# StarsX/RayTracedGGX

Measured on AMD Instinct MI355X. Metric: Mrays/s + ms/frame, bunny 1920x1080 1spp+denoise, 1/2/4/8 GPUs, higher is better.
Workload: dtype f32; 1 GPU; configs[1]: bunny.obj + rnl_cross env, 1920x1080, 1spp GGX reflection + full denoise chain (refl H,V; diff H,V, shared-memory variant; temporal; tone map), all-metal default materials, dt=1/60; parallelism=row strips x1, history_apron_rows=18, history_overreach_rows=0, setup_priming_frames=256, trace_workgroup_waves=12

## Files before the change

include/rtggx.h:

```cpp
#ifndef RTGGX_H
#define RTGGX_H

#include <stddef.h>
#include <stdint.h>

#ifdef __cplusplus
extern "C" {
#endif

typedef struct rtggx_context rtggx_context;

enum { RTGGX_GROUND = 0, RTGGX_MODEL_OBJ = 1, RTGGX_NUM_MESH = 2 };

typedef struct RtggxCBGlobal {
  float    WorldViewProjs[2][16];
  float    WorldViewProjsPrev[2][16];
  float    Worlds[2][12];
  float    WorldITs0[12];
  float    WorldIT1[11];
  uint32_t FrameIndex;
} RtggxCBGlobal;
typedef struct RtggxRayGenConstants {
  float ProjToWorld[16];
  float EyePt[4];
  float ProjBias[2];
  float pad[2];
} RtggxRayGenConstants;
typedef struct RtggxCBPerObject {
  float WorldViewProj[16];
  float ProjBias[2];
  float pad[2];
} RtggxCBPerObject;
typedef struct RtggxCBMaterial {
  float BaseColors[2][4];
  float RoughMetals[2][4];
} RtggxCBMaterial;
typedef struct RtggxFrameConstants {
  RtggxCBGlobal        global;
  RtggxRayGenConstants rayGen;
  RtggxCBPerObject     perObject[2];
  RtggxCBMaterial      material;
} RtggxFrameConstants;

enum { RTGGX_FORMAT_RGBA32F = 2, RTGGX_FORMAT_RGBA16F = 10, RTGGX_FORMAT_BC6H_UF16 = 95, RTGGX_FORMAT_BC6H_SF16 = 96 };

enum {
  RTGGX_BUF_VISIBILITY = 0,
  RTGGX_BUF_DEPTH = 1,
  RTGGX_BUF_NORMAL = 2,
  RTGGX_BUF_ROUGH_METAL = 3,
  RTGGX_BUF_VELOCITY = 4,
  RTGGX_BUF_RT_REFL = 5,
  RTGGX_BUF_RT_DIFF = 6,
  RTGGX_BUF_TSS0 = 7,
  RTGGX_BUF_TSS1 = 8,
  RTGGX_BUF_FLT_RFL = 9,
  RTGGX_BUF_FLT_DFF = 10,
  RTGGX_BUF_BACKBUFFER = 11,
  RTGGX_BUF_SH_COEFFS = 12,
  RTGGX_BUF_BVH_NODES0 = 13,
  RTGGX_BUF_BVH_TRIS0 = 14,
  RTGGX_BUF_BVH_NODES1 = 15,
  RTGGX_BUF_BVH_TRIS1 = 16,
  RTGGX_BUF_TLAS = 17,
  RTGGX_BUF_ENV = 18,
  RTGGX_BUF_BVH4_NODES0 = 19,
  RTGGX_BUF_BVH4_NODES1 = 20,
  RTGGX_BUF_BIN_WORK = 21,
  RTGGX_BUF_BVH4_TOP0 = 22,
  RTGGX_BUF_BVH4_TOP1 = 23,
  RTGGX_BUF_EXCHANGE_TOKENS = 24,
  RTGGX_BUF_ACC_REFL = 25,
  RTGGX_BUF_ACC_DIFF = 26,
  RTGGX_BUF_CONVERGED = 27,
  RTGGX_BUF_COUNT = 28
};

typedef struct RtggxTimings {
  float update_as, visibility, ray_trace, spatial_refl_h, spatial_refl_v, spatial_diff_h, spatial_diff_v,
        temporal, tone_map, frame,
        ray_trace_kernel;
} RtggxTimings;

const char* rtggx_last_error(void);

int  rtggx_create(rtggx_context** out, uint32_t width, uint32_t height, int device);
void rtggx_destroy(rtggx_context* ctx);

int  rtggx_set_strip(rtggx_context* ctx, uint32_t row_begin, uint32_t row_end);

int  rtggx_set_history_apron(rtggx_context* ctx, uint32_t rows);
int  rtggx_history_overreach(rtggx_context* ctx, uint32_t* rows, int reset);

int  rtggx_set_stream(rtggx_context* ctx, void* hip_stream);
int  rtggx_get_stream(rtggx_context* ctx, void** hip_stream);
#define RTGGX_MAX_PEERS 16
#define RTGGX_IPC_HANDLE_BYTES 64
int  rtggx_set_history_peers(rtggx_context* ctx, uint32_t world, const uint32_t* bounds, void* const* tss0, void* const* tss1);
int  rtggx_history_ipc_export(rtggx_context* ctx, void* handles, size_t bytes);
int  rtggx_history_ipc_open(rtggx_context* ctx, const void* handles, size_t bytes, void** tss0, void** tss1);

int  rtggx_set_async_compute(rtggx_context* ctx, int enable);

int  rtggx_set_mesh(rtggx_context* ctx, uint32_t slot, const float* verts, uint32_t num_verts,
                    const uint32_t* indices, uint32_t num_indices);
int  rtggx_set_env(rtggx_context* ctx, int format, uint32_t size, uint32_t mips, const void* data, size_t bytes);
enum { RTGGX_ENV_EQUIRECT = 0, RTGGX_ENV_VCROSS = 1, RTGGX_ENV_HCROSS = 2 };
enum { RTGGX_PIXELS_RGBE8 = 0, RTGGX_PIXELS_RGB32F = 1 };
int  rtggx_set_env_image(rtggx_context* ctx, int layout, int pixels, uint32_t width, uint32_t height, const void* data, size_t bytes,
                         uint32_t cube_size);
int  rtggx_generate_env_mips(rtggx_context* ctx);
int  rtggx_set_material(rtggx_context* ctx, uint32_t mesh, const float base_color[4], float roughness, float metallic);
int  rtggx_set_metallic(rtggx_context* ctx, uint32_t mesh, float metallic);
int  rtggx_set_sampler(rtggx_context* ctx, int vndf);
int  rtggx_set_ray_rate(rtggx_context* ctx, uint32_t pixels_per_ray);
#define RTGGX_MAX_RECURSION_DEPTH 4u
int  rtggx_set_max_recursion_depth(rtggx_context* ctx, uint32_t depth);
#define RTGGX_MAX_SAMPLES_PER_PIXEL 8u
int  rtggx_set_samples_per_pixel(rtggx_context* ctx, uint32_t samples);
#define RTGGX_MIN_SAMPLE_SET 256u
#define RTGGX_MAX_SAMPLE_SET 65536u
int  rtggx_set_sample_set(rtggx_context* ctx, uint32_t size);
int  rtggx_set_accumulation(rtggx_context* ctx, int enable);
int  rtggx_reset_accumulation(rtggx_context* ctx);
int  rtggx_accumulated_frames(rtggx_context* ctx, uint32_t* frames);
int  rtggx_present_accumulation(rtggx_context* ctx);

typedef struct RtggxScore {
  uint64_t index;
  uint32_t frame_index;
  uint32_t pad;
  uint64_t pixels, covered;
  uint64_t skipped_out, skipped_raw;
  double se_out_rgb, se_out_luma;
  double se_raw_rgb, se_raw_luma;
  double ref_rgb2, ref_luma2;
  double se_out_rgb_cov, se_raw_rgb_cov, ref_rgb2_cov;
} RtggxScore;
enum { RTGGX_SCORE_RING = 256 };
int  rtggx_set_reference(rtggx_context* ctx, const void* rgba16f, size_t bytes);
int  rtggx_reference_from_accumulation(rtggx_context* ctx);
int  rtggx_set_scoring(rtggx_context* ctx, int enable);
int  rtggx_read_scores(rtggx_context* ctx, RtggxScore* out, uint32_t capacity, uint32_t* count);

int  rtggx_set_sample_map(rtggx_context* ctx, const uint8_t* counts, uint32_t blocks_x, uint32_t blocks_y);
int  rtggx_read_sample_map(rtggx_context* ctx, uint8_t* counts, uint32_t capacity, uint32_t* blocks_x, uint32_t* blocks_y);

int  rtggx_build_as(rtggx_context* ctx);

int  rtggx_refit_as(rtggx_context* ctx, uint32_t slot, const float* verts, uint32_t num_verts);
int  rtggx_refit_as_device(rtggx_context* ctx, uint32_t slot, const float* device_verts, uint32_t num_verts, void* hip_stream);
int  rtggx_set_refit_policy(rtggx_context* ctx, float rebuild_ratio, uint32_t steps_per_frame);
int  rtggx_refit_stats(rtggx_context* ctx, uint32_t slot, float* cost_ratio, uint32_t* refits, uint32_t* rebuilds);

int  rtggx_update_frame(rtggx_context* ctx, const RtggxFrameConstants* constants);
int  rtggx_update_as(rtggx_context* ctx);
int  rtggx_transform_sh(rtggx_context* ctx);
int  rtggx_render_visibility(rtggx_context* ctx);
int  rtggx_ray_trace(rtggx_context* ctx);
int  rtggx_denoise(rtggx_context* ctx, int use_shared_mem);
int  rtggx_tone_map(rtggx_context* ctx);

int  rtggx_debug_fuse_tone_map(rtggx_context* ctx, int mode);
int  rtggx_debug_placement(rtggx_context* ctx, int force_small, uint32_t* key, uint32_t* where);
int  rtggx_debug_tile_words(rtggx_context* ctx, int enable);
int  rtggx_debug_static_sky(rtggx_context* ctx, int enable);
int  rtggx_debug_sky_runs(rtggx_context* ctx, uint32_t* runs, uint32_t capacity, uint32_t* tiles_x, uint32_t* tiles_y, uint32_t* threshold);
int  rtggx_debug_settled_sky(rtggx_context* ctx, int enable);
int  rtggx_debug_settled_words(rtggx_context* ctx, uint32_t* words0, uint32_t* words1, uint32_t capacity, uint32_t* blocks_x, uint32_t* blocks_y, uint32_t* epoch);
int  rtggx_debug_collapse_weights(rtggx_context* ctx, const float* set, float* get);
int  rtggx_debug_fence_wait(rtggx_context* ctx, double* us_total, uint32_t* waits, int reset);

int  rtggx_sync(rtggx_context* ctx);
int  rtggx_ray_count(rtggx_context* ctx, uint64_t* rays);
int  rtggx_ray_total(rtggx_context* ctx, uint64_t* rays, int reset);
int  rtggx_debug_counters(rtggx_context* ctx, uint32_t* out, uint32_t n, int reset);
int  rtggx_debug_trace_split(rtggx_context* ctx, uint32_t work_per_wave, uint32_t max_shift, int capacity, uint32_t* last_demand);
int  rtggx_debug_trace_residency(rtggx_context* ctx, uint32_t force_waves, uint32_t* waves, float* share);
int  rtggx_debug_environment(rtggx_context* ctx, const float* dirs3, const float* levels, uint32_t n, int level0_path, float* rgb3);
int  rtggx_get_timings(rtggx_context* ctx, RtggxTimings* out);
#define RTGGX_KERNEL_RING 4096
int  rtggx_enable_timing(rtggx_context* ctx, int mode);
int  rtggx_kernel_times(rtggx_context* ctx, float* ms, uint32_t capacity, uint32_t* count);

int  rtggx_debug_shader_clock(rtggx_context* ctx, double* mhz);

int  rtggx_copy_bandwidth(rtggx_context* ctx, size_t bytes, int iterations, double* gbytes_per_s);

int  rtggx_buffer_size(rtggx_context* ctx, int buffer_id, size_t* bytes);
int  rtggx_readback(rtggx_context* ctx, int buffer_id, void* dst, size_t bytes);
int  rtggx_buffer_ptr(rtggx_context* ctx, int buffer_id, void** device_ptr);
int  rtggx_upload(rtggx_context* ctx, int buffer_id, const void* src, size_t bytes);
int  rtggx_frame_parity(rtggx_context* ctx, uint32_t* parity);
int  rtggx_bvh_root(rtggx_context* ctx, uint32_t slot, int32_t* root);

int  rtggx_trace_rays(rtggx_context* ctx, const float* rays, uint32_t n, float* out);

#ifdef __cplusplus
}
#endif
#endif
```

raytracedggx_amd/capi.py:

```python
import ctypes as C
import os

import numpy as np

_HERE = os.path.dirname(os.path.abspath(__file__))
LIB_PATH = os.path.join(_HERE, "librtggx.so")

BUF_VISIBILITY, BUF_DEPTH, BUF_NORMAL, BUF_ROUGH_METAL, BUF_VELOCITY, BUF_RT_REFL, BUF_RT_DIFF, BUF_TSS0, BUF_TSS1, \
    BUF_FLT_RFL, BUF_FLT_DFF, BUF_BACKBUFFER, BUF_SH_COEFFS, BUF_BVH_NODES0, BUF_BVH_TRIS0, BUF_BVH_NODES1, BUF_BVH_TRIS1, \
    BUF_TLAS, BUF_ENV, BUF_BVH4_NODES0, BUF_BVH4_NODES1, BUF_BIN_WORK, BUF_BVH4_TOP0, BUF_BVH4_TOP1, BUF_EXCHANGE_TOKENS, \
    BUF_ACC_REFL, BUF_ACC_DIFF, BUF_CONVERGED = range(28)
MAX_PEERS, IPC_HANDLE_BYTES = 16, 64
FORMAT_RGBA32F, FORMAT_RGBA16F, FORMAT_BC6H_UF16, FORMAT_BC6H_SF16 = 2, 10, 95, 96
ENV_EQUIRECT, ENV_VCROSS, ENV_HCROSS = 0, 1, 2
PIXELS_RGBE8, PIXELS_RGB32F = 0, 1

_BUF_DTYPE = {BUF_VISIBILITY: np.uint32, BUF_DEPTH: np.uint32, BUF_NORMAL: np.uint32, BUF_ROUGH_METAL: np.uint16,
              BUF_VELOCITY: np.uint32, BUF_RT_REFL: np.uint32, BUF_RT_DIFF: np.uint32, BUF_TSS0: np.uint64, BUF_TSS1: np.uint64,
              BUF_FLT_RFL: np.uint64, BUF_FLT_DFF: np.uint64, BUF_BACKBUFFER: np.uint32, BUF_SH_COEFFS: np.float32,
              BUF_BVH_NODES0: np.uint32, BUF_BVH_TRIS0: np.uint32, BUF_BVH_NODES1: np.uint32, BUF_BVH_TRIS1: np.uint32,
              BUF_TLAS: np.float32, BUF_ENV: np.uint16, BUF_BVH4_NODES0: np.uint32, BUF_BVH4_NODES1: np.uint32, BUF_BIN_WORK: np.uint32,
              BUF_BVH4_TOP0: np.uint32, BUF_BVH4_TOP1: np.uint32, BUF_EXCHANGE_TOKENS: np.uint32,
              BUF_ACC_REFL: np.float32, BUF_ACC_DIFF: np.float32, BUF_CONVERGED: np.uint64}

EXPORTS = ["rtggx_last_error", "rtggx_create", "rtggx_destroy", "rtggx_set_strip", "rtggx_set_stream", "rtggx_set_mesh",
           "rtggx_set_env", "rtggx_set_material", "rtggx_set_metallic", "rtggx_build_as", "rtggx_update_frame", "rtggx_update_as",
           "rtggx_transform_sh", "rtggx_render_visibility", "rtggx_ray_trace", "rtggx_denoise", "rtggx_tone_map", "rtggx_sync",
           "rtggx_ray_count", "rtggx_get_timings", "rtggx_enable_timing", "rtggx_buffer_size", "rtggx_readback", "rtggx_buffer_ptr",
           "rtggx_upload", "rtggx_frame_parity", "rtggx_bvh_root", "rtggx_trace_rays", "rtggx_ray_total", "rtggx_kernel_times", "rtggx_debug_counters", "rtggx_debug_trace_split", "rtggx_debug_trace_residency", "rtggx_get_stream", "rtggx_set_history_peers", "rtggx_history_ipc_export", "rtggx_history_ipc_open",
           "rtggx_set_async_compute", "rtggx_set_history_apron", "rtggx_history_overreach", "rtggx_copy_bandwidth", "rtggx_refit_as", "rtggx_refit_as_device", "rtggx_refit_stats", "rtggx_set_refit_policy", "rtggx_set_sampler", "rtggx_set_ray_rate", "rtggx_set_max_recursion_depth", "rtggx_set_samples_per_pixel", "rtggx_debug_fuse_tone_map", "rtggx_debug_placement", "rtggx_debug_tile_words", "rtggx_debug_static_sky", "rtggx_debug_settled_sky", "rtggx_debug_settled_words", "rtggx_debug_sky_runs", "rtggx_debug_collapse_weights", "rtggx_debug_fence_wait", "rtggx_debug_shader_clock", "rtggx_debug_environment",
           "rtggx_set_accumulation", "rtggx_reset_accumulation", "rtggx_accumulated_frames", "rtggx_present_accumulation", "rtggx_set_sample_set",
           "rtggx_set_reference", "rtggx_reference_from_accumulation", "rtggx_set_scoring", "rtggx_read_scores",
           "rtggx_set_env_image", "rtggx_generate_env_mips",
           "rtggx_set_sample_map", "rtggx_read_sample_map"]
SCORE_RING = 256


class Timings(C.Structure):
    _fields_ = [(n, C.c_float) for n in ("update_as", "visibility", "ray_trace", "spatial_refl_h", "spatial_refl_v",
                                         "spatial_diff_h", "spatial_diff_v", "temporal", "tone_map", "frame", "ray_trace_kernel")]


class Score(C.Structure):
    _fields_ = [("index", C.c_uint64), ("frame_index", C.c_uint32), ("pad", C.c_uint32), ("pixels", C.c_uint64), ("covered", C.c_uint64),
                ("skipped_out", C.c_uint64), ("skipped_raw", C.c_uint64)] + \
               [(n, C.c_double) for n in ("se_out_rgb", "se_out_luma", "se_raw_rgb", "se_raw_luma", "ref_rgb2", "ref_luma2",
                                          "se_out_rgb_cov", "se_raw_rgb_cov", "ref_rgb2_cov")]

    def as_dict(self):
        return {n: getattr(self, n) for n, _ in self._fields_ if n != "pad"}


_lib = None


def load():
    global _lib
    if _lib is not None:
        return _lib
    if not os.path.exists(LIB_PATH):
        raise ImportError("librtggx.so is not built: run `python -c 'import __graft_entry__ as g; g.build()'` "
                          "or `make -C raytracedggx_amd` (hipcc, gfx950). There is no CPU path.")
    L = C.CDLL(LIB_PATH)
    L.rtggx_last_error.restype = C.c_char_p
    vp = C.c_void_p
    L.rtggx_create.argtypes = [C.POINTER(vp), C.c_uint32, C.c_uint32, C.c_int]
    L.rtggx_destroy.argtypes = [vp]
    L.rtggx_destroy.restype = None
    L.rtggx_set_strip.argtypes = [vp, C.c_uint32, C.c_uint32]
    L.rtggx_set_stream.argtypes = [vp, vp]
    L.rtggx_set_async_compute.argtypes = [vp, C.c_int]
    L.rtggx_set_ray_rate.argtypes = [vp, C.c_uint32]
    L.rtggx_set_max_recursion_depth.argtypes = [vp, C.c_uint32]
    L.rtggx_set_samples_per_pixel.argtypes = [vp, C.c_uint32]
    L.rtggx_set_sample_set.argtypes = [vp, C.c_uint32]
    L.rtggx_set_accumulation.argtypes = [vp, C.c_int]
    L.rtggx_reset_accumulation.argtypes = [vp]
    L.rtggx_accumulated_frames.argtypes = [vp, C.POINTER(C.c_uint32)]
    L.rtggx_present_accumulation.argtypes = [vp]
    L.rtggx_set_reference.argtypes = [vp, vp, C.c_size_t]
    L.rtggx_reference_from_accumulation.argtypes = [vp]
    L.rtggx_set_scoring.argtypes = [vp, C.c_int]
    L.rtggx_read_scores.argtypes = [vp, C.POINTER(Score), C.c_uint32, C.POINTER(C.c_uint32)]
    L.rtggx_set_sample_map.argtypes = [vp, vp, C.c_uint32, C.c_uint32]
    L.rtggx_read_sample_map.argtypes = [vp, vp, C.c_uint32, C.POINTER(C.c_uint32), C.POINTER(C.c_uint32)]
    L.rtggx_set_history_apron.argtypes = [vp, C.c_uint32]
# ... 67 lines not shown

    def set_stream(self, stream_handle):
        self._check(self.L.rtggx_set_stream(self.h, C.c_void_p(stream_handle)))

    def shader_clock_mhz(self):
        m = C.c_double()
        self._check(self.L.rtggx_debug_shader_clock(self.h, C.byref(m)))
        return m.value

    def copy_bandwidth(self, nbytes=1 << 30, iterations=8):
        g = C.c_double()
        self._check(self.L.rtggx_copy_bandwidth(self.h, int(nbytes), int(iterations), C.byref(g)))
        return g.value

    def set_history_apron(self, rows):
        self._check(self.L.rtggx_set_history_apron(self.h, int(rows)))

    def history_overreach(self, reset=True):
        n = C.c_uint32()
        self._check(self.L.rtggx_history_overreach(self.h, C.byref(n), int(reset)))
        return n.value

    def set_async_compute(self, enable):
        self._check(self.L.rtggx_set_async_compute(self.h, int(bool(enable))))

    def set_mesh(self, slot, verts, indices):
        v = np.ascontiguousarray(verts, np.float32).reshape(-1, 6)
        i = np.ascontiguousarray(indices, np.uint32).reshape(-1)
        self._check(self.L.rtggx_set_mesh(self.h, slot, _p(v), v.shape[0], _p(i), i.size))

    def refit_as(self, slot, verts):
        v = np.ascontiguousarray(verts, np.float32).reshape(-1, 6)
        self._check(self.L.rtggx_refit_as(self.h, slot, _p(v), v.shape[0]))

    def refit_as_device(self, slot, device_ptr, num_verts, stream=0):
        self.L.rtggx_refit_as_device.argtypes = [C.c_void_p, C.c_uint32, C.c_void_p, C.c_uint32, C.c_void_p]
        self._check(self.L.rtggx_refit_as_device(self.h, slot, C.c_void_p(int(device_ptr)), int(num_verts), C.c_void_p(int(stream) or None)))

    def fence_wait(self, reset=True):
        us, n = C.c_double(0.0), C.c_uint32(0)
        self.L.rtggx_debug_fence_wait.argtypes = [C.c_void_p, C.POINTER(C.c_double), C.POINTER(C.c_uint32), C.c_int]
        self._check(self.L.rtggx_debug_fence_wait(self.h, C.byref(us), C.byref(n), 1 if reset else 0))
        return us.value, n.value

    def fuse_tone_map(self, mode):
        self._check(self.L.rtggx_debug_fuse_tone_map(self.h, -1 if mode is None else 1 if mode else 0))

    def tile_words(self, enable):
        self._check(self.L.rtggx_debug_tile_words(self.h, 1 if enable else 0))

    def static_sky(self, enable):
        self._check(self.L.rtggx_debug_static_sky(self.h, 1 if enable else 0))

    def sky_runs(self):
        tiles = ((self.W + 15) // 16) * ((self.H + 15) // 16 + 1)
        runs = np.zeros(tiles, np.uint32)
        tx, ty, th = C.c_uint32(), C.c_uint32(), C.c_uint32()
        self.L.rtggx_debug_sky_runs.argtypes = [C.c_void_p, C.c_void_p, C.c_uint32, C.c_void_p, C.c_void_p, C.c_void_p]
        self._check(self.L.rtggx_debug_sky_runs(self.h, _p(runs), tiles, C.byref(tx), C.byref(ty), C.byref(th)))
        return runs[:tx.value * ty.value].reshape(ty.value, tx.value), int(th.value)

    def settled_sky(self, enable):
        self.L.rtggx_debug_settled_sky.argtypes = [C.c_void_p, C.c_int]
        self._check(self.L.rtggx_debug_settled_sky(self.h, 1 if enable else 0))

    def settled_words(self):
        n = ((self.W + 63) // 64) * ((self.H + 3) // 4)
        w = np.zeros((2, n), np.uint32)
        bx, by, ep = C.c_uint32(), C.c_uint32(), C.c_uint32()
        self.L.rtggx_debug_settled_words.argtypes = [C.c_void_p, C.c_void_p, C.c_void_p, C.c_uint32, C.c_void_p, C.c_void_p, C.c_void_p]
        self._check(self.L.rtggx_debug_settled_words(self.h, _p(w[0]), _p(w[1]), n, C.byref(bx), C.byref(by), C.byref(ep)))
        return np.ascontiguousarray(w.reshape(2, bx.value, by.value).transpose(0, 2, 1)), int(ep.value)

    def placement(self, force_small=-1):
        k, w = C.c_uint32(), C.c_uint32()
        self.L.rtggx_debug_placement.argtypes = [C.c_void_p, C.c_int, C.c_void_p, C.c_void_p]
        self._check(self.L.rtggx_debug_placement(self.h, int(force_small), C.byref(k), C.byref(w)))
        names = ("main", "B", "C", "R", "?")
        key = {n: bool((k.value >> i) & 1) for i, n in enumerate(("small", "strip", "deforming", "diffuse", "caller_stream"))}
        where = {"raster": names[(w.value >> 16) & 15], "gen": names[w.value & 15], "trace": names[(w.value >> 4) & 15], "shade": names[(w.value >> 8) & 15], "frames_in_flight": (w.value >> 12) & 15}
        return key, where

    def collapse_weights(self, area=None, tris=None):
        self.L.rtggx_debug_collapse_weights.argtypes = [C.c_void_p, C.c_void_p, C.c_void_p]
        get = (C.c_float * 2)()
        if area is not None:
            st = (C.c_float * 2)(float(area), float(tris))
            self._check(self.L.rtggx_debug_collapse_weights(self.h, st, get))
        else:
            self._check(self.L.rtggx_debug_collapse_weights(self.h, None, get))
        return float(get[0]), float(get[1])

    def set_history_peers(self, bounds, tss0, tss1):
        self.L.rtggx_set_history_peers.argtypes = [C.c_void_p, C.c_uint32, C.c_void_p, C.c_void_p, C.c_void_p]
        if bounds is None:
            self._check(self.L.rtggx_set_history_peers(self.h, 0, None, None, None))
            return
        world = len(bounds) - 1
        b = (C.c_uint32 * (world + 1))(*[int(x) for x in bounds])
        p0 = (C.c_void_p * world)(*[C.c_void_p(int(x) or None) for x in tss0])
        p1 = (C.c_void_p * world)(*[C.c_void_p(int(x) or None) for x in tss1])
        self._check(self.L.rtggx_set_history_peers(self.h, world, b, p0, p1))

    def history_ipc_export(self):
        self.L.rtggx_history_ipc_export.argtypes = [C.c_void_p, C.c_void_p, C.c_size_t]
        buf = C.create_string_buffer(2 * IPC_HANDLE_BYTES)
# ... 250 lines not shown
```

raytracedggx_amd/csrc/context.hip:

```cpp
#include <cstdarg>
#include <cstdio>
#include <cstring>
#include <cmath>
#include <vector>
#include "capi_internal.h"
#include "rt_queue.h"

#ifndef RT_REFIT_REBUILD_RATIO
#define RT_REFIT_REBUILD_RATIO 1.2f
#endif
#ifndef RT_REBUILD_STEPS
#define RT_REBUILD_STEPS 16u
#endif
namespace rt {
static thread_local char g_err[512] = "";
void setError(const char* fmt, ...) {
  va_list ap; va_start(ap, fmt); vsnprintf(g_err, sizeof g_err, fmt, ap); va_end(ap);
}

__global__ void uploadParamsKernel(FrameParams src, FrameParams* dst) {
  const uint32_t* s = reinterpret_cast<const uint32_t*>(&src);
  uint32_t* d = reinterpret_cast<uint32_t*>(dst);
  for (uint32_t i = threadIdx.x; i < sizeof(FrameParams) / 4; i += blockDim.x) d[i] = s[i];
}
int uploadParams(rtggx_context* c, uint32_t slot, hipStream_t s) {
  hipLaunchKernelGGL(uploadParamsKernel, dim3(1), dim3(64), 0, s, c->slots[slot], c->dParams + slot);
  RT_HIP(hipGetLastError());
  return 0;
}
int resetSettled(rtggx_context* c) {
  for (auto& w : c->settled) {
    RT_HIP(hipMemset(w, 0xFF, c->settledWords() * 4));
    RT_HIP(hipMemset2D(w + c->settledPitch + 1u, (size_t)c->settledPitch * 4, 0, (size_t)c->settledY * 4, c->settledX));
  }
  RT_HIP(hipStreamSynchronize(nullptr));
  return 0;
}
int allocSet(rtggx_context* c, uint32_t i) {
  InputSet& s = c->sets[i];
  const size_t n = (size_t)c->W * c->H, slots = (size_t)c->numBinsMax * c->binSlots;
  for (DevBuf<uint32_t>* p : {&s.normal, &s.depth32, &s.velocity, &s.rtRefl, &s.rtDiff}) if (!*p) RT_HIP(allocFilled(*p, n));
  if (!s.roughMetal) RT_HIP(allocFilled(s.roughMetal, n));
  if (!s.rayQueue) RT_HIP(alloc(s.rayQueue, slots * sizeof(rt::RayRec)));
  if (!s.hitQueue) RT_HIP(alloc(s.hitQueue, slots * 8));
  if (!s.binCount) RT_HIP(allocFilled(s.binCount, (size_t)c->numBinsMax));
  if (!s.splitList) RT_HIP(alloc(s.splitList, (size_t)RT_SPLIT_CAP));
  if (!s.skyRun) RT_HIP(allocFilled(s.skyRun, c->skyTiles));
  c->breakSkyRuns();
  s.splitCount = c->largeCountBase + 2 + i;
  if (!s.evRead) RT_HIP(create(s.evRead, RT_EVENT_FLAGS));
  return 0;
}

static int initContext(rtggx_context* c, uint32_t width, uint32_t height, int device) {
  c->device = device; c->W = width; c->H = height; c->rowBegin = 0; c->rowEnd = height;
  const size_t n = (size_t)width * height;
  int prioLeast = 0, prioGreatest = 0;
  RT_HIP(hipDeviceGetStreamPriorityRange(&prioLeast, &prioGreatest));
  const int prioMid = (prioLeast + prioGreatest) / 2;
  RT_HIP(create(c->ownMain, hipStreamNonBlocking, prioGreatest));
  RT_HIP(create(c->ownAS, hipStreamNonBlocking, prioLeast));
  c->streamMain = c->ownMain; c->streamAS = c->ownAS;
  RT_HIP(create(c->ownVis, hipStreamNonBlocking, prioLeast)); c->streamVis = c->ownVis;
  RT_HIP(create(c->streamRefit, hipStreamNonBlocking, prioMid));
  for (Event* e : {&c->evVis, &c->evRefit, &c->evAS, &c->evRT}) RT_HIP(create(*e, RT_EVENT_FLAGS));
  for (auto& f : c->frames) { RT_HIP(create(f.gen, RT_EVENT_FLAGS)); RT_HIP(create(f.trace, RT_EVENT_FLAGS)); }
  for (auto& e : c->tev) RT_HIP(create(e));
  c->rebuildRatio = RT_REFIT_REBUILD_RATIO; c->rebuildSteps = RT_REBUILD_STEPS;
  {
    hipDeviceProp_t prop;
    RT_HIP(hipGetDeviceProperties(&prop, device));
    c->numCUs = prop.multiProcessorCount > 0 ? (uint32_t)prop.multiProcessorCount : 256u;
  }
  c->numBinsMax = ((width + 15) / 16) * ((height + 15) / 16) * 4u;
  if (c->numBinsMax < 64u) c->numBinsMax = 64u;
  c->binSlots = RT_BIN_MIN;
  c->largeCapacity = 1u << 16;
  c->skyTiles = (size_t)((width + 15) / 16) * ((height + 15) / 16 + 1);
  for (auto& b : c->largeTrisBuf) RT_HIP(alloc(b, (size_t)c->largeCapacity * 56));
  RT_HIP(allocFilled(c->largeCountBase, 2 + RT_SETS));
  for (uint32_t i = 0; i < RT_SETS; ++i) { const int r = allocSet(c, i); if (r) return r; }
  for (auto& v : c->vis) { RT_HIP(allocFilled(v.depth, n)); RT_HIP(allocFilled(v.dirty, c->skyTiles, 0xFF)); }
  RT_HIP(allocFilled(c->visDirtyOnes, c->skyTiles, 0xFF));
  c->settledX = (width + 63) / 64; c->settledY = (height + 3) / 4;
  c->settledPitch = (c->settledY + 3u) / 4u * 4u + 2u;
  for (auto& w : c->settled) RT_HIP(alloc(w, c->settledWords()));
  { const int r = resetSettled(c); if (r) return r; }
  RT_HIP(allocFilled(c->backbuffer, n));
  RT_HIP(allocFilled(c->tss[0], n)); RT_HIP(allocFilled(c->tss[1], n)); RT_HIP(allocFilled(c->fltRfl, n)); RT_HIP(allocFilled(c->fltDff, n));
  RT_HIP(allocFilled(c->rayCounter, 512));
  RT_HIP(allocFilled(c->rayCounterBuf, 1792));
  c->lastRayCounter32 = c->rayCounterBuf;
  RT_HIP(allocFilled(c->traceStamps, 8));
  RT_HIP(alloc(c->hostRayCounters, 264)); memset(c->hostRayCounters, 0, 264 * 4); RT_HIP(create(c->evRayCounters, hipEventDisableTiming));
  for (auto& b : c->binWorkBuf) RT_HIP(allocFilled(b, (size_t)c->numBinsMax));
  c->selectSet(0);
  c->splitWork = RT_SPLIT_WORK; c->splitMaxShift = RT_SPLIT_MAX_SHIFT;
  RT_HIP(allocFilled(c->dEnvMipOffset, 16));
  RT_HIP(allocFilled(c->dummyRecord, 128));
  RT_HIP(allocFilled(c->histReach, 1));
  RT_HIP(allocFilled(c->exchangeTokens, 2 * RT_MAX_PEERS));
  RT_HIP(allocFilled(c->dPeerTable, sizeof(void*) * 2 * RT_MAX_PEERS + 4 * (RT_MAX_PEERS + 1)));
  RT_HIP(allocFilled(c->sh, 27));
  RT_HIP(alloc(c->cosSinTab, 512));
  RT_HIP(alloc(c->dParams, RT_SLOTS));
  {
    float tab[512];
    for (int s = 0; s < 256; ++s) { const double phi = 2.0 * 3.14159265358979323846 * (double)s / 256.0; tab[s] = (float)cos(phi); tab[256 + s] = (float)sin(phi); }
    RT_HIP(hipMemcpy(c->cosSinTab, tab, sizeof tab, hipMemcpyHostToDevice));
  }
  const float bc0[4] = {0.95f, 0.93f, 0.88f, 1.0f}, bc1[4] = {1.0f, 0.71f, 0.29f, 1.0f};
  const float rm0[4] = {0.5f, 1.0f, 0.0f, 0.0f}, rm1[4] = {0.16f, 1.0f, 0.0f, 0.0f};
  memcpy(c->material.BaseColors[0], bc0, 16); memcpy(c->material.BaseColors[1], bc1, 16);
  memcpy(c->material.RoughMetals[0], rm0, 16); memcpy(c->material.RoughMetals[1], rm1, 16);
  memset(c->invWorld, 0, sizeof c->invWorld);
  for (int i = 0; i < 2; ++i) for (int k = 0; k < 4; ++k) c->invWorld[i][k * 5] = 1.0f;
  memset(c->slots, 0, sizeof c->slots);
  { const int r = setMeshImpl(c, RTGGX_GROUND, &kGroundVerts[0][0], 24, kGroundIdx, 36); if (r) return r; }
  RT_HIP(hipStreamSynchronize(nullptr));
  return 0;
}
int allocSamples(rtggx_context* c) {
  if (c->sppAcc && c->sppParams) return 0;
  const size_t n = (size_t)c->W * c->H;
  if (!c->evSpp) RT_HIP(create(c->evSpp, hipEventDisableTiming));
  if (!c->sppParams) RT_HIP(alloc(c->sppParams, RT_SLOTS * RTGGX_MAX_SAMPLES_PER_PIXEL));
  if (!c->sppAcc) {
    RT_HIP(allocFilled(c->sppAcc, n * 2u * 3u));
    RT_HIP(hipStreamSynchronize(nullptr));
  }
  return 0;
}
int allocSampleTable(rtggx_context* c, uint32_t m) {
  DevBuf<float>& tab = c->cosSinWide[rtggx_context::sampleSetSlot(m)];
  if (tab) return 0;
  std::vector<float> host(2u * (size_t)m);
  for (uint32_t s = 0; s < m; ++s) { const double phi = 2.0 * 3.14159265358979323846 * (double)s / (double)m; host[2u * s] = (float)cos(phi); host[2u * s + 1u] = (float)sin(phi); }
  DevBuf<float> d;
  hipError_t e = alloc(d, host.size());
  if (e == hipSuccess) e = hipMemcpy(d, host.data(), host.size() * sizeof(float), hipMemcpyHostToDevice);
  if (e != hipSuccess) { setError("rtggx_set_sample_set: %s (%zu bytes for the table of %u samples)", hipGetErrorString(e), host.size() * sizeof(float), m); return -2; }
  tab = std::move(d);
  return 0;
}
int allocAccumulation(rtggx_context* c) {
  if (c->accRefl) return 0;
  const size_t n = (size_t)c->W * c->H;
// ... 115 lines not shown
int rtggx_history_ipc_export(rtggx_context* c, void* handles, size_t bytes) {
  RT_CHECK_CTX(c);
  static_assert(sizeof(hipIpcMemHandle_t) == RTGGX_IPC_HANDLE_BYTES, "hipIpcMemHandle_t size");
  if (!handles || bytes < 2 * sizeof(hipIpcMemHandle_t)) { setError("rtggx_history_ipc_export: room for two %zu-byte handles", sizeof(hipIpcMemHandle_t)); return -1; }
  hipIpcMemHandle_t h[2];
  for (int p = 0; p < 2; ++p) RT_HIP(hipIpcGetMemHandle(&h[p], c->tss[p]));
  memcpy(handles, h, sizeof h);
  return 0;
}
int rtggx_history_ipc_open(rtggx_context* c, const void* handles, size_t bytes, void** tss0, void** tss1) {
  RT_CHECK_CTX(c);
  if (!handles || bytes < 2 * sizeof(hipIpcMemHandle_t) || !tss0 || !tss1) { setError("rtggx_history_ipc_open: bad arguments"); return -1; }
  hipIpcMemHandle_t h[2]; memcpy(h, handles, sizeof h);
  void* p[2] = {nullptr, nullptr};
  for (int k = 0; k < 2; ++k) {
    IpcMapping mapped;
    RT_HIP(hipIpcOpenMemHandle(mapped.put(), h[k], hipIpcMemLazyEnablePeerAccess));
    p[k] = mapped;
    c->ipcMapped.push_back(std::move(mapped));
  }
  *tss0 = p[0]; *tss1 = p[1];
  return 0;
}

int rtggx_get_stream(rtggx_context* c, void** stream) {
  RT_CHECK_CTX(c);
  if (!stream) { setError("rtggx_get_stream: null"); return -1; }
  *stream = (void*)c->streamMain;
  return 0;
}

int rtggx_set_async_compute(rtggx_context* c, int enable) {
  RT_CHECK_CTX(c);
  if ((enable != 0) == c->asyncCompute) return 0;
  RT_HIP(syncStreams(c));
  c->asyncCompute = enable != 0; c->sppStream = nullptr;
  c->streamAS = c->asyncCompute ? c->ownAS : c->streamMain;
  c->streamVis = c->asyncCompute ? c->ownVis : nullptr;
  c->evVisStream = nullptr; for (auto& f : c->frames) f.genFrame = 0u;
  return 0;
}

int rtggx_set_ray_rate(rtggx_context* c, uint32_t pixelsPerRay) {
  RT_CHECK_CTX(c);
  if (pixelsPerRay != 1u && pixelsPerRay != 4u) { setError("rtggx_set_ray_rate: %u pixels per ray: 1 or 4", pixelsPerRay); return -1; }
  if (pixelsPerRay != 1u && c->samplesRequested > 1u) { setError("rtggx_set_ray_rate: rate %u on a context tracing %u samples per pixel (rtggx_set_samples_per_pixel): one asks for fewer rays, the other for more", pixelsPerRay, c->samplesRequested); return -1; }
  if (pixelsPerRay != 1u && c->accumulateRequested) { setError("rtggx_set_ray_rate: rate %u on an accumulating context (rtggx_set_accumulation): three quarters of such a frame are interpolations", pixelsPerRay); return -1; }
  if (pixelsPerRay != 1u && (c->rowBegin > 0u || c->rowEnd < c->H)) { setError("rtggx_set_ray_rate: rate %u on a strip (rows [%u,%u) of %u): whole frames only", pixelsPerRay, c->rowBegin, c->rowEnd, c->H); return -1; }
  if (pixelsPerRay == c->rayRate) return 0;
  RT_HIP(syncStreams(c));
  c->rayRate = pixelsPerRay;
  for (auto& b : c->binWorkBuf) RT_HIP(hipMemset(b, 0, (size_t)c->numBinsMax * 4));
  RT_HIP(hipDeviceSynchronize());
  c->splitDemand = 0u; c->rayCountersInFlight = false; c->lastFrameRays = 0xFFFFFFFFu; c->traceLaunches = 0u;
  return 0;
}

int rtggx_set_max_recursion_depth(rtggx_context* c, uint32_t depth) {
  RT_CHECK_CTX(c);
  if (depth < 1u || depth > RTGGX_MAX_RECURSION_DEPTH) { setError("rtggx_set_max_recursion_depth: depth %u: 1 to %u", depth, RTGGX_MAX_RECURSION_DEPTH); return -1; }
  c->depthRequested = depth;
  return 0;
}

int rtggx_set_samples_per_pixel(rtggx_context* c, uint32_t samples) {
  RT_CHECK_CTX(c);
  if (samples != 1u && samples != 2u && samples != 4u && samples != 8u) { setError("rtggx_set_samples_per_pixel: %u samples per pixel: 1, 2, 4 or %u", samples, RTGGX_MAX_SAMPLES_PER_PIXEL); return -1; }
  if (samples > 1u && c->rayRate != 1u) { setError("rtggx_set_samples_per_pixel: %u samples per pixel on a context tracing one pixel in %u (rtggx_set_ray_rate): one asks for more rays, the other for fewer", samples, c->rayRate); return -1; }
  if (samples > 1u) { const int r = allocSamples(c); if (r) return r; }
  c->samplesRequested = samples;
  return 0;
}

int rtggx_set_sample_set(rtggx_context* c, uint32_t size) {
  RT_CHECK_CTX(c);
  if (size < RTGGX_MIN_SAMPLE_SET || size > RTGGX_MAX_SAMPLE_SET || (size & (size - 1u)) != 0u) { setError("rtggx_set_sample_set: %u samples: a power of two from %u to %u", size, RTGGX_MIN_SAMPLE_SET, RTGGX_MAX_SAMPLE_SET); return -1; }
  if (size == c->sampleSetRequested) return 0;
  RT_HIP(syncStreams(c));
  if (size > RTGGX_MIN_SAMPLE_SET) { const int r = allocSampleTable(c, size); if (r) return r; }
  c->sampleSetRequested = size;
  return 0;
}

int rtggx_set_accumulation(rtggx_context* c, int enable) {
  RT_CHECK_CTX(c);
  if (enable && c->rayRate != 1u) { setError("rtggx_set_accumulation: on a context tracing one pixel in %u (rtggx_set_ray_rate): three quarters of such a frame are interpolations", c->rayRate); return -1; }
  if (enable) { const int r = allocAccumulation(c); if (r) return r; }
  c->accumulateRequested = enable != 0;
  return 0;
}
int rtggx_reset_accumulation(rtggx_context* c) {
  RT_CHECK_CTX(c);
  if (c->accRefl) {
    const size_t n = (size_t)c->W * c->H;
    RT_HIP(hipMemsetAsync(c->accRefl, 0, n * 16, c->streamMain));
    RT_HIP(hipMemsetAsync(c->accDiff, 0, n * 16, c->streamMain));
  }
  c->accumFrames = 0u;
  return 0;
}
int rtggx_accumulated_frames(rtggx_context* c, uint32_t* frames) {
  RT_CHECK_CTX(c);
  if (!frames) { setError("rtggx_accumulated_frames: null result"); return -1; }
  *frames = c->accumFrames;
  return 0;
}
int rtggx_present_accumulation(rtggx_context* c) {
// ... 180 lines not shown
```

raytracedggx_amd/csrc/debug.hip:

```cpp
#include <cstring>
#include "capi_internal.h"
#include "rt_queue.h"
namespace rt {
__global__ void __launch_bounds__(256) copyKernel(const float4* __restrict__ src, float4* __restrict__ dst, size_t n) {
  for (size_t i = (size_t)blockIdx.x * 256u + threadIdx.x; i < n; i += (size_t)gridDim.x * 256u) dst[i] = src[i];
}
typedef float __attribute__((ext_vector_type(4))) CopyVec4;
__global__ void __launch_bounds__(256) copyKernelNT(const CopyVec4* __restrict__ src, CopyVec4* __restrict__ dst, size_t n) {
  for (size_t i = (size_t)blockIdx.x * 256u + threadIdx.x; i < n; i += (size_t)gridDim.x * 256u) __builtin_nontemporal_store(__builtin_nontemporal_load(&src[i]), &dst[i]);
}
}
using namespace rt;

extern "C" {
int rtggx_ray_count(rtggx_context* c, uint64_t* rays) {
  RT_CHECK_CTX(c);
  uint32_t h[256];
  RT_HIP(syncStreams(c));
  RT_HIP(hipMemcpy(h, c->lastRayCounter32, sizeof h, hipMemcpyDeviceToHost));
  uint64_t s = 0; for (auto v : h) s += v;
  *rays = s;
  return 0;
}

int rtggx_debug_counters(rtggx_context* c, uint32_t* out, uint32_t n, int reset) {
  RT_CHECK_CTX(c);
  if (n > 768) { setError("rtggx_debug_counters: at most 768 words"); return -1; }
  RT_HIP(syncStreams(c));
  RT_HIP(hipMemcpy(out, c->rayCounterBuf + 1024, (size_t)n * 4, hipMemcpyDeviceToHost));
  if (reset) { RT_HIP(hipMemset(c->rayCounterBuf + 1024, 0, 768 * 4)); RT_HIP(hipStreamSynchronize(nullptr)); }
  return 0;
}

int rtggx_debug_fence_wait(rtggx_context* c, double* usTotal, uint32_t* waits, int reset) {
  RT_CHECK_CTX(c);
  if (usTotal) *usTotal = c->fenceWaitUs;
  if (waits) *waits = c->fenceWaits;
  if (reset) { c->fenceWaitUs = 0.0; c->fenceWaits = 0u; }
  return 0;
}
int rtggx_debug_fuse_tone_map(rtggx_context* c, int mode) {
  RT_CHECK_CTX(c);
  c->fuseToneMap = mode < 0 ? -1 : mode != 0;
  return 0;
}
int rtggx_debug_tile_words(rtggx_context* c, int enable) {
  RT_CHECK_CTX(c);
  c->useTileWords = enable != 0;
  c->breakSkyRuns();
  return 0;
}
int rtggx_debug_static_sky(rtggx_context* c, int enable) {
  RT_CHECK_CTX(c);
  c->staticSky = enable != 0;
  c->breakSkyRuns();
  return 0;
}
int rtggx_debug_sky_runs(rtggx_context* c, uint32_t* runs, uint32_t capacity, uint32_t* tilesX, uint32_t* tilesY, uint32_t* threshold) {
  RT_CHECK_CTX(c);
  const uint32_t n = c->skyGen.tilesX * c->skyGen.tilesY;
  if (!runs || capacity < n || n > c->skyTiles) { setError("rtggx_debug_sky_runs: room for %u words", n); return -1; }
  RT_HIP(syncStreams(c));
  if (n) RT_HIP(hipMemcpy(runs, c->cur().skyRun, (size_t)n * 4, hipMemcpyDeviceToHost));
  for (uint32_t i = 0; i < n; ++i) runs[i] = (runs[i] >> 8) == c->skyEpoch ? runs[i] & 0xFFu : 0u;
  if (tilesX) *tilesX = c->skyGen.tilesX;
  if (tilesY) *tilesY = c->skyGen.tilesY;
  if (threshold) *threshold = RT_SKY_PREV_RUN + 1u;
  return 0;
}
int rtggx_debug_settled_sky(rtggx_context* c, int enable) {
  RT_CHECK_CTX(c);
  c->settledSky = enable != 0;
  c->breakSkyRuns();
  return 0;
}
int rtggx_debug_settled_words(rtggx_context* c, uint32_t* words0, uint32_t* words1, uint32_t capacity, uint32_t* blocksX, uint32_t* blocksY, uint32_t* epoch) {
  RT_CHECK_CTX(c);
  const uint32_t n = c->settledX * c->settledY;
  if (!words0 || !words1 || capacity < n) { setError("rtggx_debug_settled_words: room for %u words each", n); return -1; }
  RT_HIP(syncStreams(c));
  uint32_t* const out[2] = {words0, words1};
  for (int p = 0; p < 2 && n; ++p)
    RT_HIP(hipMemcpy2D(out[p], (size_t)c->settledY * 4, c->settled[p] + c->settledPitch + 1u, (size_t)c->settledPitch * 4, (size_t)c->settledY * 4, c->settledX, hipMemcpyDeviceToHost));
  if (blocksX) *blocksX = c->settledX;
  if (blocksY) *blocksY = c->settledY;
  if (epoch) *epoch = c->skyEpoch;
  return 0;
}
int rtggx_debug_placement(rtggx_context* c, int forceSmall, uint32_t* key, uint32_t* where) {
  RT_CHECK_CTX(c);
  if (forceSmall < -1 || forceSmall > 1) { setError("rtggx_debug_placement: force_small is -1, 0 or 1"); return -1; }
  c->forcePlacement = forceSmall;
  if (forceSmall >= 0) c->lastTraceSmall = forceSmall == 1;
  if (key) *key = c->lastPlacement[0];
  if (where) *where = c->lastPlacement[1];
  return 0;
}
int rtggx_debug_collapse_weights(rtggx_context* c, const float* set, float* get) {
  RT_CHECK_CTX(c);
  if (set) { if (!(set[0] >= 0.0f) || !(set[1] >= 0.0f) || !(set[0] + set[1] > 0.0f)) { setError("rtggx_debug_collapse_weights: two non-negative weights, not both zero"); return -1; }
             c->collapseWeights[0] = set[0]; c->collapseWeights[1] = set[1]; }
  if (get) { get[0] = c->collapseWeights[0]; get[1] = c->collapseWeights[1]; }
  return 0;
}
int rtggx_debug_trace_residency(rtggx_context* c, uint32_t forceWaves, uint32_t* waves, float* share) {
  RT_CHECK_CTX(c);
  if (forceWaves != 0u && forceWaves != 10u && forceWaves != 12u && forceWaves != 14u && forceWaves != 16u) { setError("rtggx_debug_trace_residency: %u waves: 0, 10, 12, 14 or 16", forceWaves); return -1; }
  c->traceWavesForced = forceWaves;
  if (forceWaves) c->traceWaves = forceWaves;
  if (waves) *waves = c->traceWaves;
  if (share) *share = c->traceShare;
  return 0;
}

int rtggx_debug_environment(rtggx_context* c, const float* dirs3, const float* levels, uint32_t n, int level0Path, float* rgb3) {
  RT_CHECK_CTX(c);
  if (!c->env.texels) { setError("rtggx_debug_environment: no environment map"); return -1; }
  if (n == 0 || !dirs3 || !rgb3 || (!levels && !level0Path)) { setError("rtggx_debug_environment: no directions, levels or result (n %u)", n); return -1; }
  DevBuf<float> dD, dL, dO;
  hipError_t e = alloc(dD, (size_t)n * 3);
  if (e == hipSuccess) e = alloc(dO, (size_t)n * 3);
  if (e == hipSuccess && levels) e = alloc(dL, (size_t)n);
  if (e == hipSuccess) e = hipMemcpy(dD, dirs3, (size_t)n * 12, hipMemcpyHostToDevice);
  if (e == hipSuccess && levels) e = hipMemcpy(dL, levels, (size_t)n * 4, hipMemcpyHostToDevice);
  int r = 0;
  if (e == hipSuccess) r = launchDebugEnvironment(c, dD, dL, n, level0Path, dO, c->streamMain);
  if (e == hipSuccess && !r) e = hipStreamSynchronize(c->streamMain);
  if (e == hipSuccess && !r) e = hipMemcpy(rgb3, dO, (size_t)n * 12, hipMemcpyDeviceToHost);
  if (e != hipSuccess) { setError("rtggx_debug_environment: %s", hipGetErrorString(e)); return -2; }
  return r;
}

int rtggx_debug_trace_split(rtggx_context* c, uint32_t workPerWave, uint32_t maxShift, int capacity, uint32_t* lastDemand) {
  RT_CHECK_CTX(c);
  if (maxShift > 3u) { setError("rtggx_debug_trace_split: max_shift %u > 3", maxShift); return -1; }
  if (capacity > (int)RT_SPLIT_CAP) { setError("rtggx_debug_trace_split: capacity %d > %u", capacity, RT_SPLIT_CAP); return -1; }
  RT_HIP(syncStreams(c));
  if (lastDemand) RT_HIP(hipMemcpy(lastDemand, c->cur().splitCount, 4, hipMemcpyDeviceToHost));
  c->splitWork = workPerWave; c->splitMaxShift = maxShift;
  c->splitCapForced = capacity < 0 ? 0xFFFFFFFFu : ((uint32_t)capacity / 32u) * 32u;
  return 0;
}

int rtggx_ray_total(rtggx_context* c, uint64_t* rays, int reset) {
  RT_CHECK_CTX(c);
  unsigned long long h[256];
  RT_HIP(syncStreams(c));
  RT_HIP(hipMemcpy(h, c->rayCounter + 256, sizeof h, hipMemcpyDeviceToHost));
// ... 12 lines not shown
    for (uint32_t i = 0; i < RTGGX_KERNEL_RING; ++i) { RT_HIP(create(c->kevBegin[i])); RT_HIP(create(c->kevEnd[i])); }
  }
  return 0;
}
int rtggx_kernel_times(rtggx_context* c, float* ms, uint32_t capacity, uint32_t* count) {
  RT_CHECK_CTX(c);
  RT_HIP(syncStreams(c));
  const uint32_t n = c->kevCount < capacity ? c->kevCount : capacity;
  for (uint32_t i = 0; i < n; ++i) RT_HIP(hipEventElapsedTime(&ms[i], c->kevBegin[i], c->kevEnd[i]));
  *count = n;
  c->kevCount = 0;
  return 0;
}
int rtggx_get_timings(rtggx_context* c, RtggxTimings* out) {
  RT_CHECK_CTX(c);
  if (!c->timing || !c->timingsPending) { setError("rtggx_get_timings: timing not enabled or no complete frame"); return -1; }
  RT_HIP(syncStreams(c));
  auto ms = [&](int a, int b) { float t = 0.0f; hipEventElapsedTime(&t, c->tev[a], c->tev[b]); return t; };
  RtggxTimings t;
  t.update_as = ms(0, 1); t.visibility = ms(2, 13); t.ray_trace = ms(3, 14); t.spatial_refl_h = ms(9, 4); t.spatial_refl_v = ms(4, 5);
  t.spatial_diff_h = ms(5, 6); t.spatial_diff_v = ms(6, 7); t.temporal = ms(7, 8); t.tone_map = ms(8, 10); t.frame = ms(2, 10);
  t.ray_trace_kernel = ms(11, 12);
  *out = t;
  return 0;
}

static int bufferInfo(rtggx_context* c, int id, void** ptr, size_t* bytes) {
  const size_t n = (size_t)c->W * c->H;
  switch (id) {
    case RTGGX_BUF_VISIBILITY: case RTGGX_BUF_DEPTH: *ptr = nullptr; *bytes = n * 4; return 0;
    case RTGGX_BUF_NORMAL: *ptr = c->cur().normal; *bytes = n * 4; return 0;
    case RTGGX_BUF_ROUGH_METAL: *ptr = c->cur().roughMetal; *bytes = n * 2; return 0;
    case RTGGX_BUF_VELOCITY: *ptr = c->cur().velocity; *bytes = n * 4; return 0;
    case RTGGX_BUF_RT_REFL: *ptr = c->cur().rtRefl; *bytes = n * 4; return 0;
    case RTGGX_BUF_RT_DIFF: *ptr = c->cur().rtDiff; *bytes = n * 4; return 0;
    case RTGGX_BUF_TSS0: *ptr = c->tss[0]; *bytes = n * 8; return 0;
    case RTGGX_BUF_TSS1: *ptr = c->tss[1]; *bytes = n * 8; return 0;
    case RTGGX_BUF_FLT_RFL: *ptr = c->fltRflIsFltDff ? c->fltDff.get() : c->fltRfl.get(); *bytes = n * 8; return 0;
    case RTGGX_BUF_FLT_DFF: *ptr = c->fltDff; *bytes = n * 8; return 0;
    case RTGGX_BUF_BACKBUFFER: *ptr = c->backbuffer; *bytes = n * 4; return 0;
    case RTGGX_BUF_SH_COEFFS: *ptr = c->sh; *bytes = 108; return 0;
    case RTGGX_BUF_BVH_NODES0: case RTGGX_BUF_BVH_NODES1: { const MeshDev& m = c->mesh[id == RTGGX_BUF_BVH_NODES1]; *ptr = m.nodes; *bytes = m.numTris > 1 && m.nodes ? (size_t)(m.numTris - 1) * 64 : 0; return 0; }
    case RTGGX_BUF_BVH_TRIS0: case RTGGX_BUF_BVH_TRIS1: { const MeshDev& m = c->mesh[id == RTGGX_BUF_BVH_TRIS1]; *ptr = m.tris; *bytes = m.tris ? (size_t)m.numTris * 64 : 0; return 0; }
    case RTGGX_BUF_TLAS: *ptr = nullptr; *bytes = 128; return 0;
    case RTGGX_BUF_BVH4_NODES0: case RTGGX_BUF_BVH4_NODES1: { const MeshDev& m = c->mesh[id == RTGGX_BUF_BVH4_NODES1]; *ptr = m.nodes4; *bytes = m.numTris > 1 && m.nodes4 ? (size_t)(m.numTris - 1) * sizeof(Bvh4Node) : 0; return 0; }
    case RTGGX_BUF_BVH4_TOP0: case RTGGX_BUF_BVH4_TOP1: { const MeshDev& m = c->mesh[id == RTGGX_BUF_BVH4_TOP1]; *ptr = m.top; *bytes = m.top ? (size_t)m.topCount * sizeof(Bvh4Node) : 0; return 0; }
    case RTGGX_BUF_BIN_WORK: *ptr = c->binWork; *bytes = (size_t)(((c->W + 15) / 16) * ((c->H + 15) / 16)) * 4u * 4u; return 0;
    case RTGGX_BUF_ENV: *ptr = c->env.texels; *bytes = (size_t)c->env.totalTexels * 8; return 0;
    case RTGGX_BUF_EXCHANGE_TOKENS: *ptr = c->exchangeTokens; *bytes = 4 * 2 * RT_MAX_PEERS; return 0;
    case RTGGX_BUF_ACC_REFL: case RTGGX_BUF_ACC_DIFF: case RTGGX_BUF_CONVERGED:
      if (!c->accRefl) { setError("buffer %d exists once accumulation has been enabled (rtggx_set_accumulation)", id); return -1; }
      *ptr = id == RTGGX_BUF_ACC_REFL ? (void*)c->accRefl : id == RTGGX_BUF_ACC_DIFF ? (void*)c->accDiff : (void*)c->converged;
      *bytes = n * (id == RTGGX_BUF_CONVERGED ? 8u : 16u); return 0;
    default: setError("unknown buffer id %d", id); return -1;
  }
}

int rtggx_buffer_size(rtggx_context* c, int id, size_t* bytes) { RT_CHECK_CTX(c); void* p; return bufferInfo(c, id, &p, bytes); }

int rtggx_buffer_ptr(rtggx_context* c, int id, void** dptr) {
  RT_CHECK_CTX(c);
  size_t bytes;
  const int r = bufferInfo(c, id, dptr, &bytes);
  if (r) return r;
  if (id == RTGGX_BUF_VISIBILITY || id == RTGGX_BUF_DEPTH) *dptr = c->curVis().depth;
  if (!*dptr) { setError("buffer %d has no device storage", id); return -1; }
  return 0;
}

int rtggx_readback(rtggx_context* c, int id, void* dst, size_t bytes) {
  RT_CHECK_CTX(c);
  void* p; size_t need;
  int r = bufferInfo(c, id, &p, &need);
  if (r) return r;
  if (bytes < need) { setError("rtggx_readback: buffer %d needs %zu bytes, %zu given", id, need, bytes); return -1; }
  RT_HIP(syncStreams(c));
  if (id == RTGGX_BUF_TLAS) { memcpy(dst, c->invWorld, 128); return 0; }
  if (id == RTGGX_BUF_VISIBILITY || id == RTGGX_BUF_DEPTH) {
    DevBuf<uint32_t> dVis, dDepth;
    RT_HIP(alloc(dVis, need / 4)); RT_HIP(alloc(dDepth, need / 4));
    r = unpackVisDepth(c, dVis, dDepth, c->streamMain);
    if (!r && hipStreamSynchronize(c->streamMain) != hipSuccess) { setError("readback: stream sync failed"); r = -2; }
    if (!r) { hipError_t e = hipMemcpy(dst, id == RTGGX_BUF_VISIBILITY ? dVis.get() : dDepth.get(), need, hipMemcpyDeviceToHost); if (e != hipSuccess) { setError("hipMemcpy: %s", hipGetErrorString(e)); r = -2; } }
    return r;
  }
  if (need == 0) return 0;
  RT_HIP(hipMemcpy(dst, p, need, hipMemcpyDeviceToHost));
  return 0;
}

int rtggx_upload(rtggx_context* c, int id, const void* src, size_t bytes) {
  RT_CHECK_CTX(c);
  void* p; size_t need;
  int r = bufferInfo(c, id, &p, &need);
  if (r) return r;
  if (bytes != need) { setError("rtggx_upload: buffer %d is %zu bytes, %zu given", id, need, bytes); return -1; }
  RT_HIP(syncStreams(c));
  c->toneMapDone = false;
  c->curVis().flags.rasterFrame = 0u;
  c->breakSkyRuns();
  if (id == RTGGX_BUF_VISIBILITY || id == RTGGX_BUF_DEPTH) {
    DevBuf<uint32_t> dVis, dDepth;
    RT_HIP(alloc(dVis, need / 4)); RT_HIP(alloc(dDepth, need / 4));
    r = unpackVisDepth(c, dVis, dDepth, c->streamMain);
    if (!r && hipStreamSynchronize(c->streamMain) != hipSuccess) { setError("upload: stream sync failed"); r = -2; }
    if (!r) { hipError_t e = hipMemcpy(id == RTGGX_BUF_VISIBILITY ? dVis.get() : dDepth.get(), src, need, hipMemcpyHostToDevice); if (e != hipSuccess) { setError("hipMemcpy: %s", hipGetErrorString(e)); r = -2; } }
// ... 90 lines not shown
```

raytracedggx_amd/csrc/denoise.hip:

```cpp
#include <cstring>
#include <type_traits>
#include "rtggx_context.h"

namespace rt {

#define RT_RADIUS 16
#ifndef RT_VBW
#define RT_VBW 16
#define RT_VBH 16
#endif

RT_DEV float rcpFast(float x) { return __builtin_amdgcn_rcpf(x); }

struct GTexel { float nx, ny, nz, nw, rough, metal, depth; };

RT_DEV GTexel loadG(const uint32_t* __restrict__ normal, const uint16_t* __restrict__ roughMetal, const uint32_t* __restrict__ depth32,
                    int x, int y, int W, int H) {
  GTexel g;
  if (x < 0 || y < 0 || x >= W || y >= H) { g.nx = g.ny = g.nz = -1023.0f; g.nw = 0.0f; g.rough = 0.0f; g.metal = 0.0f; g.depth = 0.0f; return g; }
  const size_t i = (size_t)y * W + x;
  const uint32_t n = normal[i];
  g.nx = (float)(2 * (int)(n & 1023u) - 1023);
  g.ny = (float)(2 * (int)((n >> 10) & 1023u) - 1023);
  g.nz = (float)(2 * (int)((n >> 20) & 1023u) - 1023);
  g.nw = (float)(n >> 30) * (1.0f / 3.0f);
  const uint32_t rm = roughMetal[i];
  g.rough = (float)(rm & 0xFFu) * (1.0f / 255.0f); g.metal = (rm >> 8) == 255u ? 1.0f : (float)(rm >> 8) * (1.0f / 255.0f);
  g.depth = (float)depth32[i] * (1.0f / 16777215.0f);
  return g;
}
RT_DEV f3 TM3(f3 c) { const float r = rcpFast(1.0f + ((c.x * 0.25f + c.y * 0.5f) + c.z * 0.25f)); return mk3(c.x * r, c.y * r, c.z * r); }
RT_DEV f3 ITM3(f3 c) { const float r = rcpFast(1.0f - ((c.x * 0.25f + c.y * 0.5f) + c.z * 0.25f)); return mk3(c.x * r, c.y * r, c.z * r); }
struct Targets {
  const uint32_t* normal; const uint16_t* roughMetal; const uint32_t* depth32; const uint32_t* velocity;
  const uint32_t* rtRefl; const uint32_t* rtDiff;
  uint2* scratch; const uint2* history; uint2* fltRfl; uint2* fltDff; uint32_t* backbuffer;
  int W, H, rowBegin, rowEnd;
  int histLo, histHi; uint32_t* histReach;
  const uint2* const* peerHist; const uint32_t* peerBounds; int peerWorld;
  int outBegin, outEnd;
  const uint32_t* tileWords; int tilesX, tileRow0;
  const uint32_t* skyRun; uint32_t skyEpoch;
  uint32_t* settledOut; const uint32_t* settledIn; uint32_t settledPitch;
};
#define RT_SGPR(v) ((uint32_t)__builtin_amdgcn_readfirstlane((int)(v)))
RT_DEV uint32_t tileWordsOr(const uint32_t* words, uint32_t i0, uint32_t i1, uint32_t i2, uint32_t i3) {
  uint32_t a, b, c, d;
  asm volatile("s_load_dword %0, %4, %5\n\ts_load_dword %1, %4, %6\n\ts_load_dword %2, %4, %7\n\ts_load_dword %3, %4, %8\n\ts_waitcnt lgkmcnt(0)"
               : "=&s"(a), "=&s"(b), "=&s"(c), "=&s"(d) : "s"(words), "s"(RT_SGPR(i0 * 4u)), "s"(RT_SGPR(i1 * 4u)), "s"(RT_SGPR(i2 * 4u)), "s"(RT_SGPR(i3 * 4u)) : "memory");
  return a | b | c | d;
}

RT_DEV uint32_t tileWordsOr6(const uint32_t* words, uint32_t i0, uint32_t i1, uint32_t i2, uint32_t i3, uint32_t i4, uint32_t i5) {
  uint32_t a, b, c, d, e, f;
  asm volatile("s_load_dword %0, %6, %7\n\ts_load_dword %1, %6, %8\n\ts_load_dword %2, %6, %9\n\ts_load_dword %3, %6, %10\n\ts_load_dword %4, %6, %11\n\ts_load_dword %5, %6, %12\n\ts_waitcnt lgkmcnt(0)"
               : "=&s"(a), "=&s"(b), "=&s"(c), "=&s"(d), "=&s"(e), "=&s"(f)
               : "s"(words), "s"(RT_SGPR(i0 * 4u)), "s"(RT_SGPR(i1 * 4u)), "s"(RT_SGPR(i2 * 4u)), "s"(RT_SGPR(i3 * 4u)), "s"(RT_SGPR(i4 * 4u)), "s"(RT_SGPR(i5 * 4u)) : "memory");
  return a | b | c | d | e | f;
}
RT_DEV uint32_t skyRunMin6(const uint32_t* words, uint32_t epoch, uint32_t i0, uint32_t i1, uint32_t i2, uint32_t i3, uint32_t i4, uint32_t i5) {
  uint32_t w[6];
  asm volatile("s_load_dword %0, %6, %7\n\ts_load_dword %1, %6, %8\n\ts_load_dword %2, %6, %9\n\ts_load_dword %3, %6, %10\n\ts_load_dword %4, %6, %11\n\ts_load_dword %5, %6, %12\n\ts_waitcnt lgkmcnt(0)"
               : "=&s"(w[0]), "=&s"(w[1]), "=&s"(w[2]), "=&s"(w[3]), "=&s"(w[4]), "=&s"(w[5])
               : "s"(words), "s"(RT_SGPR(i0 * 4u)), "s"(RT_SGPR(i1 * 4u)), "s"(RT_SGPR(i2 * 4u)), "s"(RT_SGPR(i3 * 4u)), "s"(RT_SGPR(i4 * 4u)), "s"(RT_SGPR(i5 * 4u)) : "memory");
  uint32_t run = 0xFFu;
#pragma unroll
  for (int k = 0; k < 6; ++k) run = min(run, (w[k] >> 8) == epoch ? w[k] & 0xFFu : 0u);
  return run;
}

typedef uint32_t U2 __attribute__((ext_vector_type(2)));
typedef uint32_t U4 __attribute__((ext_vector_type(4)));
RT_DEV void loadTemporalWords(const uint32_t* rowA, const uint32_t* rowB, const uint32_t* col0, const uint32_t* col1, const uint32_t* col2,
                              U4& a4, U2& a2, U4& b4, U2& b2, U4& c0, U4& c1, U4& c2) {
  asm volatile("s_load_dwordx4 %0, %7, 0x0\n\ts_load_dwordx2 %1, %7, 0x10\n\ts_load_dwordx4 %2, %8, 0x0\n\ts_load_dwordx2 %3, %8, 0x10\n\t"
               "s_load_dwordx4 %4, %9, 0x0\n\ts_load_dwordx4 %5, %10, 0x0\n\ts_load_dwordx4 %6, %11, 0x0\n\ts_waitcnt lgkmcnt(0)"
               : "=&s"(a4), "=&s"(a2), "=&s"(b4), "=&s"(b2), "=&s"(c0), "=&s"(c1), "=&s"(c2)
               : "s"(rowA), "s"(rowB), "s"(col0), "s"(col1), "s"(col2) : "memory");
}
RT_DEV void loadToneMapWords(const uint32_t* col0, const uint32_t* col1, const uint32_t* col2, U4& a4, U2& a2, U4& b4, U2& b2, U4& c4, U2& c2) {
  asm volatile("s_load_dwordx4 %0, %6, 0x0\n\ts_load_dwordx2 %1, %6, 0x10\n\ts_load_dwordx4 %2, %7, 0x0\n\ts_load_dwordx2 %3, %7, 0x10\n\t"
               "s_load_dwordx4 %4, %8, 0x0\n\ts_load_dwordx2 %5, %8, 0x10\n\ts_waitcnt lgkmcnt(0)"
               : "=&s"(a4), "=&s"(a2), "=&s"(b4), "=&s"(b2), "=&s"(c4), "=&s"(c2) : "s"(col0), "s"(col1), "s"(col2) : "memory");
}

#define RT_LOG2E 1.44269504088896341f

struct Centre { float nx, ny, nz, depth, rough, gaussK , depthK ; };
#define RT_NORMAL_SCALE_SQ 1046529.0f
RT_DEV float log2OfDot(float I) {
  const float d = fmaxf((I - RT_NORMAL_SCALE_SQ) * (1.0f / RT_NORMAL_SCALE_SQ), -1.0f);
  const float xr = 1.0f + d;
  const float dropped = (1.0f - xr) + d;
  return __builtin_fmaf(dropped, RT_LOG2E, __builtin_amdgcn_logf(xr));
}
template <bool DIFFUSE, int UNIFORM = 0>
RT_DEV float tapWeight(const Centre& c, int i, float nx, float ny, float nz, float depth, float rough) {
// ... 18 lines not shown
  const float sigma = (float)(br + 1) * (1.0f / 3.0f);
  c.gaussK = (-0.5f * RT_LOG2E) * rcpFast(sigma * sigma);
  c.depthK = depth * (4.0f * RT_LOG2E);
  return c;
}
template <int MODE>
RT_DEV void storeFiltered(const Targets& T, size_t pix, float mx, float my, float mz, float wsum) {
  const float rw = rcpFast(wsum);
  f3 mu = mk3(mx * rw, my * rw, mz * rw);
  if (MODE == 0 || MODE == 2) T.scratch[pix] = packRGBA16F(mu.x, mu.y, mu.z, 0.0f);
  if (MODE == 1) { mu = ITM3(mu); const uint2 v = packRGBA16F(mu.x, mu.y, mu.z, 1.0f); if (T.fltRfl) T.fltRfl[pix] = v; T.fltDff[pix] = v; }
  if (MODE == 3) {
    const f4 dest = unpackRGBA16F(T.fltRfl[pix]);
    mu = ITM3(mu);
    T.fltDff[pix] = packRGBA16F(dest.x + mu.x, dest.y + mu.y, dest.z + mu.z, dest.w);
  }
}
template <int MODE>
RT_DEV void storeSkipped(const Targets& T, size_t pix) {
  if (MODE == 1) { const f3 s = unpackR11G11B10F(T.rtRefl[pix]); const uint2 v = packRGBA16F(s.x, s.y, s.z, 0.0f); if (T.fltRfl) T.fltRfl[pix] = v; T.fltDff[pix] = v; }
}
template <int MODE>
RT_DEV f3 tapColour(const Targets& T, size_t ti) {
  if (MODE & 1) { const f4 v = unpackRGBA16F(T.scratch[ti]); return mk3(v.x, v.y, v.z); }
  return TM3(unpackR11G11B10F(MODE >= 2 ? T.rtDiff[ti] : T.rtRefl[ti]));
}

template <int MODE>
__global__ void __launch_bounds__(256) spatialDirectKernel(Targets T) {
  constexpr bool vertical = (MODE & 1) != 0;
  constexpr bool diffuse = MODE >= 2;
  const int x = blockIdx.x * 64 + (threadIdx.x & 63);
  const int y = T.rowBegin + blockIdx.y * 4 + (threadIdx.x >> 6);
  if (x >= T.W || y >= T.rowEnd) return;
  const size_t pix = (size_t)y * T.W + x;
  const GTexel gc = loadG(T.normal, T.roughMetal, T.depth32, x, y, T.W, T.H);
  if (diffuse ? (gc.nw <= 0.0f || gc.metal >= 1.0f) : (gc.nw <= 0.0f)) { storeSkipped<MODE>(T, pix); return; }
  const Centre c = makeCentre<diffuse>(gc.nx, gc.ny, gc.nz, gc.depth, gc.rough, T.W, T.H);
  float mx = 0.0f, my = 0.0f, mz = 0.0f, wsum = 0.0f;
  for (int i = -RT_RADIUS; i <= RT_RADIUS; ++i) {
    const int tx = vertical ? x : x + i, ty = vertical ? y + i : y;
    const bool inside = tx >= 0 && ty >= 0 && tx < T.W && ty < T.H;
    const GTexel g = loadG(T.normal, T.roughMetal, T.depth32, tx, ty, T.W, T.H);
    if (diffuse && (g.nw <= 0.0f || g.metal >= 1.0f)) continue;
    const f3 src = inside ? tapColour<MODE>(T, (size_t)ty * T.W + tx) : mk3(0.0f, 0.0f, 0.0f);
    const float w = tapWeight<diffuse>(c, i, g.nx, g.ny, g.nz, g.depth, g.nw > 0.0f ? g.rough : __uint_as_float(__float_as_uint(g.rough) | 0x80000000u));
    mx = __builtin_fmaf(src.x, w, mx); my = __builtin_fmaf(src.y, w, my); mz = __builtin_fmaf(src.z, w, mz);
    wsum += w;
  }
  storeFiltered<MODE>(T, pix, mx, my, mz, wsum);
}

typedef float V4 __attribute__((ext_vector_type(4)));
template <int MODE>
__global__ void __launch_bounds__(256) spatialTiledKernel(Targets T) {
  constexpr bool vertical = (MODE & 1) != 0;
  constexpr bool diffuse = MODE >= 2;
  constexpr int BW = vertical ? RT_VBW : 64, BH = vertical ? RT_VBH : 4;
  constexpr int TW = vertical ? RT_VBW : 96, TH = vertical ? RT_VBH + 2 * RT_RADIUS : 4;
  constexpr int PER = vertical ? BW * BH / 256 : 1, ROWSTEP = 256 / BW;
  constexpr int N = TW * TH;
  __shared__ V4 smA[N], smB[N];
  __shared__ uint32_t roughLo, roughHi, unflagged;
  if (threadIdx.x == 0) { roughLo = 0xFFFFFFFFu; roughHi = 0u; unflagged = 0u; }
  const int bx0 = blockIdx.x * BW, by0 = T.rowBegin + blockIdx.y * BH;
  const int lx = threadIdx.x % BW, ly = threadIdx.x / BW;
  const int x = bx0 + lx;

  static_assert(RT_VBW <= 32 && RT_VBH <= 32, "the V block spans at most two tiles across and three down");
  bool nothingDrawn;
  { const uint32_t txLast = (uint32_t)T.tilesX - 1u, tx0 = (uint32_t)bx0 >> 4, tx1 = min(tx0 + 1u, txLast);
    const uint32_t ty0 = (uint32_t)(by0 - T.tileRow0) >> 4, ty1 = (uint32_t)(min(by0 + BH, T.rowEnd) - 1 - T.tileRow0) >> 4;
    const uint32_t r0 = ty0 * (uint32_t)T.tilesX, r1 = ty1 * (uint32_t)T.tilesX, rm = ((ty0 + ty1) >> 1) * (uint32_t)T.tilesX;
    if (MODE == 1 && T.skyRun != nullptr && skyRunMin6(T.skyRun, T.skyEpoch, r0 + tx0, r0 + tx1, rm + tx0, rm + tx1, r1 + tx0, r1 + tx1) >= RT_SKY_V_RUN) return;
    nothingDrawn = vertical ? tileWordsOr6(T.tileWords, r0 + tx0, r0 + tx1, rm + tx0, rm + tx1, r1 + tx0, r1 + tx1) == 0u
                            : tileWordsOr(T.tileWords, r0 + tx0, r0 + tx1, r0 + min(tx0 + 2u, txLast), r0 + min(tx0 + 3u, txLast)) == 0u; }
  if (nothingDrawn) {
    if (MODE == 1) {
#pragma unroll
      for (int k = 0; k < PER; ++k) { const int y = by0 + ly + k * ROWSTEP; if (x < T.W && y < T.rowEnd) storeSkipped<MODE>(T, (size_t)y * T.W + x); }
    }
    return;
  }
  bool todo[PER]; bool any = false;
#pragma unroll
  for (int k = 0; k < PER; ++k) {
    const int y = by0 + ly + k * ROWSTEP;
    todo[k] = false;
    if (x < T.W && y < T.rowEnd) {
      const size_t pix = (size_t)y * T.W + x;
      const bool skip = (T.normal[pix] >> 30) == 0u || (diffuse && (T.roughMetal[pix] >> 8) == 255u);
      if (skip) storeSkipped<MODE>(T, pix); else { todo[k] = true; any = true; }
    }
  }
  if (!__syncthreads_or(any ? 1 : 0)) return;

  const int ox = vertical ? bx0 : bx0 - RT_RADIUS, oy = vertical ? by0 - RT_RADIUS : by0;
  uint32_t myLo = 0xFFFFFFFFu, myHi = 0u, myUnflagged = 0u;
  for (int t = threadIdx.x; t < N; t += 256) {
    const int tx = ox + t % TW, ty = oy + t / TW;
    float v[8] = {0.0f, 0.0f, 0.0f, 0.0f, 0.0f, 0.0f, 0.0f, 0.0f};
    const bool inside = tx >= 0 && ty >= 0 && tx < T.W && ty < T.H;
    const GTexel g = loadG(T.normal, T.roughMetal, T.depth32, tx, ty, T.W, T.H);
    v[3] = g.depth; v[4] = g.rough;
    if (diffuse) {
      if (g.nw > 0.0f && g.metal < 1.0f) {
        const f3 src = tapColour<MODE>(T, (size_t)ty * T.W + tx);
        v[0] = g.nx; v[1] = g.ny; v[2] = g.nz; v[5] = src.x; v[6] = src.y; v[7] = src.z;
      }
    } else {
      v[0] = g.nx; v[1] = g.ny; v[2] = g.nz;
      if (g.nw <= 0.0f) { v[4] = __uint_as_float(__float_as_uint(g.rough) | 0x80000000u); myUnflagged = 1u; }
      else { myLo = min(myLo, __float_as_uint(g.rough)); myHi = max(myHi, __float_as_uint(g.rough)); }
      if (inside) { const f3 src = tapColour<MODE>(T, (size_t)ty * T.W + tx); v[5] = src.x; v[6] = src.y; v[7] = src.z; }
    }
    smA[t] = V4{v[0], v[1], v[2], v[3]}; smB[t] = V4{v[4], v[5], v[6], v[7]};
  }
  if (!diffuse) {
    for (int o = 32; o > 0; o >>= 1) { myLo = min(myLo, (uint32_t)__shfl_down((int)myLo, o)); myHi = max(myHi, (uint32_t)__shfl_down((int)myHi, o)); }
    const unsigned long long anyUnflagged = __ballot(myUnflagged != 0u);
    if ((threadIdx.x & 63) == 0) { atomicMin(&roughLo, myLo); atomicMax(&roughHi, myHi); if (anyUnflagged) atomicOr(&unflagged, 1u); }
  }
  __syncthreads();
  const int uniform = diffuse ? 0 : (roughLo != roughHi ? 0 : unflagged ? 1 : 2);

  auto filter = [&](auto uniformTag) {
    constexpr int UNIFORM = decltype(uniformTag)::value;
#pragma unroll
    for (int k = 0; k < PER; ++k) {
      if (!todo[k]) continue;
      const int y = by0 + ly + k * ROWSTEP;
      const int ci = vertical ? (ly + k * ROWSTEP + RT_RADIUS) * TW + lx : ly * TW + lx + RT_RADIUS;
      const V4 ca = smA[ci];
      const Centre c = makeCentre<diffuse>(ca.x, ca.y, ca.z, ca.w, smB[ci].x, T.W, T.H);
      float mx = 0.0f, my = 0.0f, mz = 0.0f, wsum = 0.0f;
      typedef __attribute__((address_space(3))) const V4 LdsV4;
      LdsV4* pa = (LdsV4*)&smA[ci - RT_RADIUS * (vertical ? TW : 1)]; LdsV4* pb = (LdsV4*)&smB[ci - RT_RADIUS * (vertical ? TW : 1)];
      asm volatile("" : "+v"(pa)); asm volatile("" : "+v"(pb));
#pragma unroll
      for (int i = -RT_RADIUS; i <= RT_RADIUS; ++i) {
        const int ti = (i + RT_RADIUS) * (vertical ? TW : 1);
        const V4 a = pa[ti], b = pb[ti];
        const float w = tapWeight<diffuse, UNIFORM>(c, i, a.x, a.y, a.z, a.w, b.x);
        mx = __builtin_fmaf(b.y, w, mx); my = __builtin_fmaf(b.z, w, my); mz = __builtin_fmaf(b.w, w, mz);
        wsum += w;
      }
      storeFiltered<MODE>(T, (size_t)y * T.W + x, mx, my, mz, wsum);
    }
  };
  if (uniform == 2) filter(std::integral_constant<int, 2>{});
  else if (uniform == 1) filter(std::integral_constant<int, 1>{});
  else filter(std::integral_constant<int, 0>{});
}

RT_DEV f3 rgbToYCoCg(f3 c) {
  return mk3((c.x * 1.0f + c.y * 2.0f) + c.z * 1.0f, (c.x * 2.0f + c.y * 0.0f) + c.z * -2.0f, (c.x * -1.0f + c.y * 2.0f) + c.z * -1.0f);
}
RT_DEV f3 yCoCgToRGB(f3 c) {
  const float y = c.x * 0.25f, co = c.y * 0.25f, cg = c.z * 0.25f;
  return mk3(y + co - cg, y + cg, y - co - cg);
}
RT_DEV f3 tssTM(f3 hdr) {
  const f3 c = rgbToYCoCg(hdr); const float d = 4.0f + c.x;
  f3 q; div3Shared(c.x, c.y, c.z, d, q.x, q.y, q.z); return q;
}
RT_DEV f3 tssITM(f3 col) { const float k = 4.0f * rcpFast(1.0f - col.x); return yCoCgToRGB(mk3(col.x * k, col.y * k, col.z * k)); }
RT_DEV f3 tssTMSmooth(f3 hdr) { const f3 c = rgbToYCoCg(hdr); const float r = rcpFast(4.0f + c.x); return mk3(c.x * r, c.y * r, c.z * r); }
RT_DEV f2 loadVel(const uint32_t* __restrict__ vel, int x, int y, int W, int H) {
  f2 v; v.x = 0.0f; v.y = 0.0f;
  if (x < 0 || y < 0 || x >= W || y >= H) return v;
  const uint32_t p = vel[(size_t)y * W + x];
  v.x = f16ToF32(p & 0xFFFFu); v.y = f16ToF32(p >> 16);
  return v;
}
RT_DEV f4 loadRGBA16(const uint2* __restrict__ b, int x, int y, int W, int H) {
  if (x < 0 || y < 0 || x >= W || y >= H) { f4 z; z.x = z.y = z.z = z.w = 0.0f; return z; }
  return unpackRGBA16F(b[(size_t)y * W + x]);
}

RT_DEV const uint2* peerHistoryRow(const Targets& T, int iy) {
  int r = 0;
  while (r + 1 < T.peerWorld && (int)T.peerBounds[r + 1] <= iy) ++r;
  return T.peerHist[r] + (size_t)iy * T.W;
}
template <int ROWS, int PITCH>
RT_DEV uint2 temporalPixel(const Targets& T, const float4 (&tile)[ROWS][PITCH], const uint32_t (&velRaw)[ROWS][PITCH], const float (&velSq)[ROWS][PITCH], int x, int y, int lx, int ly) {
  const int W = T.W, H = T.H;
  const float Wf = (float)W, Hf = (float)H;
  const float uvx = ((float)x + 0.5f) * rcpFast(Wf), uvy = ((float)y + 0.5f) * rcpFast(Hf);
  const float4 cur = tile[ly][lx];
  const f3 currentTM = mk3(cur.x, cur.y, cur.z);
  f4 current; current.x = current.y = current.z = 0.0f; current.w = cur.w;
  const int ox[8] = {-1, 1, 0, 0, -1, 1, 1, -1}, oy[8] = {0, 0, -1, 1, -1, -1, 1, 1};
  f2 vmax;
  {
    float speedSq = velSq[ly][lx];
    uint32_t raw = velRaw[ly][lx];
    for (int i = 4; i < 8; ++i) {
      const float sq = velSq[ly + oy[i]][lx + ox[i]];
      const uint32_t r = velRaw[ly + oy[i]][lx + ox[i]];
      if (sq > speedSq) { raw = r; speedSq = sq; }
    }
    vmax.x = f16ToF32(raw & 0xFFFFu); vmax.y = f16ToF32(raw >> 16);
  }
  float alphaFiltered = cur.w;
  for (int i = 0; i < 8; ++i) alphaFiltered = __builtin_fmaf(tile[ly + oy[i]][lx + ox[i]].w, i < 4 ? 0.5f : 0.25f, alphaFiltered);
// ... 296 lines not shown
  T.peerHist = peers ? reinterpret_cast<const uint2* const*>(c->dPeerTable.get()) + (c->frameParity ^ 1u) * RT_MAX_PEERS : nullptr;
  T.peerBounds = peers ? reinterpret_cast<const uint32_t*>(reinterpret_cast<const uint2* const*>(c->dPeerTable.get()) + 2 * RT_MAX_PEERS) : nullptr;
  T.peerWorld = peers ? (int)c->peerWorld : 0;
  { uint32_t gb, ge; passRows(fp, ROWS_GBUFFER, gb, ge);
    T.tileWords = c->tileWords(gb, ge); T.tilesX = (int)((fp.W + 15) / 16); T.tileRow0 = (int)gb; }
  T.skyRun = nullptr; T.skyEpoch = 0u;
  T.settledOut = nullptr; T.settledIn = nullptr; T.settledPitch = c->settledPitch;
  return T;
}

static bool skyVPassMaySkip(rtggx_context* c, const Targets& TV, uint32_t gbufferRow0, uint32_t* epoch) {
  rtggx_context::SkyV now;
  const bool genValid = c->skyGen.any && c->skyGen.frame == c->frameCounter && c->skyGen.epoch == c->skyEpoch && c->skyGen.rows[0] == gbufferRow0;
  now.any = true; now.fltRflNull = TV.fltRfl == nullptr; now.frame = c->frameCounter; now.genEpoch = genValid ? c->skyGen.epoch : 0xFFFFFFFFu;
  now.rows[0] = (uint32_t)TV.rowBegin; now.rows[1] = (uint32_t)TV.rowEnd;
  const rtggx_context::SkyV& was = c->skyV;
  const bool may = c->staticSky && genValid && was.any && (was.frame == now.frame || was.frame + 1u == now.frame) && was.genEpoch == now.genEpoch
                   && was.rows[0] == now.rows[0] && was.rows[1] == now.rows[1] && was.fltRflNull == now.fltRflNull;
  c->skyV = now;
  *epoch = c->skyEpoch;
  return may;
}

static bool skyTemporalMaySkip(rtggx_context* c, const Targets& TT, const FrameParams& fp, bool fused, bool* words) {
  rtggx_context::SkyT now;
  const rtggx_context::SkyT& was = c->skyT;
  const bool whole = fp.rowBegin == 0u && fp.rowEnd == fp.H && fp.W == c->W && fp.H == c->H;
  const bool genValid = c->skyGen.any && c->skyGen.frame == c->frameCounter && c->skyGen.epoch == c->skyEpoch && c->skyGen.rows[0] == (uint32_t)TT.tileRow0;
  now.any = true; now.frame = c->frameCounter; now.epoch = c->skyEpoch; now.parity = c->frameParity;
  now.words = c->staticSky && c->settledSky && !fused && whole && fp.W >= 96u
              && was.any && was.epoch == now.epoch;
  now.rows[0] = (uint32_t)TT.rowBegin; now.rows[1] = (uint32_t)TT.rowEnd;
  const bool may = now.words && genValid && was.words && was.frame + 1u == now.frame && was.parity == (now.parity ^ 1u)
                   && was.rows[0] == now.rows[0] && was.rows[1] == now.rows[1];
  c->skyT = now;
  ++c->tssWrites[now.parity];
  *words = now.words;
  return may;
}

int launchDenoise(rtggx_context* c, const FrameParams& fp, int useLds, hipStream_t s, hipEvent_t done, bool fuseToneMap) {
  c->frameParity ^= 1u;
  if (fp.rowEnd <= fp.rowBegin) return 0;
  const Targets TH = makeTargets(c, fp, ROWS_GBUFFER), TV = makeTargets(c, fp, ROWS_VFILTER), TT = makeTargets(c, fp, ROWS_TEMPORAL);
  const dim3 block(256);
  auto grid = [&](const Targets& T, uint32_t bw, uint32_t bh) { return dim3((fp.W + bw - 1) / bw, (T.rowEnd - T.rowBegin + bh - 1) / bh); };
  auto mark = [&](int i) { if (c->timing) hipEventRecord(c->tev[i], s); };
  const bool anyDiffuse = fp.mat.RoughMetals[0][1] < 1.0f || fp.mat.RoughMetals[1][1] < 1.0f;
  c->fltRflIsFltDff = !anyDiffuse;
  Targets TVr = TV; if (!anyDiffuse) TVr.fltRfl = nullptr;
  { uint32_t epoch;
    if (skyVPassMaySkip(c, TVr, (uint32_t)TV.tileRow0, &epoch) && useLds) { TVr.skyRun = c->cur().skyRun; TVr.skyEpoch = epoch; } }
  if (useLds) {
    hipLaunchKernelGGL(spatialTiledKernel<0>, grid(TH, 64, 4), block, 0, s, TH); mark(4);
    hipLaunchKernelGGL(spatialTiledKernel<1>, grid(TV, RT_VBW, RT_VBH), block, 0, s, TVr); mark(5);
    if (anyDiffuse) hipLaunchKernelGGL(spatialTiledKernel<2>, grid(TH, 64, 4), block, 0, s, TH);
    mark(6);
    if (anyDiffuse) hipLaunchKernelGGL(spatialTiledKernel<3>, grid(TV, RT_VBW, RT_VBH), block, 0, s, TV);
    mark(7);
  } else if (!anyDiffuse) {
    hipLaunchKernelGGL(spatialDirectKernel<0>, grid(TH, 64, 4), block, 0, s, TH); mark(4);
    hipLaunchKernelGGL(spatialDirectKernel<1>, grid(TV, 64, 4), block, 0, s, TVr); mark(5); mark(6); mark(7);
  } else {
    hipLaunchKernelGGL(spatialDirectKernel<0>, grid(TH, 64, 4), block, 0, s, TH); mark(4);
    hipLaunchKernelGGL(spatialDirectKernel<1>, grid(TV, 64, 4), block, 0, s, TV); mark(5);
    hipLaunchKernelGGL(spatialDirectKernel<2>, grid(TH, 64, 4), block, 0, s, TH); mark(6);
    hipLaunchKernelGGL(spatialDirectKernel<3>, grid(TV, 64, 4), block, 0, s, TV); mark(7);
  }
  Targets TTs = TT;
  { bool words;
    const bool may = skyTemporalMaySkip(c, TT, fp, fuseToneMap, &words);
    if (words) { TTs.settledOut = c->settled[c->frameParity]; TTs.skyEpoch = c->skyEpoch; }
    if (may) { TTs.settledIn = c->settled[c->frameParity ^ 1u]; TTs.skyRun = c->cur().skyRun; } }
  if (fuseToneMap) {
    const dim3 g((fp.W + RT_TT_W - 1) / RT_TT_W, (uint32_t)(TT.outEnd - TT.outBegin + RT_TT_H - 1) / RT_TT_H), b(RT_TT_TW * RT_TT_TH);
    launch(temporalToneKernel, g, b, s, nullptr, done, TT);
    c->skyTM.any = false;
  } else launch(TTs.settledOut ? temporalKernel<true> : temporalKernel<false>, grid(TT, 64, RT_TP_ROWS), block, s, nullptr, done, TTs);
  mark(8);
  RT_HIP(hipGetLastError());
  return 0;
}

int launchToneMap(rtggx_context* c, const FrameParams& fp, hipStream_t s, hipEvent_t done, const uint2* source) {
  if (fp.rowEnd <= fp.rowBegin) return 0;
  Targets T = makeTargets(c, fp, ROWS_FINAL);
  if (source) T.scratch = const_cast<uint2*>(source);
  { rtggx_context::SkyTM now;
    now.any = true; now.fromTss = source == nullptr; now.frame = c->frameCounter; now.epoch = c->skyEpoch; now.parity = c->frameParity; now.writes = c->tssWrites[c->frameParity];
    now.rows[0] = (uint32_t)T.rowBegin; now.rows[1] = (uint32_t)T.rowEnd;
    const rtggx_context::SkyTM& was = c->skyTM; const rtggx_context::SkyT& t = c->skyT;
    const bool whole = fp.rowBegin == 0u && fp.rowEnd == fp.H && fp.W == c->W && fp.H == c->H;
    const bool may = c->staticSky && c->settledSky && whole && now.fromTss && t.any && t.words && t.frame == now.frame && t.parity == now.parity && t.epoch == now.epoch
                     && was.any && was.fromTss && was.frame + 1u == now.frame && was.epoch == now.epoch && was.rows[0] == now.rows[0] && was.rows[1] == now.rows[1]
                     && was.parity == (now.parity ^ 1u) && was.writes == c->tssWrites[now.parity ^ 1u];
    c->skyTM = now;
    if (may) { T.settledIn = c->settled[c->frameParity]; T.skyEpoch = c->skyEpoch; } }
  const dim3 grid((fp.W + 63) / 64, (uint32_t)(T.rowEnd - T.rowBegin + RT_TM_ROWS - 1) / RT_TM_ROWS), block(256);
  launch(T.settledIn ? toneMapKernel<true> : toneMapKernel<false>, grid, block, s, nullptr, done, T);
  RT_HIP(hipGetLastError());
  return 0;
}

}
```

raytracedggx_amd/csrc/raytrace.hip:

```cpp
#include <cstring>
#include <type_traits>
#include "rt_queue.h"
#include "rt_traverse.h"

namespace rt {

#define RT_PI 3.1415926535897f
#define RT_SGPR(v) ((uint32_t)__builtin_amdgcn_readfirstlane((int)(v)))

struct EnvRef { const uint2* __restrict__ texels; uint32_t size, mips; const uint32_t* __restrict__ mipOffset; };

RT_DEV void cubeFaceUV(f3 d, int& face, float& u, float& v) {
  const float ax = fabsf(d.x), ay = fabsf(d.y), az = fabsf(d.z);
  if (ax >= ay && ax >= az) { face = d.x >= 0.0f ? 0 : 1; u = (d.x >= 0.0f ? -d.z : d.z) / ax; v = -d.y / ax; }
  else if (ay >= az) { face = d.y >= 0.0f ? 2 : 3; u = d.x / ay; v = (d.y >= 0.0f ? d.z : -d.z) / ay; }
  else { face = d.z >= 0.0f ? 4 : 5; u = (d.z >= 0.0f ? d.x : -d.x) / az; v = -d.y / az; }
}
RT_DEV f3 cubeFaceDir(int face, float u, float v) {
  switch (face) {
    case 0: return mk3(1.0f, -v, -u);
    case 1: return mk3(-1.0f, -v, u);
    case 2: return mk3(u, 1.0f, v);
    case 3: return mk3(u, -1.0f, -v);
    case 4: return mk3(u, -v, 1.0f);
    default: return mk3(-u, -v, -1.0f);
  }
}
template <bool MIP0 = false>
RT_DEV f3 cubeTexel(const EnvRef& e, uint32_t mip, int face, int x, int y) {
  const int s = (int)((e.size >> mip) ? (e.size >> mip) : 1u);
  if (x < 0 || y < 0 || x >= s || y >= s) {
    const float u = ((float)x + 0.5f) / (float)s * 2.0f - 1.0f, v = ((float)y + 0.5f) / (float)s * 2.0f - 1.0f;
    float uu, vv; cubeFaceUV(cubeFaceDir(face, u, v), face, uu, vv);
    x = (int)floorf((uu * 0.5f + 0.5f) * (float)s); y = (int)floorf((vv * 0.5f + 0.5f) * (float)s);
    x = min(max(x, 0), s - 1); y = min(max(y, 0), s - 1);
  }
  const uint2 t = e.texels[(MIP0 ? 0u : e.mipOffset[mip]) + (uint32_t)face * (uint32_t)(s * s) + (uint32_t)(y * s + x)];
  return mk3(f16ToF32(t.x & 0xFFFFu), f16ToF32(t.x >> 16), f16ToF32(t.y & 0xFFFFu));
}
template <bool MIP0 = false>
RT_DEV f3 cubeBilinear(const EnvRef& e, uint32_t mip, int face, float u, float v) {
  const int s = (int)((e.size >> mip) ? (e.size >> mip) : 1u);
  const float x = (u * 0.5f + 0.5f) * (float)s - 0.5f, y = (v * 0.5f + 0.5f) * (float)s - 0.5f;
  const float x0 = floorf(x), y0 = floorf(y);
  const float fx = x - x0, fy = y - y0;
  const int ix = (int)x0, iy = (int)y0;
  const float w00 = (1.0f - fx) * (1.0f - fy), w10 = fx * (1.0f - fy), w01 = (1.0f - fx) * fy, w11 = fx * fy;
  const f3 c00 = cubeTexel<MIP0>(e, mip, face, ix, iy), c10 = cubeTexel<MIP0>(e, mip, face, ix + 1, iy);
  const f3 c01 = cubeTexel<MIP0>(e, mip, face, ix, iy + 1), c11 = cubeTexel<MIP0>(e, mip, face, ix + 1, iy + 1);
  return ((c00 * w00 + c10 * w10) + c01 * w01) + c11 * w11;
}
RT_DEV f3 environmentLevel0(const EnvRef& e, f3 dir) {
  int face; float u, v; cubeFaceUV(dir, face, u, v);
  return cubeBilinear<true>(e, 0u, face, u, v);
}
__device__ __noinline__ f3 environment(EnvRef e, f3 dir, float level) {
// ... 199 lines not shown
  for (uint32_t k = 0; k < 4u; ++k) {
    const uint32_t r = waveRays[0][k], d = waveRays[1][k];
    if (k < wave) { baseR += r; baseD += d; }
    nR += r; nD += d;
  }
  RayRec* dst = A.rays + (size_t)bin * A.binSlots;
  HitKey* keys = A.hits + (size_t)bin * A.binSlots;
  if (wantRefl) { const uint32_t k = baseR + (uint32_t)__popcll(maskR & below); dst[k] = rr; keys[k] = hitKey(RT_RAY_TMAX, 0xFFFFFFFFu); }
  const uint32_t kD = nR + baseD + (uint32_t)__popcll(maskD & below);
  if (wantDiff && kD < A.binSlots) { dst[kD] = rd; keys[kD] = hitKey(RT_RAY_TMAX, 0xFFFFFFFFu); }
  if (threadIdx.x != 0) return;
  const uint32_t nRaysInBin = min(nR + nD, A.binSlots);
  uint32_t mark = 0u;
  if (A.binWork != nullptr) {
    const uint32_t w = A.binWork[bin];
    A.binWork[bin] = 0u;
    uint32_t shift = 0u;
    while (shift < A.splitMaxShift && (w >> shift) > A.splitWork) ++shift;
    const uint32_t n = (shift || w > A.frontWork) ? 1u << shift : 0u;
    if (n) {
      const uint32_t base = atomicAdd(A.splitCount, n);
      const bool fits = base + n <= A.splitCap;
      for (uint32_t k = 0; k < n && base + k < A.splitCap; ++k) A.splitList[base + k] = fits ? ((shift << 28) | (k << 24) | bin) : 0xFFFFFFFFu;
      mark = fits ? (shift << 1) | 1u : 0u;
    }
  }
  A.binCount[bin] = nRaysInBin | (mark << 8);
}
template <int RATE, bool WIDE = false>
__global__ void __launch_bounds__(256, RT_GEN_MIN_BLOCKS) rayGenKernel(const FrameParams* __restrict__ fpp, GenArgs A) {
  const FrameParams& fp = *fpp;
  if (blockIdx.x == 0) A.frameRays[threadIdx.x] = 0u;
  if (blockIdx.x == 0 && threadIdx.x == 0 && A.visNext != nullptr) { *A.zeroNext0 = 0u; *A.zeroNext1 = 0u; }
  uint32_t tile = blockIdx.x;
  if constexpr (RATE == 4) {
    const uint32_t superX = (A.tilesX + 1u) >> 1, sup = blockIdx.x >> 2;
    const uint32_t tx = (sup % superX) * 2u + (blockIdx.x & 1u), ty = (sup / superX) * 2u + ((blockIdx.x >> 1) & 1u);
    tile = ty * A.tilesX + tx;
    if (tx >= A.tilesX || tile >= A.numTiles) {
      if (threadIdx.x == 0) { A.binCount[blockIdx.x] = 0u; if (A.binWork != nullptr) A.binWork[blockIdx.x] = 0u; }
      return;
    }
  }
  const uint32_t wave = threadIdx.x >> 6, lane = threadIdx.x & 63u;
  const uint32_t px = (tile % A.tilesX) * 16 + (wave & 1u) * 8 + (lane & 7u);
  const uint32_t py = A.rowBegin + (tile / A.tilesX) * 16 + (wave >> 1) * 8 + (lane >> 3);
  const bool inside = px < fp.W && py < A.rowEnd;
  const bool traced = RATE == 1 || quadTraced(px, py, fp.g.FrameIndex);
  uint32_t wordHere, wordNext, skyWord;
  asm volatile("s_load_dword %0, %3, %6\n\ts_load_dword %1, %4, %6\n\ts_load_dword %2, %5, %6\n\ts_waitcnt lgkmcnt(0)"
               : "=&s"(wordHere), "=&s"(wordNext), "=&s"(skyWord) : "s"(A.visDirty), "s"(A.visDirtyNext), "s"(A.skyPrev), "s"(tile * 4u) : "memory");
  const bool drawn = wordHere != 0u;
  const bool clearNext = A.visNext != nullptr && wordNext != 0u;
  const uint32_t skyPrevRun = (skyWord >> 8) == A.skyEpoch ? skyWord & 0xFFu : 0u;
  const uint32_t skyWordOut = (A.skyEpoch << 8) | (drawn || RATE != 1 ? 0u : min(skyPrevRun + 1u, RT_SKY_RUN_CAP));
  if (RATE == 1 && !drawn && !clearNext && skyPrevRun >= A.skyPrevRun) {
    if (threadIdx.x == 0) A.skyOut[tile] = skyWordOut;
    return;
  }
  const EnvRef env{A.env, A.envSize, A.envMips, A.envMipOffset};
  bool wantRefl = false, wantDiff = false;
  RayRec rr, rd;
  if (inside) {
    const uint32_t W = fp.W, H = fp.H;
    const size_t pix = (size_t)py * W + px;
    const unsigned long long visWord = drawn ? A.visDepth[pix] : RT_VIS_CLEAR;
    if (clearNext) A.visNext[pix] = RT_VIS_CLEAR;
    float xiY = 0.0f, cosPhi = 0.0f, sinPhi = 0.0f;
    if constexpr (WIDE) { if (drawn) sampleParamWide(fp, A.cosSin, py * W + px, xiY, cosPhi, sinPhi); }
    else if (drawn) {
      uint32_t s = py * W + px;
      s = rng(s); s += fp.g.FrameIndex; s = rng(s); s %= 256u;
      xiY = (float)(rng(s) & 0xffffu) / 65536.0f;
      cosPhi = A.cosSin[s]; sinPhi = A.cosSin[256 + s];
    }
    uint32_t visibility = (uint32_t)visWord;
    A.depthOut[pix] = (uint32_t)(visWord >> 32);
    f2 screenPos; screenPos.x = ((float)px + 0.5f) / (float)W * 2.0f - 1.0f; screenPos.y = ((float)py + 0.5f) / (float)H * 2.0f - 1.0f;
    screenPos.y = -screenPos.y;
    const f3 eye = mk3(fp.rg.EyePt[0], fp.rg.EyePt[1], fp.rg.EyePt[2]);
    bool hit; f3 N, V, P, color; f2 rghMtl, velocity; uint32_t inst = 0, prim = 0;
    if (visibility > 0) {
      --visibility;
      hit = true; inst = visibility >> 24; prim = visibility & 0xFFFFFFu;
      asm volatile("" : "+v"(prim));
      const Tri3 v = getVertices(inst ? A.fat1 : A.fat0, prim);
      const M4 wvp = cbLoad4x4(fp.g.WorldViewProjs[inst]);
      f4 p[3];
      for (int k = 0; k < 3; ++k) p[k] = mulPoint(v.pos[k], wvp);
      screenPos.x -= fp.rg.ProjBias[0]; screenPos.y -= fp.rg.ProjBias[1];
      const f2 bary = calcBarycentrics(p, screenPos);
      const Attrib a = interpAttrib(v, bary.x, bary.y);
      color = mk3(fp.mat.BaseColors[inst][0], fp.mat.BaseColors[inst][1], fp.mat.BaseColors[inst][2]);
      rghMtl = getRoughMetal(fp.mat, inst, a.UV);
      const f4 hPrev = mulPoint(a.Pos, cbLoad4x4(fp.g.WorldViewProjsPrev[inst]));
      velocity.x = (screenPos.x - hPrev.x / hPrev.w) * 0.5f; velocity.y = (screenPos.y - hPrev.y / hPrev.w) * -0.5f;
      const f4 P4 = mulPoint(a.Pos, cbLoad4x3(fp.g.Worlds[inst]));
      P = mk3(P4.x, P4.y, P4.z);
      N = normalize3(mulDir(a.Nrm, cbLoad3x3(inst ? fp.g.WorldIT1 : fp.g.WorldITs0)));
      V = normalize3(eye - P);
    } else {
      f4 sp4; sp4.x = screenPos.x; sp4.y = screenPos.y; sp4.z = 0.0f; sp4.w = 1.0f;
      const f4 world = mulVec4(sp4, cbLoad4x4(fp.rg.ProjToWorld));
      hit = false; velocity.x = 0.0f; velocity.y = 0.0f;
      P = mk3(world.x / world.w, world.y / world.w, world.z / world.w);
      N = mk3(0.0f, 0.0f, 0.0f);
      V = normalize3(eye - P);
      rghMtl.x = 0.0f; rghMtl.y = 0.0f;
// ... 46 lines not shown
        if (traced) {
          const float cosTheta = 1.0f - 2.0f * xiY;
          const float sinTheta = sqrtf(1.0f - cosTheta * cosTheta);
          const f3 dir = normalize3(N + mk3(cosPhi * sinTheta, sinPhi * sinTheta, cosTheta));
          wantDiff = true;
          rd.ox = P.x; rd.oy = P.y; rd.oz = P.z;
          rd.dx = dir.x; rd.dy = dir.y; rd.dz = dir.z;
          rd.pixel = (uint32_t)pix; rd.skip = skip; rd.flags = 1u;
          rd.wx = color.x * (1.0f - 0.04f); rd.wy = color.y * (1.0f - 0.04f); rd.wz = color.z * (1.0f - 0.04f);
        }
      } else if (A.diffPrev != nullptr) A.diffOut[pix] = A.diffPrev[pix];
    }
  }
  if (threadIdx.x == 0) { A.skyOut[tile] = skyWordOut; if (clearNext) A.visDirtyNextOut[tile] = 0u; }
  if constexpr (RATE == 4) { rayGenQuadBin(A, wantRefl, wantDiff, rr, rd); return; }

  const uint32_t bin = blockIdx.x * 4u + wave;
  const unsigned long long maskR = __ballot(wantRefl), maskD = __ballot(wantDiff), below = (1ull << lane) - 1ull;
  const uint32_t nR = (uint32_t)__popcll(maskR);
  RayRec* dst = A.rays + (size_t)bin * A.binSlots;
  HitKey* keys = A.hits + (size_t)bin * A.binSlots;
  if (wantRefl) { const uint32_t k = (uint32_t)__popcll(maskR & below); dst[k] = rr; keys[k] = hitKey(RT_RAY_TMAX, 0xFFFFFFFFu); }
  const uint32_t kD = nR + (uint32_t)__popcll(maskD & below);
  if (wantDiff && kD < A.binSlots) { dst[kD] = rd; keys[kD] = hitKey(RT_RAY_TMAX, 0xFFFFFFFFu); }
  const uint32_t nRaysInBin = min(nR + (uint32_t)__popcll(maskD), A.binSlots);
  if (A.binWork == nullptr) {
    if (lane == 0) A.binCount[bin] = nRaysInBin;
    return;
  }
  __shared__ uint32_t want[4], listBase;
  uint32_t shift = 0u, n = 0u;
  if (lane == 0) {
    const uint32_t w = A.binWork[bin];
    A.binWork[bin] = 0u;
    while (shift < A.splitMaxShift && (w >> shift) > A.splitWork) ++shift;
    n = (shift || w > A.frontWork) ? 1u << shift : 0u;
    want[wave] = n;
  }
  __syncthreads();
  if (threadIdx.x == 0) { const uint32_t total = want[0] + want[1] + want[2] + want[3]; listBase = total ? atomicAdd(A.splitCount, total) : 0u; }
  __syncthreads();
  if (lane == 0) {
    uint32_t base = listBase, mark = 0u;
    for (uint32_t k = 0; k < wave; ++k) base += want[k];
    if (n) {
      const bool fits = base + n <= A.splitCap;
      for (uint32_t k = 0; k < n && base + k < A.splitCap; ++k) A.splitList[base + k] = fits ? ((shift << 28) | (k << 24) | bin) : 0xFFFFFFFFu;
      mark = fits ? (shift << 1) | 1u : 0u;
    }
    A.binCount[bin] = nRaysInBin | (mark << 8);
  }
}

struct ShadeArgs {
  const RayRec* rays; const HitKey* hits; const uint32_t* binCount; uint32_t binSlots;
  const float4* fat0; const float4* fat1;
  const uint2* env; const uint32_t* envMipOffset; uint32_t envSize, envMips;
  const float* sh;
  uint32_t* reflOut; uint32_t* diffOut;
  const uint32_t* diffPrev; const unsigned long long* visDepth; uint32_t tilesX, rowBegin, rowEnd, carryMask;
  const uint32_t* tileWords;
  RayRec* spawnRays; HitKey* spawnHits; uint32_t* spawnCount; const float* cosSin;
  float* accRefl; float* accDiff;
};

enum ShadePass { SHADE_FINAL = 0, SHADE_SPAWN = 1, SHADE_FINAL_DEEP = 2, SHADE_ACCUM = 3, SHADE_SPAWN_ACCUM = 4 };
constexpr bool shadeSpawns(int pass) { return pass == SHADE_SPAWN || pass == SHADE_SPAWN_ACCUM; }
constexpr bool shadeAccumulates(int pass) { return pass == SHADE_ACCUM || pass == SHADE_SPAWN_ACCUM; }

RT_DEV f3 reflectionDepth1(const EnvRef& env, f2 rghMtl, f3 N, f3 V, f3 color) {
  const float level = calcMipFromRoughness(rghMtl.x, (float)env.mips);
  const float a = rghMtl.x * rghMtl.x;
  const f3 R = reflect3(-V, N);
  const f3 dir = lerp3(N, R, (1.0f - a) * (sqrtf(1.0f - a) + a));
  const float NoL = dot3(N, dir);
  if (NoL <= 0.0f) return mk3(0.0f, 0.0f, 0.0f);
  const f3 e = environment(env, dir, level);
  const f3 f0 = mk3(lerpf(0.04f, color.x, rghMtl.y), lerpf(0.04f, color.y, rghMtl.y), lerpf(0.04f, color.z, rghMtl.y));
  const float NoV = saturatef(dot3(N, V));
  return e * envBRDFApprox(f0, rghMtl.x, NoV);
}

RT_DEV uint32_t quadTileWord(const uint32_t* words, uint32_t tile32, uint32_t tilesX, uint32_t tilesY) {
  const uint32_t superX = (tilesX + 1u) >> 1, tx = (tile32 % superX) * 2u, ty = (tile32 / superX) * 2u;
  const uint32_t i0 = ty * tilesX + tx;
  const bool right = tx + 1u < tilesX, down = ty + 1u < tilesY;
  const uint32_t i1 = right ? i0 + 1u : i0, i2 = down ? i0 + tilesX : i0, i3 = right && down ? i0 + tilesX + 1u : i0;
  uint32_t a, b, c, d;
  asm volatile("s_load_dword %0, %4, %5\n\ts_load_dword %1, %4, %6\n\ts_load_dword %2, %4, %7\n\ts_load_dword %3, %4, %8\n\ts_waitcnt lgkmcnt(0)"
               : "=&s"(a), "=&s"(b), "=&s"(c), "=&s"(d)
               : "s"(words), "s"(RT_SGPR(i0 * 4u)), "s"(RT_SGPR(i1 * 4u)), "s"(RT_SGPR(i2 * 4u)), "s"(RT_SGPR(i3 * 4u)) : "memory");
  return a | b | c | d;
}
template <int RATE, int PASS, bool WIDE = false>
__global__ void __launch_bounds__(256, RT_GEN_MIN_BLOCKS) shadeKernel(const FrameParams* __restrict__ fpp, ShadeArgs A) {
  const FrameParams& fp = *fpp;
  const EnvRef env{A.env, A.envSize, A.envMips, A.envMipOffset};
  const uint32_t tile = blockIdx.x;
  { uint32_t word;
    if constexpr (RATE == 1) asm volatile("s_load_dword %0, %1, %2\n\ts_waitcnt lgkmcnt(0)" : "=s"(word) : "s"(A.tileWords), "s"(tile * 4u) : "memory");
    else word = quadTileWord(A.tileWords, tile, A.tilesX, (A.rowEnd - A.rowBegin + 15u) / 16u);
    if (word == 0u) return; }
  const uint32_t bin = tile * 4u + (threadIdx.x >> 6);
  if (RATE == 1 && A.carryMask != 0u) {
    const uint32_t lane = threadIdx.x & 63u, wave = threadIdx.x >> 6;
    const uint32_t px = (tile % A.tilesX) * 16u + (wave & 1u) * 8u + (lane & 7u);
    const uint32_t py = A.rowBegin + (tile / A.tilesX) * 16u + (wave >> 1) * 8u + (lane >> 3);
    if (px < fp.W && py < A.rowEnd) {
      const size_t pix = (size_t)py * fp.W + px;
      const uint32_t vis = (uint32_t)A.visDepth[pix];
      if (vis != 0u && ((A.carryMask >> ((vis - 1u) >> 24)) & 1u)) A.diffOut[pix] = A.diffPrev[pix];
    }
  }
  const uint32_t count = min(A.binCount[bin] & 0xFFu, A.binSlots);
  uint32_t spawned = 0u;
  for (uint32_t i = threadIdx.x & 63u; i < count; i += 64u) {
    const size_t slot = (size_t)bin * A.binSlots + i;
    const float4* rp = reinterpret_cast<const float4*>(A.rays + slot);
    const float4 q0 = rp[0], q1 = rp[1], q2 = rp[2];
    const float4 ra = make_float4(q0.x, q0.y, q0.z, RT_RAY_TMIN), rb = make_float4(q0.w, q1.x, q1.y, RT_RAY_TMAX), rw = make_float4(q2.x, q2.y, q2.z, 0.0f);
    const uint4 rc = make_uint4(__float_as_uint(q1.z), __float_as_uint(q1.w), __float_as_uint(q2.w), 0u);
    const uint32_t hitId = hitKeyId(A.hits[slot]);
    const f3 dir = mk3(rb.x, rb.y, rb.z);
    const bool diffuseGroup = (rc.z & 1u) != 0u;
    const uint32_t srcInst = rc.y >> 24;
    f3 col;
    bool child = false; RayRec cr;
    if (hitId == 0xFFFFFFFFu) col = environmentLevel0(env, dir);
    else {
      const float m = fp.mat.RoughMetals[srcInst][1];
      const f3 preset = mk3(fp.mat.BaseColors[srcInst][0] * m, fp.mat.BaseColors[srcInst][1] * m, fp.mat.BaseColors[srcInst][2] * m);
      if (!diffuseGroup && preset.x <= 0.0f && preset.y <= 0.0f && preset.z <= 0.0f) col = preset;
      else {
        const uint32_t hInst = hitId >> 24;
        uint32_t hPrim = hitId & 0xFFFFFFu;
        asm volatile("" : "+v"(hPrim));
        const Tri3 v = getVertices(hInst ? A.fat1 : A.fat0, hPrim);
        float ht, hb1 = 0.0f, hb2 = 0.0f;
        woopTestVerts(toObject(ra.x, ra.y, ra.z, rb.x, rb.y, rb.z, hInst ? fp.invWorld[1] : fp.invWorld[0]), v.pos[0], v.pos[1], v.pos[2], ht, hb1, hb2);
        const Attrib a = interpAttrib(v, hb1, hb2);
        const f3 N = normalize3(mulDir(a.Nrm, cbLoad3x3(hInst ? fp.g.WorldIT1 : fp.g.WorldITs0)));
        const f2 rm = getRoughMetal(fp.mat, hInst, a.UV);
        f3 color = mk3(fp.mat.BaseColors[hInst][0], fp.mat.BaseColors[hInst][1], fp.mat.BaseColors[hInst][2]);
        const f3 V = -dir;
        if constexpr (!shadeSpawns(PASS)) {
          if (rm.y > 0.5f) col = reflectionDepth1(env, rm, N, V, color);
          else {
            if (diffuseGroup) color = color * (1.0f - rm.y);
            const f3 irr = evaluateSHIrradiance(A.sh, N);
            col = mk3(irr.x / RT_PI, irr.y / RT_PI, irr.z / RT_PI) * color;
          }
        } else {
          const f3 P = mk3(ra.x + ht * rb.x, ra.y + ht * rb.y, ra.z + ht * rb.z);
          float xiY, cosPhi, sinPhi;
          if constexpr (WIDE) sampleParamWide(fp, A.cosSin, rc.x, xiY, cosPhi, sinPhi);
          else {
            uint32_t s = rng(rc.x); s += fp.g.FrameIndex; s = rng(s); s %= 256u;
            xiY = (float)(rng(s) & 0xffffu) / 65536.0f; cosPhi = A.cosSin[s]; sinPhi = A.cosSin[256 + s];
          }
          const uint32_t toDiffImage = (rc.z ^ (rc.z >> 1)) & 1u;
          f3 w, L;
          if (rm.y > 0.5f) {
            const bool vndf = (fp.flags & RT_FLAG_VNDF) != 0u;
            const f3 Hh = reflectionHalfVector(vndf, N, V, rm.x * rm.x, cosPhi, sinPhi, xiY);
            L = reflect3(-V, Hh);
            const float NoL = dot3(N, L);
            if (NoL <= 0.0f) col = mk3(0.0f, 0.0f, 0.0f);
            else { w = reflectionWeight(vndf, N, V, Hh, NoL, rm, color); child = true; cr.flags = toDiffImage << 1; }
          } else {
            if (diffuseGroup) color = color * (1.0f - rm.y);
            L = diffuseDirection(N, cosPhi, sinPhi, xiY);
            w = color; child = true; cr.flags = 1u | ((toDiffImage ^ 1u) << 1);
          }
          if (child) {
            cr.ox = P.x; cr.oy = P.y; cr.oz = P.z; cr.dx = L.x; cr.dy = L.y; cr.dz = L.z;
            cr.pixel = rc.x; cr.skip = hitId;
            cr.wx = rw.x * w.x; cr.wy = rw.y * w.y; cr.wz = rw.z * w.z;
          }
        }
      }
    }
    if constexpr (shadeSpawns(PASS)) {
      const unsigned long long mask = __ballot(child);
      if (child) {
        const size_t k = (size_t)bin * A.binSlots + spawned + (uint32_t)__popcll(mask & ((1ull << (threadIdx.x & 63u)) - 1ull));
        A.spawnRays[k] = cr; A.spawnHits[k] = hitKey(RT_RAY_TMAX, 0xFFFFFFFFu);
      }
      spawned += (uint32_t)__popcll(mask);
      if (child) continue;
    }
    if constexpr (shadeAccumulates(PASS)) {
      float* acc = (((rc.z ^ (rc.z >> 1)) & 1u) != 0u ? A.accDiff : A.accRefl) + 3u * (size_t)rc.x;
      acc[0] = acc[0] + col.x * rw.x; acc[1] = acc[1] + col.y * rw.y; acc[2] = acc[2] + col.z * rw.z;
      continue;
    }
    const uint32_t packed = packR11G11B10F(mk3(col.x * rw.x, col.y * rw.y, col.z * rw.z));
    const bool toDiff = PASS == SHADE_FINAL ? diffuseGroup : ((rc.z ^ (rc.z >> 1)) & 1u) != 0u;
    if (toDiff) A.diffOut[rc.x] = packed; else A.reflOut[rc.x] = packed;
  }
  if constexpr (shadeSpawns(PASS)) { if ((threadIdx.x & 63u) == 0u) A.spawnCount[bin] = spawned; }
}

struct ReconArgs {
  const unsigned long long* visDepth; const uint32_t* normal; const uint16_t* roughMetal; const uint32_t* depth32;
  uint32_t* reflOut; uint32_t* diffOut;
  const uint32_t* diffPrev; uint32_t carryMask, diffMask;
  const uint32_t* tileWords; uint32_t tilesX, rowBegin, rowEnd;
};
struct ReconTexel { float nx, ny, nz, depth, rough; };
RT_DEV ReconTexel reconTexel(const ReconArgs& A, size_t i) {
  const uint32_t n = A.normal[i];
  ReconTexel t;
  t.nx = (float)(2 * (int)(n & 1023u) - 1023); t.ny = (float)(2 * (int)((n >> 10) & 1023u) - 1023); t.nz = (float)(2 * (int)((n >> 20) & 1023u) - 1023);
  t.depth = (float)A.depth32[i] * (1.0f / 16777215.0f);
  t.rough = (float)(A.roughMetal[i] & 0xFFu) * (1.0f / 255.0f);
  return t;
}
RT_DEV float reconNormalDepthWeight(const ReconTexel& c, const ReconTexel& q) {
  const float I = (c.nx * q.nx + c.ny * q.ny) + c.nz * q.nz;
  float x = fmaxf(I * (1.0f / 1046529.0f), 0.0f);
  x = x * x; x = x * x; x = x * x; x = x * x; x = x * x;
  return x * (float)exp((double)(-fabsf(c.depth - q.depth) * c.depth * 4.0f));
}
RT_DEV f3 reconDivide(f3 s, float w) {
  const double d = (double)w;
  return mk3((float)((double)s.x / d), (float)((double)s.y / d), (float)((double)s.z / d));
}
__global__ void __launch_bounds__(256) reconstructKernel(const FrameParams* __restrict__ fpp, ReconArgs A) {
  const FrameParams& fp = *fpp;
  const uint32_t tile = blockIdx.x;
  { uint32_t word;
    asm volatile("s_load_dword %0, %1, %2\n\ts_waitcnt lgkmcnt(0)" : "=s"(word) : "s"(A.tileWords), "s"(tile * 4u) : "memory");
    if (word == 0u) return; }
  const uint32_t W = fp.W;
  const uint32_t px = (tile % A.tilesX) * 16u + (threadIdx.x & 15u), py = A.rowBegin + (tile / A.tilesX) * 16u + (threadIdx.x >> 4);
  if (px >= W || py >= A.rowEnd) return;
  const size_t pix = (size_t)py * W + px;
  const uint32_t vis = (uint32_t)A.visDepth[pix];
  if (vis == 0u) return;
  const uint32_t inst = (vis - 1u) >> 24;
  if ((A.carryMask >> inst) & 1u) A.diffOut[pix] = A.diffPrev[pix];
  const uint32_t f = fp.g.FrameIndex & 3u, ox = (0x6u >> f) & 1u, oy = (0xAu >> f) & 1u;
  if ((px & 1u) == ox && (py & 1u) == oy) return;
  const bool diffuse = ((A.diffMask >> inst) & 1u) != 0u;
  const ReconTexel c = reconTexel(A, pix);
  f3 sumR = mk3(0.0f, 0.0f, 0.0f), sumD = sumR, meanR = sumR, meanD = sumR;
  float wR = 0.0f, wD = 0.0f;
  uint32_t n = 0u;
  for (int dy = -1; dy <= 1; ++dy)
    for (int dx = -1; dx <= 1; ++dx) {
      const int qx = (int)px + dx, qy = (int)py + dy;
      if (qx < 0 || qy < 0 || qx >= (int)W || qy >= (int)fp.H || ((uint32_t)qx & 1u) != ox || ((uint32_t)qy & 1u) != oy) continue;
      const size_t q = (size_t)qy * W + (uint32_t)qx;
// ... 163 lines not shown
  now.tilesX = (fp.W + 15u) / 16u; now.tilesY = (re - rb + 15u) / 16u;
  memcpy(now.camera, fp.rg.ProjToWorld, 64); memcpy(now.camera + 16, fp.rg.EyePt, 16);
  const rtggx_context::SkyGen& was = c->skyGen;
  bool same = was.any && (was.frame == now.frame || was.frame + 1u == now.frame) && was.rows[0] == rb && was.rows[1] == re && was.rate == now.rate
              && was.adaptive == adaptive && was.sliceShift == sliceShift && was.stream == sGen;
#ifndef RT_SKY_NO_CAMERA_CHECK
  same = same && memcmp(was.camera, now.camera, sizeof now.camera) == 0;
#endif
  if (!same) c->breakSkyRuns();
  now.epoch = c->skyEpoch;
  c->skyGen = now;
  return now.epoch;
}

int launchRayTrace(rtggx_context* c, const FrameParams& fp, hipStream_t sGen, hipStream_t s, hipEvent_t done) {
  uint32_t rb, re;
  passRows(fp, ROWS_GBUFFER, rb, re);
  if (re <= rb) return 0;
  const uint32_t tilesX = (fp.W + 15) / 16, tilesY = (re - rb + 15) / 16;
  const bool quad = c->rayRate == 4u;
  const uint32_t quadX = (tilesX + 1u) / 2u, quadY = (tilesY + 1u) / 2u;
  if ((fp.mat.RoughMetals[0][1] < 1.0f || fp.mat.RoughMetals[1][1] < 1.0f) && c->binSlots < RT_BIN) {
    setError("rtggx_ray_trace: a material with metallic below 1 (a diffuse ray per pixel as well) but ray bins of %u slots: rtggx_update_frame sizes them", c->binSlots); return -1;
  }
  GenArgs G;
  const InputSet& set = c->cur();
  { const uint32_t thenFrame = c->frameCounter + 2u;
    VisTarget& vn = c->visOf(thenFrame);
    G.visNext = vn.depth; G.zeroNext0 = c->largeCountBase + (thenFrame & 1u); G.zeroNext1 = c->next().splitCount;
    vn.cleared.frame = thenFrame; vn.cleared.rows[0] = rb; vn.cleared.rows[1] = re;
    if (c->traceShare > 0.93f) c->traversalBound = true; else if (c->traceShare < 0.89f) c->traversalBound = false;
    G.visDirty = c->tileWords(rb, re); c->traceTileWords = quad ? c->visDirtyOnes : G.visDirty;
    G.visDirtyNextOut = vn.dirty;
    G.visDirtyNext = c->useTileWords && !c->traversalBound && vn.flags.rows[0] == rb && vn.flags.rows[1] == re ? vn.dirty : c->visDirtyOnes;
    vn.flags.rows[0] = rb; vn.flags.rows[1] = re;
  }
  G.visDepth = c->curVis().depth; G.depthOut = set.depth32; G.normalOut = set.normal; G.roughMetalOut = set.roughMetal; G.velocityOut = set.velocity; G.reflOut = set.rtRefl; G.diffOut = set.rtDiff;
  G.roughMetalPrev = c->prev().roughMetal;
  G.diffPrev = c->genCarriesDiff ? c->prev().rtDiff : nullptr;
  G.fat0 = c->mesh[0].fat; G.fat1 = c->mesh[1].fat;
  G.env = c->env.texels; G.envMipOffset = c->dEnvMipOffset; G.envSize = c->env.size; G.envMips = c->env.mips; G.cosSin = c->sampleTable();
  G.rays = (RayRec*)set.rayQueue.get(); G.hits = (HitKey*)set.hitQueue.get(); G.binCount = set.binCount; G.binSlots = c->binSlots; G.frameRays = c->rayCounter32;
  G.tilesX = tilesX; G.numTiles = tilesX * tilesY; G.rowBegin = rb; G.rowEnd = re;
  const uint32_t splitWork = c->splitWork, splitMaxShift = c->splitMaxShift;
  const uint32_t numBins = quad ? quadX * quadY * 4u : G.numTiles * 4u;
  const uint32_t sliceShift = chooseSliceShift(c, true, numBins);
  c->lastTraceSmall = c->forcePlacement >= 0 ? c->forcePlacement == 1 : (sliceShift > 0u || c->lastFrameRays < RT_WIDE_RAYS);
  const bool adaptive = splitWork != 0u && sliceShift == 0u;
  const uint32_t splitCap = !adaptive ? 0u : c->splitCapForced != 0xFFFFFFFFu ? c->splitCapForced
                          : c->splitDemand == 0u ? 0u : ((c->splitDemand + c->splitDemand / 8u + 64u + 31u) / 32u) * 32u;
  G.binWork = adaptive ? c->binWork : nullptr; G.splitList = set.splitList; G.splitCount = set.splitCount;
  G.frontWork = RT_SPLIT_FRONT < splitWork ? RT_SPLIT_FRONT : splitWork;
  G.splitWork = splitWork; G.splitMaxShift = splitMaxShift < 3u ? splitMaxShift : 3u; G.splitCap = splitCap < RT_SPLIT_CAP ? splitCap : RT_SPLIT_CAP;
  G.skyEpoch = skyEpochForGen(c, fp, rb, re, sGen, adaptive, sliceShift);
  if (c->skyEpochWrapped) {
    RT_HIP(hipDeviceSynchronize());
    for (auto& st : c->sets) RT_HIP(hipMemset(st.skyRun, 0, c->skyTiles * 4));
    { const int r = resetSettled(c); if (r) return r; }
    RT_HIP(hipStreamSynchronize(nullptr));
    c->skyEpochWrapped = false;
  }
  G.skyPrev = c->prev().skyRun; G.skyOut = set.skyRun; G.skyPrevRun = c->staticSky ? RT_SKY_PREV_RUN : RT_SKY_RUN_CAP + 1u;
  FrameEvents& ev = c->frameEvents(c->frameCounter);
  const FrameParams* genParams = c->dParams + c->slot;
  if (c->samples > 1u) {
    FrameParams* const sp = c->sppParams + (size_t)c->slot * RTGGX_MAX_SAMPLES_PER_PIXEL;
    hipLaunchKernelGGL(sampleParamsKernel, dim3(1), dim3(256), 0, sGen, genParams, sp, c->samples);
    genParams = sp;
  }
  const bool wide = c->sampleSet > RTGGX_MIN_SAMPLE_SET;
  launch(wide ? (quad ? rayGenKernel<4, true> : rayGenKernel<1, true>) : quad ? rayGenKernel<4> : rayGenKernel<1>, dim3(quad ? numBins : G.numTiles), dim3(256), sGen, nullptr, sGen != s ? ev.gen : nullptr, genParams, G);
  ev.genFrame = 0u; ev.genStream = sGen;
  if (sGen != s) {
    RT_HIP(hipStreamWaitEvent(s, ev.gen, 0));
    ev.genFrame = c->frameCounter;
  }
  if (c->timing) hipEventRecord(c->tev[11], s);
  const bool ring = c->kernelRing && c->kevCount < c->kevBegin.size() && (c->ringTick++ % c->ringStride) == 0u;
  const TraceQueue q{G.rays, G.hits, G.binCount};
  c->traceGrid[0] = numBins; c->traceGrid[1] = quad ? quadX : tilesX; c->traceGrid[2] = quad ? quadY : tilesY; c->traceGrid[3] = sliceShift;
  { const int r = launchTrace(c, fp, s, q, numBins, true, quad ? quadX : tilesX, quad ? quadY : tilesY, sliceShift, adaptive ? (int)G.splitCap : -1,
                              ring ? c->kevBegin[c->kevCount] : nullptr, ring ? c->kevEnd[c->kevCount] : done); if (r) return r; }
  if (c->timing) hipEventRecord(c->tev[12], s);
  if (ring) ++c->kevCount;
  if (done && ring) hipEventRecord(done, s);
  RT_HIP(hipGetLastError());
  return 0;
}

static void (*const kShade[3][2])(const FrameParams*, ShadeArgs) = {
    {shadeKernel<1, SHADE_FINAL>, shadeKernel<4, SHADE_FINAL>}, {shadeKernel<1, SHADE_SPAWN>, shadeKernel<4, SHADE_SPAWN>},
    {shadeKernel<1, SHADE_FINAL_DEEP>, shadeKernel<4, SHADE_FINAL_DEEP>}};
static void (*const kShadeSpawnWide[2])(const FrameParams*, ShadeArgs) = {shadeKernel<1, SHADE_SPAWN, true>, shadeKernel<4, SHADE_SPAWN, true>};
static int launchShadeSamples(rtggx_context* c, const FrameParams& fp, hipStream_t s, hipEvent_t done, ShadeArgs S, uint32_t numTiles, int spillPart) {
  const uint32_t N = c->samples, depth = c->maxDepth;
  const bool wide = c->sampleSet > RTGGX_MIN_SAMPLE_SET;
  if (!c->sppAcc || !c->sppParams) { setError("rtggx_ray_trace: %u samples per pixel without their buffers", N); return -1; }
  if (c->sppStream && c->sppStream != s) { RT_HIP(hipEventRecord(c->evSpp, c->sppStream)); RT_HIP(hipStreamWaitEvent(s, c->evSpp, 0)); }
  c->sppStream = s;
  const InputSet& set = c->cur();
  const FrameParams* const sp = c->sppParams + (size_t)c->slot * RTGGX_MAX_SAMPLES_PER_PIXEL;
  S.accRefl = c->sppAcc; S.accDiff = c->sppAcc + 3u * (size_t)c->W * c->H;
  SampleGenArgs G;
  G.visDepth = S.visDepth; G.fat0 = S.fat0; G.fat1 = S.fat1; G.cosSin = S.cosSin;
  G.rays = S.spawnRays; G.hits = S.spawnHits; G.binCount = S.spawnCount; G.binSlots = S.binSlots;
  G.tileWords = S.tileWords; G.tilesX = S.tilesX; G.rowBegin = S.rowBegin; G.rowEnd = S.rowEnd;
  const uint32_t* const map = c->sampleMapWords();
  if (map && (S.rowBegin != 0u || S.rowEnd != c->H)) { setError("rtggx_ray_trace: a sample map on rows [%u,%u) of %u", S.rowBegin, S.rowEnd, c->H); return -1; }
  SampleGenArgsMapped GM;
  static_cast<SampleGenArgs&>(GM) = G; GM.sampleMap = map; GM.sample = 0u;
  const TraceQueue q{S.rays, S.spawnHits, S.binCount};
  for (uint32_t k = 0; k < N; ++k) {
    for (uint32_t level = 0; level < depth; ++level) {
      if (k > 0 && level == 0) {
        if (map) { GM.sample = k; launch(wide ? sampleGenKernel<true, true> : sampleGenKernel<false, true>, dim3(numTiles), dim3(256), s, nullptr, nullptr, sp + k, GM); }
        else launch(wide ? sampleGenKernel<true> : sampleGenKernel<false>, dim3(numTiles), dim3(256), s, nullptr, nullptr, sp + k, G);
      }
      if (k > 0 || level > 0) {
        const int r = launchTrace(c, fp, s, q, c->traceGrid[0], true, c->traceGrid[1], c->traceGrid[2], c->traceGrid[3], -1, nullptr, nullptr, spillPart);
        if (r) return r;
      }
      launch(level + 1u < depth ? (wide ? shadeKernel<1, SHADE_SPAWN_ACCUM, true> : shadeKernel<1, SHADE_SPAWN_ACCUM>) : shadeKernel<1, SHADE_ACCUM>, dim3(numTiles), dim3(256), s, nullptr, nullptr, sp + k, S);
      S.carryMask = 0u;
      RT_HIP(hipGetLastError());
    }
  }
  ResolveArgs R;
  R.visDepth = S.visDepth; R.accRefl = S.accRefl; R.accDiff = S.accDiff; R.reflOut = set.rtRefl; R.diffOut = set.rtDiff;
  R.tileWords = S.tileWords; R.tilesX = S.tilesX; R.rowBegin = S.rowBegin; R.rowEnd = S.rowEnd;
  R.diffMask = (fp.mat.RoughMetals[0][1] < 1.0f ? 1u : 0u) | (fp.mat.RoughMetals[1][1] < 1.0f ? 2u : 0u);
  R.scale = 1.0f / (float)N;
  if (map) {
    ResolveArgsMapped RM;
    static_cast<ResolveArgs&>(RM) = R; RM.sampleMap = reinterpret_cast<const uint8_t*>(map); RM.samples = N;
    launch(resolveSamplesKernel<true>, dim3(numTiles), dim3(256), s, nullptr, done, c->dParams + c->slot, RM);
  } else launch(resolveSamplesKernel<false>, dim3(numTiles), dim3(256), s, nullptr, done, c->dParams + c->slot, R);
  RT_HIP(hipGetLastError());
  return 0;
}
int launchShade(rtggx_context* c, const FrameParams& fp, hipStream_t s, hipEvent_t done) {
  uint32_t rb, re;
  passRows(fp, ROWS_GBUFFER, rb, re);
  if (re <= rb) return 0;
  const uint32_t tilesX = (fp.W + 15) / 16, numTiles = tilesX * ((re - rb + 15) / 16);
  const InputSet& set = c->cur();
  ShadeArgs S;
  S.diffPrev = c->prev().rtDiff; S.visDepth = c->curVis().depth; S.tilesX = tilesX; S.rowBegin = rb; S.rowEnd = re;
  S.carryMask = (fp.mat.RoughMetals[0][1] >= 1.0f ? 1u : 0u) | (fp.mat.RoughMetals[1][1] >= 1.0f ? 2u : 0u);
  if (c->genCarriesDiff) S.carryMask = 0u;
  S.tileWords = c->tileWords(rb, re);
  const bool quad = c->rayRate == 4u;
  const uint32_t grid = quad ? ((tilesX + 1u) / 2u) * ((re - rb + 31u) / 32u) : numTiles;
  if (quad) S.carryMask = 0u;
  S.rays = (const RayRec*)set.rayQueue.get(); S.hits = (const HitKey*)set.hitQueue.get(); S.binCount = set.binCount; S.binSlots = c->binSlots;
  S.fat0 = c->mesh[0].fat; S.fat1 = c->mesh[1].fat;
  S.env = c->env.texels; S.envMipOffset = c->dEnvMipOffset; S.envSize = c->env.size; S.envMips = c->env.mips; S.sh = c->sh;
  S.reflOut = set.rtRefl; S.diffOut = set.rtDiff;
  S.spawnRays = (RayRec*)set.rayQueue.get(); S.spawnHits = (HitKey*)set.hitQueue.get(); S.spawnCount = set.binCount; S.cosSin = c->sampleTable();
  S.accRefl = nullptr; S.accDiff = nullptr;
  const FrameParams* const dfp = c->dParams + c->slot;
  const uint32_t depth = c->maxDepth;
  const int spillPart = s == c->streamMain ? 2 : (int)c->traceSpillHalf;
  if (c->samples > 1u && !quad) return launchShadeSamples(c, fp, s, done, S, numTiles, spillPart);
  for (uint32_t level = 0; level < depth; ++level) {
    if (level > 0) {
      const TraceQueue q{S.rays, S.spawnHits, S.binCount};
      const int r = launchTrace(c, fp, s, q, c->traceGrid[0], true, c->traceGrid[1], c->traceGrid[2], c->traceGrid[3], -1, nullptr, nullptr, spillPart);
      if (r) return r;
      S.carryMask = 0u;
    }
    const int pass = level + 1u < depth ? SHADE_SPAWN : level == 0 ? SHADE_FINAL : SHADE_FINAL_DEEP;
    launch(pass == SHADE_SPAWN && c->sampleSet > RTGGX_MIN_SAMPLE_SET ? kShadeSpawnWide[quad] : kShade[pass][quad], dim3(grid), dim3(256), s, nullptr, pass == SHADE_SPAWN ? nullptr : done, dfp, S);
    RT_HIP(hipGetLastError());
  }
  return 0;
}

int launchReconstruct(rtggx_context* c, const FrameParams& fp, hipStream_t s) {
  uint32_t rb, re;
  passRows(fp, ROWS_GBUFFER, rb, re);
  if (re <= rb) return 0;
  const uint32_t tilesX = (fp.W + 15) / 16, numTiles = tilesX * ((re - rb + 15) / 16);
  const InputSet& set = c->cur();
  ReconArgs R;
  R.visDepth = c->curVis().depth; R.normal = set.normal; R.roughMetal = set.roughMetal; R.depth32 = set.depth32;
  R.reflOut = set.rtRefl; R.diffOut = set.rtDiff;
  R.diffPrev = c->prev().rtDiff;
  const uint32_t metal = (fp.mat.RoughMetals[0][1] >= 1.0f ? 1u : 0u) | (fp.mat.RoughMetals[1][1] >= 1.0f ? 2u : 0u);
  R.carryMask = c->genCarriesDiff ? 0u : metal; R.diffMask = ~metal & 3u;
  R.tileWords = c->tileWords(rb, re); R.tilesX = tilesX; R.rowBegin = rb; R.rowEnd = re;
  hipLaunchKernelGGL(reconstructKernel, dim3(numTiles), dim3(256), 0, s, c->dParams + c->slot, R);
  RT_HIP(hipGetLastError());
  return 0;
}

__global__ void fillTestQueue(const float* __restrict__ rays, uint32_t n, uint32_t binSlots, RayRec* q0, HitKey* keys, uint32_t* binCount, float2* tRange) {
  const uint32_t i = blockIdx.x * blockDim.x + threadIdx.x;
  if (i % binSlots == 0 && i < n) binCount[i / binSlots] = n - i < binSlots ? n - i : binSlots;
  if (i >= n) return;
  const float* r = rays + 8 * (size_t)i;
  RayRec rr;
  rr.ox = r[0]; rr.oy = r[1]; rr.oz = r[2]; rr.dx = r[3]; rr.dy = r[4]; rr.dz = r[5];
  rr.pixel = 0u; rr.skip = 0xFFFFFFFFu; rr.flags = 0u; rr.wx = rr.wy = rr.wz = 0.0f;
  q0[i] = rr;
  tRange[i] = make_float2(r[6], r[7]);
  keys[i] = hitKey(r[7], 0xFFFFFFFFu);
}
__global__ void exportTestHits(const FrameParams* __restrict__ fpp, const RayRec* __restrict__ rays, const HitKey* __restrict__ hits, uint32_t n,
                               const float4* __restrict__ fat0, const float4* __restrict__ fat1, float* __restrict__ out) {
  const uint32_t i = blockIdx.x * blockDim.x + threadIdx.x;
  if (i >= n) return;
  const HitKey k = hits[i];
  const uint32_t id = hitKeyId(k);
  float* o = out + 6 * (size_t)i;
  const bool valid = id != 0xFFFFFFFFu;
  float t = hitKeyT(k), b1 = 0.0f, b2 = 0.0f;
  if (valid) {
    const RayRec rr = rays[i];
    const uint32_t inst = id >> 24;
    uint32_t prim = id & 0xFFFFFFu;
    asm volatile("" : "+v"(prim));
    const Tri3 v = getVertices(inst ? fat1 : fat0, prim);
    woopTestVerts(toObject(rr.ox, rr.oy, rr.oz, rr.dx, rr.dy, rr.dz, inst ? fpp->invWorld[1] : fpp->invWorld[0]), v.pos[0], v.pos[1], v.pos[2], t, b1, b2);
  }
  o[0] = t; o[1] = u2f(valid ? id >> 24 : 0u); o[2] = u2f(valid ? id & 0xFFFFFFu : 0u); o[3] = b1; o[4] = b2; o[5] = valid ? 1.0f : 0.0f;
// ... 84 lines not shown
```

raytracedggx_amd/csrc/rtggx_context.h:

```cpp
#pragma once
#include <hip/hip_runtime.h>
#include <hip/hip_ext.h>
#include <stdint.h>
#include <stdlib.h>
#include <string>
#include <utility>
#include <vector>
#include <memory>
#include "rtggx_device.h"
#include "rt_owned_hip.h"

#ifndef RT_SETS
#define RT_SETS 4
#endif
#define RT_SLOTS (RT_SETS + 1)
#define RT_VIS_RING (RT_SETS + 2)
#define RT_VIS_CLEAR 0x00FFFFFF00000000ull
#define RT_SKY_PREV_RUN (RT_SETS + 2)
#define RT_SKY_V_RUN 2u
#define RT_SKY_WINDOW_RUN 1u
#define RT_SETTLED 1u
#define RT_SETTLED_SKIPPED 2u
#define RT_SETTLED_BORDER 0xFFFFFFFFu
#define RT_SKY_RUN_CAP 255u
// ... 41 lines not shown
  BvhTopo topo;
  std::unique_ptr<struct BuildJob> job;
  bool wantRebuild = false;
  uint32_t topoVersion = 0, topoVersionOfSet[RT_SETS] = {};
  DevBuf<float> dCost;
  PinnedBuf<float> hCost;
  Event evCost; bool costInFlight = false;
  float builtCost = 0.0f, lastCost = 0.0f;
  uint32_t refits = 0, rebuilds = 0;
  DevBuf<uint32_t> indices;
  uint32_t numVerts = 0, numIndices = 0, numTris = 0;
  BvhNode* nodes = nullptr;
  Bvh4Node* nodes4 = nullptr;
  BvhTri* tris = nullptr;
  DevBuf<BvhNode> nodesOwn[RT_SETS]; DevBuf<Bvh4Node> nodes4Own[RT_SETS]; DevBuf<BvhTri> trisOwn[RT_SETS];
  BvhNode* nodesBuf[RT_SETS] = {}; Bvh4Node* nodes4Buf[RT_SETS] = {}; BvhTri* trisBuf[RT_SETS] = {};
  uint32_t topCount = 0; uint32_t topCountBuf[RT_SETS] = {};
  Bvh4Node* top = nullptr; DevBuf<Bvh4Node> topOwn[RT_SETS]; Bvh4Node* topBuf[RT_SETS] = {};
  int32_t root = -1;
  uint32_t depth = 0;
  uint32_t stack4 = 0;
  float bmin[3] = {0, 0, 0}, bmax[3] = {0, 0, 0};
};

struct EnvDev {
  DevBuf<uint2> texels;
  uint32_t size = 0, mips = 0;
  uint32_t mipOffset[16] = {};
  uint64_t totalTexels = 0;
};

struct FrameParams {
  RtggxCBGlobal g;
  RtggxRayGenConstants rg;
  RtggxCBPerObject po[2];
  RtggxCBMaterial mat;
  float invWorld[2][16];
  uint32_t W, H;
  uint32_t rowBegin, rowEnd;
  uint32_t flags;
  uint32_t sampleMask;
  uint32_t pad[2];
};
#define RT_FLAG_VNDF 1u

struct InputSet {
  DevBuf<uint32_t> normal, velocity, rtRefl, rtDiff;
  DevBuf<uint16_t> roughMetal;
  DevBuf<uint32_t> depth32;
  DevBuf<void> rayQueue, hitQueue;
  DevBuf<uint32_t> binCount;
  DevBuf<uint32_t> splitList; uint32_t* splitCount = nullptr;
  DevBuf<uint32_t> skyRun;
  Event evRead;
  bool readRecorded = false;
};

struct VisTarget {
  DevBuf<unsigned long long> depth;
  DevBuf<uint32_t> dirty;
  struct { uint32_t frame = 0, rows[2] = {0, 0}; } cleared;
  struct { uint32_t rows[2] = {0, 0}; uint32_t rasterFrame = 0; } flags;
};

struct FrameEvents {
  Event gen;
  uint32_t genFrame = 0;
  hipStream_t genStream = nullptr;
  Event trace;
  bool traceRecorded = false;
};

}

#ifndef RT_COLLAPSE_AREA_WEIGHT
#define RT_COLLAPSE_AREA_WEIGHT 1.0f
#define RT_COLLAPSE_TRIS_WEIGHT 0.0f
#endif
#define RT_MAX_PEERS 16

struct rtggx_context {
  int device = 0;
  uint32_t W = 0, H = 0;
  uint32_t rowBegin = 0, rowEnd = 0;
  uint32_t historyApron = 18;
  rt::DevBuf<uint32_t> histReach;
  rt::Stream ownMain; hipStream_t streamMain = nullptr, streamAS = nullptr;
  rt::Stream streamRefit;
  bool refitIssued = false;
  uint32_t frameCounter = 0;
  rt::FrameEvents frames[4];
  rt::FrameEvents& frameEvents(uint32_t f) { return frames[f & 3u]; }
  rt::Stream ownAS, ownVis;
  bool asyncCompute = true;
  hipStream_t streamVis = nullptr;
  rt::Event evVis;
  hipStream_t evVisStream = nullptr;
  rt::Event evAS;
  rt::Event evRefit;
  rt::Event evRT;
  int setReadDeferred = -1;
  double fenceWaitUs = 0.0; uint32_t fenceWaits = 0;
  int fuseToneMap = -1; bool toneMapDone = false, denoiseIssued = false;
  rt::DevBuf<uint32_t> exchangeTokens;
  float collapseWeights[2] = {RT_COLLAPSE_AREA_WEIGHT, RT_COLLAPSE_TRIS_WEIGHT};
  uint32_t peerWorld = 0; rt::DevBuf<void> dPeerTable; std::vector<rt::IpcMapping> ipcMapped;
// ... 20 lines not shown
  rt::DevBuf<RtggxScore> scoreRing;
  uint64_t scoreIndex = 0, scoreRead = 0;
  uint32_t traceGrid[4] = {};
  float rebuildRatio = 1.2f; uint32_t rebuildSteps = 16;
  rt::MeshDev mesh[2];
  rt::EnvDev env;
  rt::DevBuf<float> sh;
  rt::DevBuf<float> cosSinTab;
  uint32_t sampleSet = RTGGX_MIN_SAMPLE_SET, sampleSetRequested = RTGGX_MIN_SAMPLE_SET;
  rt::DevBuf<float> cosSinWide[8];
  static uint32_t sampleSetSlot(uint32_t m) { uint32_t k = 0; while ((512u << k) < m) ++k; return k; }
  const float* sampleTable() const { return sampleSet > RTGGX_MIN_SAMPLE_SET ? cosSinWide[sampleSetSlot(sampleSet)] : cosSinTab; }

  rt::InputSet sets[RT_SETS];
  uint32_t setIndex = 0;
  uint32_t setAhead(uint32_t k) const { return (setIndex + k) % RT_SETS; }
  rt::InputSet& cur() { return sets[setIndex]; }
  rt::InputSet& prev() { return sets[setAhead(RT_SETS - 1u)]; }
  rt::InputSet& next() { return sets[setAhead(1u)]; }
  rt::VisTarget vis[RT_VIS_RING];
  rt::VisTarget& visOf(uint32_t frame) { return vis[frame % RT_VIS_RING]; }
  rt::VisTarget& curVis() { return visOf(frameCounter); }
  void selectSet(uint32_t i) {
    setIndex = i;
    largeTris = largeTrisBuf[frameCounter & 1u]; largeCount = largeCountBase ? largeCountBase + (frameCounter & 1u) : nullptr;
    for (auto& m : mesh) { m.verts = m.vertsBuf[i]; m.fat = m.fatBuf[i]; m.nodes = m.nodesBuf[i]; m.nodes4 = m.nodes4Buf[i]; m.top = m.topBuf[i]; m.topCount = m.topCountBuf[i]; m.tris = m.trisBuf[i]; }
    binWork = binWorkBuf[frameCounter & 1u]; rayCounter32 = rayCounterBuf + (frameCounter & 3u) * 256u;
  }
  rt::DevBuf<uint32_t> backbuffer;
  rt::DevBuf<uint2> tss[2], fltRfl, fltDff;
  uint32_t frameParity = 0;

  void* largeTris = nullptr; rt::DevBuf<void> largeTrisBuf[2];
  uint32_t* largeCount = nullptr;
  rt::DevBuf<uint32_t> largeCountBase;
  uint32_t* binWork = nullptr;
  rt::DevBuf<uint32_t> binWorkBuf[2];
  const uint32_t* tileWords(uint32_t rb, uint32_t re) {
    const rt::VisTarget& v = curVis();
    return useTileWords && !traversalBound && v.flags.rasterFrame == frameCounter && v.flags.rows[0] == rb && v.flags.rows[1] == re ? v.dirty.get() : visDirtyOnes.get();
  }
  bool staticSky = true;
  uint32_t skyEpoch = 1u; bool skyEpochWrapped = false; size_t skyTiles = 0;
  void breakSkyRuns() { skyEpoch = (skyEpoch + 1u) & 0xFFFFFFu; if (skyEpoch == 0u) skyEpochWrapped = true; }
  struct SkyGen { bool any = false, adaptive = false; uint32_t frame = 0, epoch = 0, rows[2] = {0, 0}, rate = 0, sliceShift = 0, tilesX = 0, tilesY = 0; hipStream_t stream = nullptr; float camera[20] = {}; } skyGen;
  struct SkyV { bool any = false, fltRflNull = false; uint32_t frame = 0, genEpoch = 0, rows[2] = {0, 0}; } skyV;
  bool settledSky = true;
  rt::DevBuf<uint32_t> settled[2]; uint32_t settledX = 0, settledY = 0, settledPitch = 0;
  size_t settledWords() const { return (size_t)(settledX + 2u) * settledPitch + 8u; }
  struct SkyT { bool any = false, words = false; uint32_t frame = 0, epoch = 0, parity = 0, rows[2] = {0, 0}; } skyT;
  struct SkyTM { bool any = false, fromTss = false; uint32_t frame = 0, epoch = 0, parity = 0, writes = 0, rows[2] = {0, 0}; } skyTM;
  uint32_t tssWrites[2] = {0, 0};
  bool useTileWords = true;
  bool traversalBound = false;
  const uint32_t* traceTileWords = nullptr;
  rt::DevBuf<uint32_t> visDirtyOnes;
  uint32_t splitDemand = 0;
  uint32_t splitCapForced = 0xFFFFFFFFu;
  uint32_t splitWork = 0, splitMaxShift = 0;
  uint32_t largeCapacity = 0;

  uint32_t numBinsMax = 0, binSlots = 64;
  rt::DevBuf<void> testRayRange; void* traceRayRange = nullptr;
  rt::DevBuf<int32_t> stackOverflow;
  uint32_t spillEntries = 0;
  rt::DevBuf<void> dummyRecord;
  rt::DevBuf<uint32_t> dEnvMipOffset;
  bool lastTraceSmall = false; uint32_t traceSpillHalf = 0;
  hipStream_t shadeStream = nullptr;
  bool genCarriesDiff = false, shadeWroteDiff = false, lastFrameDiffuse = false;
  hipStream_t diffStream = nullptr;
  uint32_t numCUs = 256;
  uint32_t traceWaves = 12, traceWavesForced = 0; float traceShare = 0.0f; rt::DevBuf<unsigned long long> traceStamps; uint32_t traceStampLaunch = 0;
  unsigned long long traceStampSum = 0, traceStampStart = 0; uint32_t traceStampAt = 0, traceSampleLaunch = 0;
  uint32_t traceTrial = 0, traceCooldown = 0, traceWavesSince = 0; float traceTrialBase = 0.0f;

  rt::PinnedBuf<uint32_t> hostRayCounters;
  rt::Event evRayCounters; bool rayCountersInFlight = false; uint32_t traceLaunches = 0;
  uint32_t lastFrameRays = 0xFFFFFFFFu;
  uint32_t* rayCounter32 = nullptr;
  rt::DevBuf<uint32_t> rayCounterBuf;
  uint32_t* lastRayCounter32 = nullptr;
  rt::DevBuf<unsigned long long> rayCounter;

  rt::FrameParams slots[RT_SLOTS];
  uint32_t slot = 0;
  rt::DevBuf<rt::FrameParams> dParams;
  bool slotUploaded = false;
  bool slotRendered = false;
  RtggxCBMaterial material;
  float invWorld[2][16];
  bool haveConstants = false, asBuilt = false, shDone = false;

  bool timing = false;
  bool kernelRing = false;
  uint32_t ringStride = 1, ringTick = 0;
  std::vector<rt::Event> kevBegin, kevEnd;
  uint32_t kevCount = 0;
  rt::Event tev[16];
  bool timingsPending = false;
};

namespace rt {
enum RowPass { ROWS_GBUFFER , ROWS_VFILTER , ROWS_TEMPORAL , ROWS_FINAL };
inline void passRows(const FrameParams& fp, RowPass pass, uint32_t& b, uint32_t& e) {
  const uint32_t apron = pass == ROWS_GBUFFER ? 18u : pass == ROWS_VFILTER ? 2u : pass == ROWS_TEMPORAL ? 1u : 0u;
  b = fp.rowBegin > apron ? fp.rowBegin - apron : 0u;
  e = fp.rowEnd + apron < fp.H ? fp.rowEnd + apron : fp.H;
  if (fp.rowEnd <= fp.rowBegin) { b = e = 0; }
}
void setError(const char* fmt, ...);
#define RT_HIP(expr) do { hipError_t _e = (expr); if (_e != hipSuccess) { rt::setError("%s failed: %s (%s:%d)", #expr, hipGetErrorString(_e), __FILE__, __LINE__); return -2; } } while (0)
template <class... P, class... A>
inline void launch(void (*k)(P...), dim3 grid, dim3 block, hipStream_t s, hipEvent_t start, hipEvent_t stop, A&&... a) {
  if (start || stop) hipExtLaunchKernelGGL(k, grid, block, 0, s, start, stop, 0, static_cast<P>(a)...);
  else hipLaunchKernelGGL(k, grid, block, 0, s, static_cast<P>(a)...);
}

int uploadParams(rtggx_context* c, uint32_t slot, hipStream_t s);
int launchVisibility(rtggx_context* c, const FrameParams& fp, hipStream_t s, hipEvent_t done = nullptr);
int buildLbvh(rtggx_context* c, uint32_t slot, hipStream_t s);
int startRebuild(rtggx_context* c, uint32_t slot, uint32_t set);
int continueRebuild(rtggx_context* c, uint32_t slot, hipStream_t s, uint32_t maxSteps, bool* swapped);
int prepareRebuild(rtggx_context* c, uint32_t slot);
void abandonRebuild(rtggx_context* c, uint32_t slot);
int refitLbvh(rtggx_context* c, uint32_t slot, uint32_t set, hipStream_t s);
void freeBuildProducts(MeshDev& m);
int buildFatTris(rtggx_context* c, uint32_t slot, uint32_t set, hipStream_t s);
int launchRayTrace(rtggx_context* c, const FrameParams& fp, hipStream_t sGen, hipStream_t sTrace, hipEvent_t done = nullptr);
int launchShade(rtggx_context* c, const FrameParams& fp, hipStream_t s, hipEvent_t done = nullptr);
int launchReconstruct(rtggx_context* c, const FrameParams& fp, hipStream_t s);
int allocSamples(rtggx_context* c);
int allocAccumulation(rtggx_context* c);
int launchAccumulate(rtggx_context* c, const FrameParams& fp, hipStream_t s);
int launchPresentAccumulation(rtggx_context* c, hipStream_t s);
#define RT_SCORE_CHUNK 1024u
#define RT_SCORE_SUMS 9u
int launchScore(rtggx_context* c, const FrameParams& fp, hipStream_t s);
int launchReferenceFromAccumulation(rtggx_context* c, hipStream_t s);
int launchTraceRays(rtggx_context* c, const FrameParams& fp, const float* dRays, uint32_t n, float* dOut, hipStream_t s);
int launchDebugEnvironment(rtggx_context* c, const float* dDirs, const float* dLevels, uint32_t n, int level0, float* dOut, hipStream_t s);
int resetSettled(rtggx_context* c);
int launchDenoise(rtggx_context* c, const FrameParams& fp, int useLds, hipStream_t s, hipEvent_t done = nullptr, bool fuseToneMap = false);
int launchToneMap(rtggx_context* c, const FrameParams& fp, hipStream_t s, hipEvent_t done = nullptr, const uint2* source = nullptr);
int decodeEnv(rtggx_context* c, int format, uint32_t size, uint32_t mips, const void* hostData, size_t bytes, hipStream_t s);
int buildEnvFromImage(rtggx_context* c, int layout, int pixels, uint32_t width, uint32_t height, const void* hostData, uint32_t size, hipStream_t s);
int generateEnvMips(rtggx_context* c, hipStream_t s);
int projectSH(rtggx_context* c, hipStream_t s);
int unpackVisDepth(rtggx_context* c, uint32_t* dVis, uint32_t* dDepth, hipStream_t s);
int packVisDepth(rtggx_context* c, const uint32_t* dVis, const uint32_t* dDepth, hipStream_t s);
}
```

raytracedggx_amd/csrc/trace.hip:

```cpp
#include <type_traits>
#include "rt_queue.h"
#include "rt_traverse.h"

namespace rt {

#define RT_PRIME_LAUNCHES 4u
#ifndef RT_STACK
#define RT_STACK 16
#endif

struct TraceArgs {
  const float4* nodes0; const float4* tris0;
  const float4* nodes1; const float4* tris1;
  int32_t root0, root1;
  uint32_t haveMesh0, haveMesh1;
  const RayRec* rays; HitKey* hits;
  const float2* tRange;
  const uint32_t* binCount; uint32_t numBins, binSlots;
  int32_t* overflow;
  uint32_t* rayTotals;
  uint32_t* stats;
  unsigned long long* runTotals;
  uint32_t countRowBegin, countRowEnd, width;
  size_t spillStride;
// ... 278 lines not shown
    if (A.launch != 0u && prev[0] != 0ull && prev[1] > prev[0]) A.stamps[6] += prev[1] - prev[0];
    A.stamps[7] = now;
    mine[0] = now; next[0] = 0ull; next[1] = 0ull;
  }
  __syncthreads();
  const uint32_t xcd = blockIdx.x & 7u, groupsPerXcd = gridDim.x >> 3;
  for (;;) {
    uint32_t j = 0;
    if ((threadIdx.x & 63u) == 0u) j = atomicAdd(&lds.next, 1u);
    j = (uint32_t)__builtin_amdgcn_readfirstlane((int)j);
    const uint32_t item = ((blockIdx.x >> 3) + j * groupsPerXcd) * 8u + xcd;
    if (j >= 0x1000000u || item >= A.totalItems) break;
    traceItem<TOP>(*fpp, A, (LdsInt*)lds.stack, (LdsUint*)lds.victims, (const LdsFloat4*)lds.top, item, blockIdx.x * (uint32_t)WAVES + (threadIdx.x >> 6));
  }
  if ((threadIdx.x & 63u) == 0u && A.stamps != nullptr && atomicAdd(&lds.done, 1u) == (uint32_t)WAVES - 1u) atomicMax(A.stamps + 2u * (A.launch % 3u) + 1u, wall_clock64());
}

#ifdef RT_TRACE_STATS
__global__ void stampKernel(uint32_t* stats) { *reinterpret_cast<unsigned long long*>(stats + 764) = wall_clock64(); }
#endif

#define RT_WAVES_TRY 0.90f
#define RT_WAVES_SHRINK 0.70f
#define RT_WAVES_RETRY 16u
static void steerTraceWaves(rtggx_context* c, const unsigned long long* stamps, uint32_t launch) {
  const unsigned long long sum = stamps[0], start = stamps[1];
  const unsigned long long dSum = sum - c->traceStampSum, dStart = start - c->traceStampStart;
  const uint32_t launches = launch - c->traceStampAt, windowBegin = c->traceStampAt;
  const bool usable = c->traceStampStart != 0ull && start > c->traceStampStart && sum >= c->traceStampSum && dSum <= dStart && launches >= 8u && launches <= 64u;
  c->traceStampSum = sum; c->traceStampStart = start; c->traceStampAt = launch;
  if (!usable) { c->traceTrial = 0u; return; }
  const float period = (float)dStart / (float)launches;
  c->traceShare = (float)dSum / (float)dStart;
  static const bool log = getenv("RTGGX_TRACE_LOG") != nullptr;
  if (log) fprintf(stderr, "[rtggx] trace sample at launch %u: %u launches, period %.1f us, share %.3f, waves %u, trial %u (base %.1f us), cooldown %u\n", launch, launches, period * 0.01f, c->traceShare, c->traceWaves, c->traceTrial, c->traceTrialBase * 0.01f, c->traceCooldown);
  if (c->traceWavesForced || c->lastTraceSmall) { c->traceTrial = 0u; return; }
  if (c->traceTrial != 0u) {
    if (++c->traceTrial == 2u) return;
    if (period < 0.97f * c->traceTrialBase) c->traceCooldown = 8u;
    else { c->traceWaves -= 2u; c->traceWavesSince = launch; c->traceCooldown = RT_WAVES_RETRY; }
    c->traceTrial = 0u;
    return;
  }
  if (c->traceCooldown) --c->traceCooldown;
  const bool clean = windowBegin >= c->traceWavesSince + 8u;
  if (c->traceShare < RT_WAVES_SHRINK && c->traceWaves > 12u) { c->traceWaves -= 2u; c->traceWavesSince = launch; if (c->traceCooldown < 4u) c->traceCooldown = 4u; }
  else if (c->traceShare > RT_WAVES_TRY && c->traceWaves < 16u && c->traceCooldown == 0u && clean) { c->traceTrialBase = period; c->traceWaves += 2u; c->traceWavesSince = launch; c->traceTrial = 1u; }
}

uint32_t chooseSliceShift(rtggx_context* c, bool countRays, uint32_t numBins) {
  if (countRays && c->rayCountersInFlight && hipEventQuery(c->evRayCounters) == hipSuccess) {
    uint32_t sum = 0; for (int i = 0; i < 256; ++i) sum += c->hostRayCounters[i];
    c->lastFrameRays = sum; c->splitDemand = c->hostRayCounters[256]; c->rayCountersInFlight = false;
    steerTraceWaves(c, reinterpret_cast<const unsigned long long*>(c->hostRayCounters + 258), c->traceSampleLaunch);
  }
  const uint32_t raysGuess = countRays ? c->lastFrameRays : numBins * 40u;
  return raysGuess < 25000u ? 3u : raysGuess < 60000u ? 2u : raysGuess < 110000u ? 1u : 0u;
}

int launchTrace(rtggx_context* c, const FrameParams& fp, hipStream_t s, const TraceQueue& q, uint32_t numBins, bool countRays, uint32_t tilesX, uint32_t tilesY, uint32_t sliceShift,
                int splitCap, hipEvent_t start, hipEvent_t stop, int spillPart) {
  const bool deeper = spillPart >= 0;
  TraceArgs T;
  if (numBins == 0) return 0;
  if (numBins > c->numBinsMax) { setError("launchTrace: %u bins exceed the %u allocated", numBins, c->numBinsMax); return -1; }
  const bool have0 = c->mesh[0].tris != nullptr, have1 = c->mesh[1].tris != nullptr;
  T.nodes0 = (const float4*)(have0 && c->mesh[0].nodes4 ? (const void*)c->mesh[0].nodes4 : c->dummyRecord);
  T.tris0 = (const float4*)(have0 ? (const void*)c->mesh[0].tris : c->dummyRecord);
  T.nodes1 = (const float4*)(have1 && c->mesh[1].nodes4 ? (const void*)c->mesh[1].nodes4 : c->dummyRecord);
  T.tris1 = (const float4*)(have1 ? (const void*)c->mesh[1].tris : c->dummyRecord);
  T.root0 = c->mesh[0].root; T.root1 = c->mesh[1].root; T.haveMesh0 = have0; T.haveMesh1 = have1;
  T.rays = q.rays; T.hits = q.hits; T.tRange = (const float2*)c->traceRayRange;
  T.binCount = q.binCount; T.numBins = numBins; T.binSlots = c->binSlots;
  const uint32_t deepest = (c->mesh[0].stack4 > c->mesh[1].stack4 ? c->mesh[0].stack4 : c->mesh[1].stack4) + 1u;
  if (deepest > RT_STACK + c->spillEntries) {
    RT_HIP(hipDeviceSynchronize());
    c->stackOverflow.reset();
    c->spillEntries = deepest - RT_STACK;
    RT_HIP(alloc(c->stackOverflow, (size_t)RT_SPILL_PARTS * c->spillEntries * RT_SPILL_WAVES * 64));
  }
  T.overflow = c->stackOverflow + (size_t)(deeper ? (uint32_t)spillPart : c->traceSpillHalf) * c->spillEntries * RT_SPILL_WAVES * 64;
  T.rayTotals = c->rayCounter32; T.stats = c->rayCounterBuf + 1024; T.runTotals = c->rayCounter + 256;
  T.spillStride = (size_t)RT_SPILL_WAVES * 64;
  T.countRowBegin = countRays ? fp.rowBegin : 0u; T.countRowEnd = countRays ? fp.rowEnd : 0u; T.width = fp.W;
#ifdef RT_TRACE_STATS
  hipLaunchKernelGGL(stampKernel, dim3(1), dim3(1), 0, s, c->rayCounterBuf + 1024);
#endif
  T.tilesX = tilesX; T.tilesY = tilesY; T.tileWords = tilesX ? c->traceTileWords : nullptr;
  T.sliceShift = sliceShift;
  const bool adaptive = splitCap >= 0 && sliceShift == 0u && tilesX != 0u;
  T.splitList = c->cur().splitList; T.splitCount = c->cur().splitCount;
  T.binWork = adaptive ? c->binWork : nullptr; T.splitBlocks = adaptive ? (uint32_t)splitCap / 4u : 0u;
  const uint32_t superTiles = ((tilesX + 7u) / 8u) * ((tilesY + 7u) / 8u);
  const uint32_t grid = T.splitBlocks + ((tilesX ? ((superTiles + 7u) / 8u) * 8u * 64u : (((numBins + 3u) / 4u + 7u) / 8u) * 8u) << T.sliceShift);
  T.totalItems = grid * 4u;
  T.top0 = (const float4*)c->mesh[0].top; T.topCount0 = have0 && c->mesh[0].top ? c->mesh[0].topCount : 0u;
  T.top1 = (const float4*)c->mesh[1].top; T.topCount1 = have1 && c->mesh[1].top ? c->mesh[1].topCount : 0u;
  if (T.topCount0 > RT_TOP_SLOT0 || T.topCount1 > RT_TOP_SLOT1) { setError("launchTrace: tree tables of %u / %u nodes exceed the LDS slots", T.topCount0, T.topCount1); return -1; }
  static const int forced = getenv("RTGGX_TRACE_WAVES") ? atoi(getenv("RTGGX_TRACE_WAVES")) : 0;
  const uint32_t waves = forced ? (uint32_t)forced : (!countRays || c->lastFrameRays < RT_TINY_RAYS) ? 1u : c->traceWaves;
  const uint32_t perCu = waves == 1u ? RT_SPILL_WAVES / 256u : 1u;
  if (waves == 1u) T.topCount0 = T.topCount1 = 0u;
  T.stamps = waves == 1u || deeper ? nullptr : c->traceStamps; T.launch = deeper ? 0u : c->traceStampLaunch++;
  const uint32_t wanted = (T.totalItems + waves - 1u) / waves;
  uint32_t blocks = c->numCUs * perCu < wanted ? c->numCUs * perCu : wanted;
  blocks = (blocks + 7u) & ~7u;
  if (blocks * waves > RT_SPILL_WAVES) blocks = (RT_SPILL_WAVES / waves) & ~7u;
  void (*kernel)(const FrameParams*, TraceArgs);
  switch (waves) {
    case 1u: kernel = traceKernel<1, 5, 0>; break;
    case 10u: kernel = traceKernel<10, 4, 1>; break;
    case 12u: kernel = traceKernel<12, 4, 1>; break;
    case 14u: kernel = traceKernel<14, 4, 1>; break;
    case 16u: kernel = traceKernel<16, 4, 1>; break;
    default: setError("launchTrace: no kernel variant with %u waves", waves); return -1;
  }
  launch(kernel, dim3(blocks), dim3(64 * waves), s, start, stop, c->dParams + c->slot, T);
  const uint32_t counterMask = 15u;
  if (countRays && !deeper && !c->rayCountersInFlight && (c->traceLaunches < 8u || (c->traceLaunches & counterMask) == 0u)) {
    RT_HIP(hipMemcpyAsync(c->hostRayCounters, c->rayCounter32, 256 * 4, hipMemcpyDeviceToHost, s));
    RT_HIP(hipMemcpyAsync(c->hostRayCounters + 256, c->cur().splitCount, 4, hipMemcpyDeviceToHost, s));
    RT_HIP(hipMemcpyAsync(c->hostRayCounters + 258, c->traceStamps + 6, 16, hipMemcpyDeviceToHost, s)); c->traceSampleLaunch = c->traceLaunches;
    RT_HIP(hipEventRecord(c->evRayCounters, s));
    c->rayCountersInFlight = true;
    if (c->traceLaunches < RT_PRIME_LAUNCHES) RT_HIP(hipEventSynchronize(c->evRayCounters));
  }
  if (countRays && !deeper) ++c->traceLaunches;
  RT_HIP(hipGetLastError());
  return 0;
}

}
```

Before: 3312 Mrays/s.

## Compact active tile lists to drive shade and reflection filter passes

Adds a per-frame compaction pass that builds lists of non-empty tiles and blocks for shading and the horizontal and vertical reflection filters. Those kernels then launch persistent, list-driven grids sized from block counts read back asynchronously with the ray counters, so no blocks are spent on empty or sky regions. The grid size uses counts that lag by a frame, the list-generation kernel adds work of its own, and the persistent loop adds a barrier per entry.

```diff
diff --git a/include/rtggx.h b/include/rtggx.h
--- a/include/rtggx.h
+++ b/include/rtggx.h
@@ -73,7 +73,11 @@
   RTGGX_BUF_ACC_REFL = 25,
   RTGGX_BUF_ACC_DIFF = 26,
   RTGGX_BUF_CONVERGED = 27,
-  RTGGX_BUF_COUNT = 28
+  RTGGX_BUF_COUNT = 28,
+  RTGGX_BUF_LIST_SHADE = 64,
+  RTGGX_BUF_LIST_H = 65,
+  RTGGX_BUF_TILE_WORDS = 67,
+  RTGGX_BUF_LIST_V = 66
 };
 
 typedef struct RtggxTimings {
@@ -167,6 +171,8 @@
 int  rtggx_debug_static_sky(rtggx_context* ctx, int enable);
 int  rtggx_debug_sky_runs(rtggx_context* ctx, uint32_t* runs, uint32_t capacity, uint32_t* tiles_x, uint32_t* tiles_y, uint32_t* threshold);
 int  rtggx_debug_settled_sky(rtggx_context* ctx, int enable);
+int  rtggx_debug_block_lists(rtggx_context* ctx, int mode, uint32_t grid_cap);
+int  rtggx_debug_block_lists_used(rtggx_context* ctx, uint32_t* kernels, uint32_t* grids);
 int  rtggx_debug_settled_words(rtggx_context* ctx, uint32_t* words0, uint32_t* words1, uint32_t capacity, uint32_t* blocks_x, uint32_t* blocks_y, uint32_t* epoch);
 int  rtggx_debug_collapse_weights(rtggx_context* ctx, const float* set, float* get);
 int  rtggx_debug_fence_wait(rtggx_context* ctx, double* us_total, uint32_t* waits, int reset);
diff --git a/raytracedggx_amd/capi.py b/raytracedggx_amd/capi.py
--- a/raytracedggx_amd/capi.py
+++ b/raytracedggx_amd/capi.py
@@ -10,6 +10,7 @@
     BUF_FLT_RFL, BUF_FLT_DFF, BUF_BACKBUFFER, BUF_SH_COEFFS, BUF_BVH_NODES0, BUF_BVH_TRIS0, BUF_BVH_NODES1, BUF_BVH_TRIS1, \
     BUF_TLAS, BUF_ENV, BUF_BVH4_NODES0, BUF_BVH4_NODES1, BUF_BIN_WORK, BUF_BVH4_TOP0, BUF_BVH4_TOP1, BUF_EXCHANGE_TOKENS, \
     BUF_ACC_REFL, BUF_ACC_DIFF, BUF_CONVERGED = range(28)
+BUF_LIST_SHADE, BUF_LIST_H, BUF_LIST_V, BUF_TILE_WORDS = 64, 65, 66, 67
 MAX_PEERS, IPC_HANDLE_BYTES = 16, 64
 FORMAT_RGBA32F, FORMAT_RGBA16F, FORMAT_BC6H_UF16, FORMAT_BC6H_SF16 = 2, 10, 95, 96
 ENV_EQUIRECT, ENV_VCROSS, ENV_HCROSS = 0, 1, 2
@@ -21,7 +22,8 @@
               BUF_BVH_NODES0: np.uint32, BUF_BVH_TRIS0: np.uint32, BUF_BVH_NODES1: np.uint32, BUF_BVH_TRIS1: np.uint32,
               BUF_TLAS: np.float32, BUF_ENV: np.uint16, BUF_BVH4_NODES0: np.uint32, BUF_BVH4_NODES1: np.uint32, BUF_BIN_WORK: np.uint32,
               BUF_BVH4_TOP0: np.uint32, BUF_BVH4_TOP1: np.uint32, BUF_EXCHANGE_TOKENS: np.uint32,
-              BUF_ACC_REFL: np.float32, BUF_ACC_DIFF: np.float32, BUF_CONVERGED: np.uint64}
+              BUF_ACC_REFL: np.float32, BUF_ACC_DIFF: np.float32, BUF_CONVERGED: np.uint64,
+              BUF_LIST_SHADE: np.uint32, BUF_LIST_H: np.uint32, BUF_LIST_V: np.uint32, BUF_TILE_WORDS: np.uint32}
 
 EXPORTS = ["rtggx_last_error", "rtggx_create", "rtggx_destroy", "rtggx_set_strip", "rtggx_set_stream", "rtggx_set_mesh",
            "rtggx_set_env", "rtggx_set_material", "rtggx_set_metallic", "rtggx_build_as", "rtggx_update_frame", "rtggx_update_as",
@@ -31,7 +33,7 @@
            "rtggx_set_async_compute", "rtggx_set_history_apron", "rtggx_history_overreach", "rtggx_copy_bandwidth", "rtggx_refit_as", "rtggx_refit_as_device", "rtggx_refit_stats", "rtggx_set_refit_policy", "rtggx_set_sampler", "rtggx_set_ray_rate", "rtggx_set_max_recursion_depth", "rtggx_set_samples_per_pixel", "rtggx_debug_fuse_tone_map", "rtggx_debug_placement", "rtggx_debug_tile_words", "rtggx_debug_static_sky", "rtggx_debug_settled_sky", "rtggx_debug_settled_words", "rtggx_debug_sky_runs", "rtggx_debug_collapse_weights", "rtggx_debug_fence_wait", "rtggx_debug_shader_clock", "rtggx_debug_environment",
            "rtggx_set_accumulation", "rtggx_reset_accumulation", "rtggx_accumulated_frames", "rtggx_present_accumulation", "rtggx_set_sample_set",
            "rtggx_set_reference", "rtggx_reference_from_accumulation", "rtggx_set_scoring", "rtggx_read_scores",
-           "rtggx_set_env_image", "rtggx_generate_env_mips",
+           "rtggx_set_env_image", "rtggx_generate_env_mips", "rtggx_debug_block_lists", "rtggx_debug_block_lists_used",
            "rtggx_set_sample_map", "rtggx_read_sample_map"]
 SCORE_RING = 256
 
@@ -205,6 +207,20 @@
     def static_sky(self, enable):
         self._check(self.L.rtggx_debug_static_sky(self.h, 1 if enable else 0))
 
+    def block_lists(self, mode=1, grid_cap=0):
+        self.L.rtggx_debug_block_lists.argtypes = [C.c_void_p, C.c_int, C.c_uint32]
+        self._check(self.L.rtggx_debug_block_lists(self.h, int(mode), int(grid_cap)))
+
+    def block_lists_used(self):
+        k, g = C.c_uint32(), (C.c_uint32 * 3)()
+        self.L.rtggx_debug_block_lists_used.argtypes = [C.c_void_p, C.c_void_p, C.c_void_p]
+        self._check(self.L.rtggx_debug_block_lists_used(self.h, C.byref(k), g))
+        return {n: (int(g[i]) if (k.value >> i) & 1 else 0) for i, n in enumerate(("shade", "h", "v"))}
+
+    def block_list(self, bid):
+        words = self.readback(bid)
+        return words[1:1 + int(words[0])].copy()
+
     def sky_runs(self):
         tiles = ((self.W + 15) // 16) * ((self.H + 15) // 16 + 1)
         runs = np.zeros(tiles, np.uint32)
diff --git a/raytracedggx_amd/csrc/context.hip b/raytracedggx_amd/csrc/context.hip
--- a/raytracedggx_amd/csrc/context.hip
+++ b/raytracedggx_amd/csrc/context.hip
@@ -5,6 +5,7 @@
 #include <vector>
 #include "capi_internal.h"
 #include "rt_queue.h"
+#include "rt_blocklist.h"
 
 #ifndef RT_REFIT_REBUILD_RATIO
 #define RT_REFIT_REBUILD_RATIO 1.2f
@@ -46,6 +47,7 @@
   if (!s.binCount) RT_HIP(allocFilled(s.binCount, (size_t)c->numBinsMax));
   if (!s.splitList) RT_HIP(alloc(s.splitList, (size_t)RT_SPLIT_CAP));
   if (!s.skyRun) RT_HIP(allocFilled(s.skyRun, c->skyTiles));
+  if (!s.blockLists) RT_HIP(allocFilled(s.blockLists, (size_t)c->listWords));
   c->breakSkyRuns();
   s.splitCount = c->largeCountBase + 2 + i;
   if (!s.evRead) RT_HIP(create(s.evRead, RT_EVENT_FLAGS));
@@ -77,6 +79,9 @@
   c->binSlots = RT_BIN_MIN;
   c->largeCapacity = 1u << 16;
   c->skyTiles = (size_t)((width + 15) / 16) * ((height + 15) / 16 + 1);
+  { const BlockListLayout L = blockListLayout(width, height);
+    for (int k = 0; k < RT_LISTS; ++k) { c->listOff[k] = L.off[k]; c->listCap[k] = L.cap[k]; }
+    c->listWords = L.words; }
   for (auto& b : c->largeTrisBuf) RT_HIP(alloc(b, (size_t)c->largeCapacity * 56));
   RT_HIP(allocFilled(c->largeCountBase, 2 + RT_SETS));
   for (uint32_t i = 0; i < RT_SETS; ++i) { const int r = allocSet(c, i); if (r) return r; }
@@ -92,7 +97,7 @@
   RT_HIP(allocFilled(c->rayCounterBuf, 1792));
   c->lastRayCounter32 = c->rayCounterBuf;
   RT_HIP(allocFilled(c->traceStamps, 8));
-  RT_HIP(alloc(c->hostRayCounters, 264)); memset(c->hostRayCounters, 0, 264 * 4); RT_HIP(create(c->evRayCounters, hipEventDisableTiming));
+  RT_HIP(alloc(c->hostRayCounters, 272)); memset(c->hostRayCounters, 0, 272 * 4); RT_HIP(create(c->evRayCounters, hipEventDisableTiming));
   for (auto& b : c->binWorkBuf) RT_HIP(allocFilled(b, (size_t)c->numBinsMax));
   c->selectSet(0);
   c->splitWork = RT_SPLIT_WORK; c->splitMaxShift = RT_SPLIT_MAX_SHIFT;
@@ -314,7 +319,7 @@
   c->rayRate = pixelsPerRay;
   for (auto& b : c->binWorkBuf) RT_HIP(hipMemset(b, 0, (size_t)c->numBinsMax * 4));
   RT_HIP(hipDeviceSynchronize());
-  c->splitDemand = 0u; c->rayCountersInFlight = false; c->lastFrameRays = 0xFFFFFFFFu; c->traceLaunches = 0u;
+  c->splitDemand = 0u; c->rayCountersInFlight = false; c->lastFrameRays = 0xFFFFFFFFu; c->traceLaunches = 0u; c->listCountsPending.any = false;
   return 0;
 }
 
diff --git a/raytracedggx_amd/csrc/debug.hip b/raytracedggx_amd/csrc/debug.hip
--- a/raytracedggx_amd/csrc/debug.hip
+++ b/raytracedggx_amd/csrc/debug.hip
@@ -1,6 +1,7 @@
 #include <cstring>
 #include "capi_internal.h"
 #include "rt_queue.h"
+#include "rt_blocklist.h"
 namespace rt {
 __global__ void __launch_bounds__(256) copyKernel(const float4* __restrict__ src, float4* __restrict__ dst, size_t n) {
   for (size_t i = (size_t)blockIdx.x * 256u + threadIdx.x; i < n; i += (size_t)gridDim.x * 256u) dst[i] = src[i];
@@ -94,6 +95,18 @@
   if (forceSmall >= 0) c->lastTraceSmall = forceSmall == 1;
   if (key) *key = c->lastPlacement[0];
   if (where) *where = c->lastPlacement[1];
+  return 0;
+}
+int rtggx_debug_block_lists(rtggx_context* c, int mode, uint32_t gridCap) {
+  RT_CHECK_CTX(c);
+  if (mode != 0 && mode != 1) { setError("rtggx_debug_block_lists: mode %d: 0 or 1", mode); return -1; }
+  c->blockListMode = mode; c->blockListGridCap = gridCap;
+  return 0;
+}
+int rtggx_debug_block_lists_used(rtggx_context* c, uint32_t* kernels, uint32_t* grids) {
+  RT_CHECK_CTX(c);
+  if (kernels) *kernels = c->listedKernels;
+  if (grids) for (int k = 0; k < RT_LISTS; ++k) grids[k] = c->listedGrid[k];
   return 0;
 }
 int rtggx_debug_collapse_weights(rtggx_context* c, const float* set, float* get) {
@@ -212,6 +225,13 @@
       if (!c->accRefl) { setError("buffer %d exists once accumulation has been enabled (rtggx_set_accumulation)", id); return -1; }
       *ptr = id == RTGGX_BUF_ACC_REFL ? (void*)c->accRefl : id == RTGGX_BUF_ACC_DIFF ? (void*)c->accDiff : (void*)c->converged;
       *bytes = n * (id == RTGGX_BUF_CONVERGED ? 8u : 16u); return 0;
+    case RTGGX_BUF_LIST_SHADE: case RTGGX_BUF_LIST_H: case RTGGX_BUF_LIST_V: {
+      const int k = id - RTGGX_BUF_LIST_SHADE;
+      *ptr = c->cur().blockLists + c->listOff[k]; *bytes = (size_t)(1u + c->listCap[k]) * 4; return 0; }
+    case RTGGX_BUF_TILE_WORDS: {
+      const FrameParams& fp = c->slots[c->slot];
+      uint32_t rb, re; passRows(fp, ROWS_GBUFFER, rb, re);
+      *ptr = const_cast<uint32_t*>(c->tileWords(rb, re)); *bytes = (size_t)((fp.W + 15u) / 16u) * ((re - rb + 15u) / 16u) * 4; return 0; }
     default: setError("unknown buffer id %d", id); return -1;
   }
 }
diff --git a/raytracedggx_amd/csrc/denoise.hip b/raytracedggx_amd/csrc/denoise.hip
--- a/raytracedggx_amd/csrc/denoise.hip
+++ b/raytracedggx_amd/csrc/denoise.hip
@@ -1,14 +1,11 @@
 #include <cstring>
 #include <type_traits>
 #include "rtggx_context.h"
+#include "rt_blocklist.h"
 
 namespace rt {
 
 #define RT_RADIUS 16
-#ifndef RT_VBW
-#define RT_VBW 16
-#define RT_VBH 16
-#endif
 
 RT_DEV float rcpFast(float x) { return __builtin_amdgcn_rcpf(x); }
 
@@ -43,6 +40,7 @@
   const uint32_t* skyRun; uint32_t skyEpoch;
   uint32_t* settledOut; const uint32_t* settledIn; uint32_t settledPitch;
 };
+struct TargetsListed : Targets { const uint32_t* blockList; };
 #define RT_SGPR(v) ((uint32_t)__builtin_amdgcn_readfirstlane((int)(v)))
 RT_DEV uint32_t tileWordsOr(const uint32_t* words, uint32_t i0, uint32_t i1, uint32_t i2, uint32_t i3) {
   uint32_t a, b, c, d;
@@ -167,8 +165,27 @@
 }
 
 typedef float V4 __attribute__((ext_vector_type(4)));
-template <int MODE>
-__global__ void __launch_bounds__(256) spatialTiledKernel(Targets T) {
+#define RT_TILED_DONE { if constexpr (LISTED) continue; else return; }
+template <int MODE, bool LISTED = false>
+__global__ void __launch_bounds__(256) spatialTiledKernel(std::conditional_t<LISTED, TargetsListed, Targets> T) {
+  static_assert(!LISTED || MODE == 0 || MODE == 1, "lists exist for the reflection passes");
+  constexpr uint32_t PER_ENTRY = MODE == 0 ? RT_LIST_H_BLOCKS : 1u;
+  uint32_t listCount = 0u, listAt = blockIdx.x - gridDim.x;
+  if constexpr (LISTED) {
+    asm volatile("s_load_dword %0, %1, 0x0\n\ts_waitcnt lgkmcnt(0)" : "=s"(listCount) : "s"(T.blockList) : "memory");
+    listCount *= PER_ENTRY;
+  }
+  for (;;) {
+  uint32_t blockX = blockIdx.x, blockY = blockIdx.y, tid = threadIdx.x;
+  if constexpr (LISTED) asm volatile("" : "+v"(tid));
+  if constexpr (LISTED) {
+    listAt += gridDim.x;
+    if (listAt >= listCount) return;
+    uint32_t entry;
+    asm volatile("s_load_dword %0, %1, %2\n\ts_waitcnt lgkmcnt(0)" : "=s"(entry) : "s"(T.blockList), "s"((listAt / PER_ENTRY) * 4u + 4u) : "memory");
+    blockX = entry & 0xFFFFu; blockY = (entry >> 16) * PER_ENTRY + listAt % PER_ENTRY;
+    if (MODE == 0 && T.rowBegin + (int)(blockY * 4u) >= T.rowEnd) continue;
+  }
   constexpr bool vertical = (MODE & 1) != 0;
   constexpr bool diffuse = MODE >= 2;
   constexpr int BW = vertical ? RT_VBW : 64, BH = vertical ? RT_VBH : 4;
@@ -177,17 +194,16 @@
   constexpr int N = TW * TH;
   __shared__ V4 smA[N], smB[N];
   __shared__ uint32_t roughLo, roughHi, unflagged;
-  if (threadIdx.x == 0) { roughLo = 0xFFFFFFFFu; roughHi = 0u; unflagged = 0u; }
-  const int bx0 = blockIdx.x * BW, by0 = T.rowBegin + blockIdx.y * BH;
-  const int lx = threadIdx.x % BW, ly = threadIdx.x / BW;
+  if (tid == 0) { roughLo = 0xFFFFFFFFu; roughHi = 0u; unflagged = 0u; }
+  const int bx0 = blockX * BW, by0 = T.rowBegin + blockY * BH;
+  const int lx = tid % BW, ly = tid / BW;
   const int x = bx0 + lx;
 
   static_assert(RT_VBW <= 32 && RT_VBH <= 32, "the V block spans at most two tiles across and three down");
   bool nothingDrawn;
-  { const uint32_t txLast = (uint32_t)T.tilesX - 1u, tx0 = (uint32_t)bx0 >> 4, tx1 = min(tx0 + 1u, txLast);
-    const uint32_t ty0 = (uint32_t)(by0 - T.tileRow0) >> 4, ty1 = (uint32_t)(min(by0 + BH, T.rowEnd) - 1 - T.tileRow0) >> 4;
-    const uint32_t r0 = ty0 * (uint32_t)T.tilesX, r1 = ty1 * (uint32_t)T.tilesX, rm = ((ty0 + ty1) >> 1) * (uint32_t)T.tilesX;
-    if (MODE == 1 && T.skyRun != nullptr && skyRunMin6(T.skyRun, T.skyEpoch, r0 + tx0, r0 + tx1, rm + tx0, rm + tx1, r1 + tx0, r1 + tx1) >= RT_SKY_V_RUN) return;
+  { const BlockTileSpan span = blockTileSpan(bx0, by0, BH, T.rowEnd, T.tileRow0, T.tilesX);
+    const uint32_t txLast = span.txLast, tx0 = span.tx0, tx1 = span.tx1, r0 = span.r0, r1 = span.r1, rm = span.rm;
+    if (MODE == 1 && T.skyRun != nullptr && skyRunMin6(T.skyRun, T.skyEpoch, r0 + tx0, r0 + tx1, rm + tx0, rm + tx1, r1 + tx0, r1 + tx1) >= RT_SKY_V_RUN) RT_TILED_DONE
     nothingDrawn = vertical ? tileWordsOr6(T.tileWords, r0 + tx0, r0 + tx1, rm + tx0, rm + tx1, r1 + tx0, r1 + tx1) == 0u
                             : tileWordsOr(T.tileWords, r0 + tx0, r0 + tx1, r0 + min(tx0 + 2u, txLast), r0 + min(tx0 + 3u, txLast)) == 0u; }
   if (nothingDrawn) {
@@ -195,7 +211,7 @@
 #pragma unroll
       for (int k = 0; k < PER; ++k) { const int y = by0 + ly + k * ROWSTEP; if (x < T.W && y < T.rowEnd) storeSkipped<MODE>(T, (size_t)y * T.W + x); }
     }
-    return;
+    RT_TILED_DONE
   }
   bool todo[PER]; bool any = false;
 #pragma unroll
@@ -208,11 +224,11 @@
       if (skip) storeSkipped<MODE>(T, pix); else { todo[k] = true; any = true; }
     }
   }
-  if (!__syncthreads_or(any ? 1 : 0)) return;
+  if (!__syncthreads_or(any ? 1 : 0)) RT_TILED_DONE
 
   const int ox = vertical ? bx0 : bx0 - RT_RADIUS, oy = vertical ? by0 - RT_RADIUS : by0;
   uint32_t myLo = 0xFFFFFFFFu, myHi = 0u, myUnflagged = 0u;
-  for (int t = threadIdx.x; t < N; t += 256) {
+  for (int t = tid; t < N; t += 256) {
     const int tx = ox + t % TW, ty = oy + t / TW;
     float v[8] = {0.0f, 0.0f, 0.0f, 0.0f, 0.0f, 0.0f, 0.0f, 0.0f};
     const bool inside = tx >= 0 && ty >= 0 && tx < T.W && ty < T.H;
@@ -234,7 +250,7 @@
   if (!diffuse) {
     for (int o = 32; o > 0; o >>= 1) { myLo = min(myLo, (uint32_t)__shfl_down((int)myLo, o)); myHi = max(myHi, (uint32_t)__shfl_down((int)myHi, o)); }
     const unsigned long long anyUnflagged = __ballot(myUnflagged != 0u);
-    if ((threadIdx.x & 63) == 0) { atomicMin(&roughLo, myLo); atomicMax(&roughHi, myHi); if (anyUnflagged) atomicOr(&unflagged, 1u); }
+    if ((tid & 63) == 0) { atomicMin(&roughLo, myLo); atomicMax(&roughHi, myHi); if (anyUnflagged) atomicOr(&unflagged, 1u); }
   }
   __syncthreads();
   const int uniform = diffuse ? 0 : (roughLo != roughHi ? 0 : unflagged ? 1 : 2);
@@ -266,7 +282,10 @@
   if (uniform == 2) filter(std::integral_constant<int, 2>{});
   else if (uniform == 1) filter(std::integral_constant<int, 1>{});
   else filter(std::integral_constant<int, 0>{});
-}
+  if constexpr (LISTED) __syncthreads(); else return;
+  }
+}
+#undef RT_TILED_DONE
 
 RT_DEV f3 rgbToYCoCg(f3 c) {
   return mk3((c.x * 1.0f + c.y * 2.0f) + c.z * 1.0f, (c.x * 2.0f + c.y * 0.0f) + c.z * -2.0f, (c.x * -1.0f + c.y * 2.0f) + c.z * -1.0f);
@@ -669,8 +688,16 @@
   { uint32_t epoch;
     if (skyVPassMaySkip(c, TVr, (uint32_t)TV.tileRow0, &epoch) && useLds) { TVr.skyRun = c->cur().skyRun; TVr.skyEpoch = epoch; } }
   if (useLds) {
-    hipLaunchKernelGGL(spatialTiledKernel<0>, grid(TH, 64, 4), block, 0, s, TH); mark(4);
-    hipLaunchKernelGGL(spatialTiledKernel<1>, grid(TV, RT_VBW, RT_VBH), block, 0, s, TVr); mark(5);
+    const dim3 gridH = grid(TH, 64, 4), gridV = grid(TV, RT_VBW, RT_VBH);
+    const uint32_t listH = blockListGrid(c, fp, RT_LIST_H, TH.tileWords, gridH.x * gridH.y);
+    const uint32_t listV = TVr.skyRun ? blockListGrid(c, fp, RT_LIST_V, TVr.tileWords, gridV.x * gridV.y) : 0u;
+    TargetsListed L;
+    if (listH) { static_cast<Targets&>(L) = TH; L.blockList = c->cur().blockLists + c->listOff[RT_LIST_H]; hipLaunchKernelGGL((spatialTiledKernel<0, true>), dim3(listH), block, 0, s, L); }
+    else hipLaunchKernelGGL(spatialTiledKernel<0>, gridH, block, 0, s, TH);
+    mark(4);
+    if (listV) { static_cast<Targets&>(L) = TVr; L.blockList = c->cur().blockLists + c->listOff[RT_LIST_V]; hipLaunchKernelGGL((spatialTiledKernel<1, true>), dim3(listV), block, 0, s, L); }
+    else hipLaunchKernelGGL(spatialTiledKernel<1>, gridV, block, 0, s, TVr);
+    mark(5);
     if (anyDiffuse) hipLaunchKernelGGL(spatialTiledKernel<2>, grid(TH, 64, 4), block, 0, s, TH);
     mark(6);
     if (anyDiffuse) hipLaunchKernelGGL(spatialTiledKernel<3>, grid(TV, RT_VBW, RT_VBH), block, 0, s, TV);
diff --git a/raytracedggx_amd/csrc/raytrace.hip b/raytracedggx_amd/csrc/raytrace.hip
--- a/raytracedggx_amd/csrc/raytrace.hip
+++ b/raytracedggx_amd/csrc/raytrace.hip
@@ -2,6 +2,7 @@
 #include <type_traits>
 #include "rt_queue.h"
 #include "rt_traverse.h"
+#include "rt_blocklist.h"
 
 namespace rt {
 
@@ -307,8 +308,8 @@
                : "=&s"(wordHere), "=&s"(wordNext), "=&s"(skyWord) : "s"(A.visDirty), "s"(A.visDirtyNext), "s"(A.skyPrev), "s"(tile * 4u) : "memory");
   const bool drawn = wordHere != 0u;
   const bool clearNext = A.visNext != nullptr && wordNext != 0u;
-  const uint32_t skyPrevRun = (skyWord >> 8) == A.skyEpoch ? skyWord & 0xFFu : 0u;
-  const uint32_t skyWordOut = (A.skyEpoch << 8) | (drawn || RATE != 1 ? 0u : min(skyPrevRun + 1u, RT_SKY_RUN_CAP));
+  const uint32_t skyPrevRun = skyRunOf(skyWord, A.skyEpoch);
+  const uint32_t skyWordOut = (A.skyEpoch << 8) | skyRunNext(skyPrevRun, drawn || RATE != 1);
   if (RATE == 1 && !drawn && !clearNext && skyPrevRun >= A.skyPrevRun) {
     if (threadIdx.x == 0) A.skyOut[tile] = skyWordOut;
     return;
@@ -461,6 +462,104 @@
   }
 }
 
+#define RT_LIST_THREADS 1024
+#define RT_LIST_MAX_TILES 49152u
+#define RT_LIST_TILES 16384u
+#define RT_LIST_DRAWN 1u
+#define RT_LIST_RUN_SHORT 2u
+struct ListArgs {
+  const uint32_t* tileWords; const uint32_t* skyPrev; uint32_t skyEpoch;
+  uint32_t* lists; uint32_t off[RT_LISTS], cap[RT_LISTS];
+  uint32_t tilesX, tilesY, W, rowBegin, rowEnd;
+};
+template <int K>
+RT_DEV bool blockListed(const ListArgs& A, const uint8_t* flag, uint32_t x, uint32_t y, uint32_t& entry) {
+  if constexpr (K == RT_LIST_SHADE) { entry = y * A.tilesX + x; return (flag[entry] & RT_LIST_DRAWN) != 0u; }
+  else if constexpr (K == RT_LIST_H) {
+    const uint32_t r0 = y * A.tilesX, last = A.tilesX - 1u;
+    entry = (y << 16) | x;
+    return ((flag[r0 + 4u * x] | flag[r0 + min(4u * x + 1u, last)] | flag[r0 + min(4u * x + 2u, last)] | flag[r0 + min(4u * x + 3u, last)]) & RT_LIST_DRAWN) != 0u;
+  } else {
+    const BlockTileSpan t = blockTileSpan((int)(x * RT_VBW), (int)(A.rowBegin + y * RT_VBH), RT_VBH, (int)A.rowEnd, (int)A.rowBegin, (int)A.tilesX);
+    entry = (y << 16) | x;
+    return ((flag[t.r0 + t.tx0] | flag[t.r0 + t.tx1] | flag[t.rm + t.tx0] | flag[t.rm + t.tx1] | flag[t.r1 + t.tx0] | flag[t.r1 + t.tx1]) & RT_LIST_RUN_SHORT) != 0u;
+  }
+}
+template <int K>
+RT_DEV unsigned long long blockListMask(const ListArgs& A, const uint8_t* flag, uint32_t first, uint32_t n, uint32_t rowLen) {
+  unsigned long long mask = 0ull;
+  uint32_t x = first % rowLen, y = first / rowLen, e;
+  for (uint32_t j = 0; j < n; ++j) {
+    if (blockListed<K>(A, flag, x, y, e)) mask |= 1ull << j;
+    if (++x == rowLen) { x = 0u; ++y; }
+  }
+  return mask;
+}
+template <int K>
+RT_DEV void blockListStore(const ListArgs& A, const uint8_t* flag, uint32_t first, uint32_t rowLen, unsigned long long mask, uint32_t at) {
+  uint32_t* const list = A.lists + A.off[K] + 1u;
+  while (mask) {
+    const uint32_t item = first + (uint32_t)__builtin_ctzll(mask), x = item % rowLen, y = item / rowLen;
+    mask &= mask - 1ull;
+    if (at < A.cap[K]) list[at] = K == RT_LIST_SHADE ? item : (y << 16) | x;
+    ++at;
+  }
+}
+__global__ void __launch_bounds__(RT_LIST_THREADS) blockListKernel(ListArgs A) {
+  extern __shared__ uint8_t flag[];
+  __shared__ uint32_t waveTotal[RT_LISTS][RT_LIST_THREADS / 64];
+  const uint32_t t = threadIdx.x, lane = t & 63u, wave = t >> 6;
+  const uint32_t numTiles = A.tilesX * A.tilesY;
+  for (uint32_t base = 0u; base < numTiles; base += 8u * RT_LIST_THREADS) {
+    uint32_t word[8], prev[8];
+#pragma unroll
+    for (uint32_t k = 0; k < 8u; ++k) { const uint32_t i = min(base + k * RT_LIST_THREADS + t, numTiles - 1u); word[k] = A.tileWords[i]; prev[k] = A.skyPrev[i]; }
+#pragma unroll
+    for (uint32_t k = 0; k < 8u; ++k) {
+      const uint32_t i = base + k * RT_LIST_THREADS + t;
+      const bool drawn = word[k] != 0u;
+      if (i < numTiles) flag[i] = (uint8_t)((drawn ? RT_LIST_DRAWN : 0u) | (skyRunNext(skyRunOf(prev[k], A.skyEpoch), drawn) < RT_SKY_V_RUN ? RT_LIST_RUN_SHORT : 0u));
+    }
+  }
+  __syncthreads();
+  const uint32_t rowLen[RT_LISTS] = {A.tilesX, (A.tilesX + 3u) / 4u, (A.W + RT_VBW - 1u) / RT_VBW};
+  const uint32_t rows[RT_LISTS] = {A.tilesY, A.tilesY, (A.rowEnd - A.rowBegin + RT_VBH - 1u) / RT_VBH};
+  uint32_t first[RT_LISTS], n[RT_LISTS];
+#pragma unroll
+  for (int k = 0; k < RT_LISTS; ++k) {
+    const uint32_t items = rowLen[k] * rows[k], per = (items + RT_LIST_THREADS - 1u) / RT_LIST_THREADS;
+    first[k] = min(t * per, items); n[k] = min(first[k] + per, items) - first[k];
+  }
+  const unsigned long long mask[RT_LISTS] = {blockListMask<RT_LIST_SHADE>(A, flag, first[0], n[0], rowLen[0]), blockListMask<RT_LIST_H>(A, flag, first[1], n[1], rowLen[1]),
+                                             blockListMask<RT_LIST_V>(A, flag, first[2], n[2], rowLen[2])};
+  uint32_t at[RT_LISTS], total[RT_LISTS];
+#pragma unroll
+  for (int k = 0; k < RT_LISTS; ++k) {
+    const uint32_t mine = (uint32_t)__popcll(mask[k]);
+    uint32_t incl = mine;
+    for (int o = 1; o < 64; o <<= 1) { const uint32_t up = (uint32_t)__shfl_up((int)incl, o); if (lane >= (uint32_t)o) incl += up; }
+    if (lane == 63u) waveTotal[k][wave] = incl;
+    at[k] = incl - mine;
+  }
+  __syncthreads();
+#pragma unroll
+  for (int k = 0; k < RT_LISTS; ++k) {
+    uint32_t before = 0u, all = 0u;
+    for (uint32_t w = 0; w < RT_LIST_THREADS / 64; ++w) { const uint32_t c = waveTotal[k][w]; if (w < wave) before += c; all += c; }
+    at[k] += before; total[k] = all;
+  }
+  blockListStore<RT_LIST_SHADE>(A, flag, first[0], rowLen[0], mask[0], at[0]);
+  blockListStore<RT_LIST_H>(A, flag, first[1], rowLen[1], mask[1], at[1]);
+  blockListStore<RT_LIST_V>(A, flag, first[2], rowLen[2], mask[2], at[2]);
+  if (t < RT_LISTS) {
+    uint32_t count = min(total[t], A.cap[t]);
+#ifdef RT_BLOCK_LISTS_DROP_LAST
+    if (count) --count;
+#endif
+    A.lists[A.off[t]] = count; A.lists[t] = count;
+  }
+}
+
 struct ShadeArgs {
   const RayRec* rays; const HitKey* hits; const uint32_t* binCount; uint32_t binSlots;
   const float4* fat0; const float4* fat1;
@@ -472,6 +571,7 @@
   RayRec* spawnRays; HitKey* spawnHits; uint32_t* spawnCount; const float* cosSin;
   float* accRefl; float* accDiff;
 };
+struct ShadeArgsListed : ShadeArgs { const uint32_t* tileList; };
 
 enum ShadePass { SHADE_FINAL = 0, SHADE_SPAWN = 1, SHADE_FINAL_DEEP = 2, SHADE_ACCUM = 3, SHADE_SPAWN_ACCUM = 4 };
 constexpr bool shadeSpawns(int pass) { return pass == SHADE_SPAWN || pass == SHADE_SPAWN_ACCUM; }
@@ -501,18 +601,29 @@
                : "s"(words), "s"(RT_SGPR(i0 * 4u)), "s"(RT_SGPR(i1 * 4u)), "s"(RT_SGPR(i2 * 4u)), "s"(RT_SGPR(i3 * 4u)) : "memory");
   return a | b | c | d;
 }
-template <int RATE, int PASS, bool WIDE = false>
-__global__ void __launch_bounds__(256, RT_GEN_MIN_BLOCKS) shadeKernel(const FrameParams* __restrict__ fpp, ShadeArgs A) {
+template <int RATE, int PASS, bool WIDE = false, bool LISTED = false>
+__global__ void __launch_bounds__(256, LISTED && PASS == SHADE_FINAL ? 8 : RT_GEN_MIN_BLOCKS) shadeKernel(const FrameParams* __restrict__ fpp, std::conditional_t<LISTED, ShadeArgsListed, ShadeArgs> A) {
+  static_assert(!LISTED || RATE == 1, "the shade list names 16x16 tiles");
   const FrameParams& fp = *fpp;
   const EnvRef env{A.env, A.envSize, A.envMips, A.envMipOffset};
-  const uint32_t tile = blockIdx.x;
+  uint32_t listCount = 0u, listAt = blockIdx.x - gridDim.x;
+  if constexpr (LISTED) asm volatile("s_load_dword %0, %1, 0x0\n\ts_waitcnt lgkmcnt(0)" : "=s"(listCount) : "s"(A.tileList) : "memory");
+  for (;;) {
+  uint32_t tile = blockIdx.x, tidListed = threadIdx.x;
+  if constexpr (LISTED) asm volatile("" : "+v"(tidListed));
+#define RT_SHADE_TID (LISTED ? tidListed : threadIdx.x)
+  if constexpr (LISTED) {
+    listAt += gridDim.x;
+    if (listAt >= listCount) return;
+    asm volatile("s_load_dword %0, %1, %2\n\ts_waitcnt lgkmcnt(0)" : "=s"(tile) : "s"(A.tileList), "s"(listAt * 4u + 4u) : "memory");
+  }
   { uint32_t word;
     if constexpr (RATE == 1) asm volatile("s_load_dword %0, %1, %2\n\ts_waitcnt lgkmcnt(0)" : "=s"(word) : "s"(A.tileWords), "s"(tile * 4u) : "memory");
     else word = quadTileWord(A.tileWords, tile, A.tilesX, (A.rowEnd - A.rowBegin + 15u) / 16u);
-    if (word == 0u) return; }
-  const uint32_t bin = tile * 4u + (threadIdx.x >> 6);
+    if (word == 0u) { if constexpr (LISTED) continue; else return; } }
+  const uint32_t bin = tile * 4u + (RT_SHADE_TID >> 6);
   if (RATE == 1 && A.carryMask != 0u) {
-    const uint32_t lane = threadIdx.x & 63u, wave = threadIdx.x >> 6;
+    const uint32_t lane = RT_SHADE_TID & 63u, wave = RT_SHADE_TID >> 6;
     const uint32_t px = (tile % A.tilesX) * 16u + (wave & 1u) * 8u + (lane & 7u);
     const uint32_t py = A.rowBegin + (tile / A.tilesX) * 16u + (wave >> 1) * 8u + (lane >> 3);
     if (px < fp.W && py < A.rowEnd) {
@@ -523,7 +634,7 @@
   }
   const uint32_t count = min(A.binCount[bin] & 0xFFu, A.binSlots);
   uint32_t spawned = 0u;
-  for (uint32_t i = threadIdx.x & 63u; i < count; i += 64u) {
+  for (uint32_t i = RT_SHADE_TID & 63u; i < count; i += 64u) {
     const size_t slot = (size_t)bin * A.binSlots + i;
     const float4* rp = reinterpret_cast<const float4*>(A.rays + slot);
     const float4 q0 = rp[0], q1 = rp[1], q2 = rp[2];
@@ -592,7 +703,7 @@
     if constexpr (shadeSpawns(PASS)) {
       const unsigned long long mask = __ballot(child);
       if (child) {
-        const size_t k = (size_t)bin * A.binSlots + spawned + (uint32_t)__popcll(mask & ((1ull << (threadIdx.x & 63u)) - 1ull));
+        const size_t k = (size_t)bin * A.binSlots + spawned + (uint32_t)__popcll(mask & ((1ull << (RT_SHADE_TID & 63u)) - 1ull));
         A.spawnRays[k] = cr; A.spawnHits[k] = hitKey(RT_RAY_TMAX, 0xFFFFFFFFu);
       }
       spawned += (uint32_t)__popcll(mask);
@@ -607,7 +718,10 @@
     const bool toDiff = PASS == SHADE_FINAL ? diffuseGroup : ((rc.z ^ (rc.z >> 1)) & 1u) != 0u;
     if (toDiff) A.diffOut[rc.x] = packed; else A.reflOut[rc.x] = packed;
   }
-  if constexpr (shadeSpawns(PASS)) { if ((threadIdx.x & 63u) == 0u) A.spawnCount[bin] = spawned; }
+  if constexpr (shadeSpawns(PASS)) { if ((RT_SHADE_TID & 63u) == 0u) A.spawnCount[bin] = spawned; }
+  if constexpr (!LISTED) return;
+  }
+#undef RT_SHADE_TID
 }
 
 struct ReconArgs {
@@ -877,6 +991,7 @@
   G.binWork = adaptive ? c->binWork : nullptr; G.splitList = set.splitList; G.splitCount = set.splitCount;
   G.frontWork = RT_SPLIT_FRONT < splitWork ? RT_SPLIT_FRONT : splitWork;
   G.splitWork = splitWork; G.splitMaxShift = splitMaxShift < 3u ? splitMaxShift : 3u; G.splitCap = splitCap < RT_SPLIT_CAP ? splitCap : RT_SPLIT_CAP;
+  const uint32_t epochBefore = c->skyGen.any ? c->skyGen.epoch : 0xFFFFFFFFu;
   G.skyEpoch = skyEpochForGen(c, fp, rb, re, sGen, adaptive, sliceShift);
   if (c->skyEpochWrapped) {
     RT_HIP(hipDeviceSynchronize());
@@ -893,6 +1008,18 @@
     hipLaunchKernelGGL(sampleParamsKernel, dim3(1), dim3(256), 0, sGen, genParams, sp, c->samples);
     genParams = sp;
   }
+  { rtggx_context::ListGen& lg = c->listGen;
+    const bool whole = fp.rowBegin == 0u && fp.rowEnd == fp.H && fp.W == c->W && fp.H == c->H;
+    lg.built = c->blockListMode != 0 && !quad && whole && !c->lastTraceSmall && G.visDirty != c->visDirtyOnes.get() && tilesX * tilesY <= RT_LIST_TILES && G.skyEpoch == epochBefore;
+    lg.frame = c->frameCounter; lg.W = fp.W; lg.H = fp.H; lg.words = G.visDirty;
+    c->listedKernels = 0u; for (auto& g : c->listedGrid) g = 0u;
+    if (lg.built) {
+      ListArgs L;
+      L.tileWords = G.visDirty; L.skyPrev = G.skyPrev; L.skyEpoch = G.skyEpoch; L.lists = set.blockLists;
+      for (int k = 0; k < RT_LISTS; ++k) { L.off[k] = c->listOff[k]; L.cap[k] = c->listCap[k]; }
+      L.tilesX = tilesX; L.tilesY = tilesY; L.W = fp.W; L.rowBegin = rb; L.rowEnd = re;
+      hipLaunchKernelGGL(blockListKernel, dim3(1), dim3(RT_LIST_THREADS), (tilesX * tilesY + 15u) & ~15u, sGen, L);
+    } }
   const bool wide = c->sampleSet > RTGGX_MIN_SAMPLE_SET;
   launch(wide ? (quad ? rayGenKernel<4, true> : rayGenKernel<1, true>) : quad ? rayGenKernel<4> : rayGenKernel<1>, dim3(quad ? numBins : G.numTiles), dim3(256), sGen, nullptr, sGen != s ? ev.gen : nullptr, genParams, G);
   ev.genFrame = 0u; ev.genStream = sGen;
@@ -913,10 +1040,28 @@
   return 0;
 }
 
+uint32_t blockListGrid(rtggx_context* c, const FrameParams& fp, int k, const uint32_t* words, uint32_t fullGrid) {
+  const rtggx_context::ListGen& lg = c->listGen;
+  if (c->blockListMode == 0 || !lg.built || lg.frame != c->frameCounter || lg.W != fp.W || lg.H != fp.H || words != lg.words || fullGrid == 0u) return 0u;
+  uint32_t grid = c->blockListGridCap;
+  if (grid == 0u) {
+    const rtggx_context::ListCounts& n = c->listCounts;
+    if (!n.any || n.W != fp.W || n.H != fp.H) return 0u;
+    const uint32_t count = n.n[k] * (k == RT_LIST_H ? RT_LIST_H_BLOCKS : 1u);
+    grid = (count + (count + 15u) / 16u + 7u) & ~7u;
+    if (grid == 0u) grid = 8u;
+  }
+  if (grid > fullGrid) grid = fullGrid;
+  c->listedKernels |= 1u << k; c->listedGrid[k] = grid;
+  return grid;
+}
+
 static void (*const kShade[3][2])(const FrameParams*, ShadeArgs) = {
     {shadeKernel<1, SHADE_FINAL>, shadeKernel<4, SHADE_FINAL>}, {shadeKernel<1, SHADE_SPAWN>, shadeKernel<4, SHADE_SPAWN>},
     {shadeKernel<1, SHADE_FINAL_DEEP>, shadeKernel<4, SHADE_FINAL_DEEP>}};
 static void (*const kShadeSpawnWide[2])(const FrameParams*, ShadeArgs) = {shadeKernel<1, SHADE_SPAWN, true>, shadeKernel<4, SHADE_SPAWN, true>};
+static void (*const kShadeListed[4])(const FrameParams*, ShadeArgsListed) = {
+    shadeKernel<1, SHADE_FINAL, false, true>, shadeKernel<1, SHADE_SPAWN, false, true>, shadeKernel<1, SHADE_FINAL_DEEP, false, true>, shadeKernel<1, SHADE_SPAWN, true, true>};
 static int launchShadeSamples(rtggx_context* c, const FrameParams& fp, hipStream_t s, hipEvent_t done, ShadeArgs S, uint32_t numTiles, int spillPart) {
   const uint32_t N = c->samples, depth = c->maxDepth;
   const bool wide = c->sampleSet > RTGGX_MIN_SAMPLE_SET;
@@ -987,6 +1132,9 @@
   const uint32_t depth = c->maxDepth;
   const int spillPart = s == c->streamMain ? 2 : (int)c->traceSpillHalf;
   if (c->samples > 1u && !quad) return launchShadeSamples(c, fp, s, done, S, numTiles, spillPart);
+  const uint32_t listGrid = quad ? 0u : blockListGrid(c, fp, RT_LIST_SHADE, S.tileWords, grid);
+  ShadeArgsListed SL;
+  SL.tileList = set.blockLists + c->listOff[RT_LIST_SHADE];
   for (uint32_t level = 0; level < depth; ++level) {
     if (level > 0) {
       const TraceQueue q{S.rays, S.spawnHits, S.binCount};
@@ -995,7 +1143,10 @@
       S.carryMask = 0u;
     }
     const int pass = level + 1u < depth ? SHADE_SPAWN : level == 0 ? SHADE_FINAL : SHADE_FINAL_DEEP;
-    launch(pass == SHADE_SPAWN && c->sampleSet > RTGGX_MIN_SAMPLE_SET ? kShadeSpawnWide[quad] : kShade[pass][quad], dim3(grid), dim3(256), s, nullptr, pass == SHADE_SPAWN ? nullptr : done, dfp, S);
+    const bool wideSpawn = pass == SHADE_SPAWN && c->sampleSet > RTGGX_MIN_SAMPLE_SET;
+    const hipEvent_t rider = pass == SHADE_SPAWN ? nullptr : done;
+    if (listGrid) { static_cast<ShadeArgs&>(SL) = S; launch(kShadeListed[wideSpawn ? 3 : pass], dim3(listGrid), dim3(256), s, nullptr, rider, dfp, SL); }
+    else launch(wideSpawn ? kShadeSpawnWide[quad] : kShade[pass][quad], dim3(grid), dim3(256), s, nullptr, rider, dfp, S);
     RT_HIP(hipGetLastError());
   }
   return 0;
diff --git a/raytracedggx_amd/csrc/rt_blocklist.h b/raytracedggx_amd/csrc/rt_blocklist.h
--- /dev/null
+++ b/raytracedggx_amd/csrc/rt_blocklist.h
@@ -0,0 +1,38 @@
+#pragma once
+#include "rtggx_context.h"
+
+namespace rt {
+
+#ifndef RT_VBW
+#define RT_VBW 16
+#define RT_VBH 16
+#endif
+
+enum { RT_LIST_SHADE = 0, RT_LIST_H = 1, RT_LIST_V = 2, RT_LISTS = 3 };
+#define RT_LIST_H_BLOCKS 4u
+struct BlockListLayout { uint32_t off[RT_LISTS], cap[RT_LISTS], words; };
+inline BlockListLayout blockListLayout(uint32_t W, uint32_t H) {
+  const uint32_t tilesX = (W + 15u) / 16u, tilesY = (H + 15u) / 16u;
+  BlockListLayout L;
+  L.cap[RT_LIST_SHADE] = tilesX * tilesY;
+  L.cap[RT_LIST_H] = ((tilesX + 3u) / 4u) * tilesY;
+  L.cap[RT_LIST_V] = ((W + RT_VBW - 1u) / RT_VBW) * ((H + RT_VBH - 1u) / RT_VBH);
+  uint32_t at = 4u;
+  for (int k = 0; k < RT_LISTS; ++k) { L.off[k] = at; at += 1u + L.cap[k]; }
+  L.words = at;
+  return L;
+}
+
+RT_DEV uint32_t skyRunOf(uint32_t word, uint32_t epoch) { return (word >> 8) == epoch ? word & 0xFFu : 0u; }
+RT_DEV uint32_t skyRunNext(uint32_t prevRun, bool ends) { return ends ? 0u : min(prevRun + 1u, RT_SKY_RUN_CAP); }
+
+struct BlockTileSpan { uint32_t txLast, tx0, tx1, r0, rm, r1; };
+RT_DEV BlockTileSpan blockTileSpan(int bx0, int by0, int bh, int rowEnd, int tileRow0, int tilesX) {
+  BlockTileSpan s;
+  s.txLast = (uint32_t)tilesX - 1u; s.tx0 = (uint32_t)bx0 >> 4; s.tx1 = min(s.tx0 + 1u, s.txLast);
+  const uint32_t ty0 = (uint32_t)(by0 - tileRow0) >> 4, ty1 = (uint32_t)(min(by0 + bh, rowEnd) - 1 - tileRow0) >> 4;
+  s.r0 = ty0 * (uint32_t)tilesX; s.r1 = ty1 * (uint32_t)tilesX; s.rm = ((ty0 + ty1) >> 1) * (uint32_t)tilesX;
+  return s;
+}
+
+}
diff --git a/raytracedggx_amd/csrc/rtggx_context.h b/raytracedggx_amd/csrc/rtggx_context.h
--- a/raytracedggx_amd/csrc/rtggx_context.h
+++ b/raytracedggx_amd/csrc/rtggx_context.h
@@ -117,6 +117,7 @@
   DevBuf<uint32_t> binCount;
   DevBuf<uint32_t> splitList; uint32_t* splitCount = nullptr;
   DevBuf<uint32_t> skyRun;
+  DevBuf<uint32_t> blockLists;
   Event evRead;
   bool readRecorded = false;
 };
@@ -243,6 +244,11 @@
   struct SkyTM { bool any = false, fromTss = false; uint32_t frame = 0, epoch = 0, parity = 0, writes = 0, rows[2] = {0, 0}; } skyTM;
   uint32_t tssWrites[2] = {0, 0};
   bool useTileWords = true;
+  int blockListMode = 1; uint32_t blockListGridCap = 0;
+  uint32_t listOff[3] = {}, listCap[3] = {}, listWords = 0;
+  struct ListGen { bool built = false; uint32_t frame = 0, W = 0, H = 0; const uint32_t* words = nullptr; } listGen;
+  struct ListCounts { bool any = false; uint32_t W = 0, H = 0, n[3] = {0, 0, 0}; } listCounts, listCountsPending;
+  uint32_t listedKernels = 0, listedGrid[3] = {0, 0, 0};
   bool traversalBound = false;
   const uint32_t* traceTileWords = nullptr;
   rt::DevBuf<uint32_t> visDirtyOnes;
@@ -319,6 +325,7 @@
 void freeBuildProducts(MeshDev& m);
 int buildFatTris(rtggx_context* c, uint32_t slot, uint32_t set, hipStream_t s);
 int launchRayTrace(rtggx_context* c, const FrameParams& fp, hipStream_t sGen, hipStream_t sTrace, hipEvent_t done = nullptr);
+uint32_t blockListGrid(rtggx_context* c, const FrameParams& fp, int k, const uint32_t* words, uint32_t fullGrid);
 int launchShade(rtggx_context* c, const FrameParams& fp, hipStream_t s, hipEvent_t done = nullptr);
 int launchReconstruct(rtggx_context* c, const FrameParams& fp, hipStream_t s);
 int allocSamples(rtggx_context* c);
diff --git a/raytracedggx_amd/csrc/trace.hip b/raytracedggx_amd/csrc/trace.hip
--- a/raytracedggx_amd/csrc/trace.hip
+++ b/raytracedggx_amd/csrc/trace.hip
@@ -354,6 +354,7 @@
   if (countRays && c->rayCountersInFlight && hipEventQuery(c->evRayCounters) == hipSuccess) {
     uint32_t sum = 0; for (int i = 0; i < 256; ++i) sum += c->hostRayCounters[i];
     c->lastFrameRays = sum; c->splitDemand = c->hostRayCounters[256]; c->rayCountersInFlight = false;
+    if (c->listCountsPending.any) { c->listCounts = c->listCountsPending; for (int k = 0; k < 3; ++k) c->listCounts.n[k] = c->hostRayCounters[264 + k]; }
     steerTraceWaves(c, reinterpret_cast<const unsigned long long*>(c->hostRayCounters + 258), c->traceSampleLaunch);
   }
   const uint32_t raysGuess = countRays ? c->lastFrameRays : numBins * 40u;
@@ -423,6 +424,8 @@
     RT_HIP(hipMemcpyAsync(c->hostRayCounters, c->rayCounter32, 256 * 4, hipMemcpyDeviceToHost, s));
     RT_HIP(hipMemcpyAsync(c->hostRayCounters + 256, c->cur().splitCount, 4, hipMemcpyDeviceToHost, s));
     RT_HIP(hipMemcpyAsync(c->hostRayCounters + 258, c->traceStamps + 6, 16, hipMemcpyDeviceToHost, s)); c->traceSampleLaunch = c->traceLaunches;
+    c->listCountsPending.any = c->listGen.built && c->listGen.frame == c->frameCounter; c->listCountsPending.W = c->listGen.W; c->listCountsPending.H = c->listGen.H;
+    if (c->listCountsPending.any) RT_HIP(hipMemcpyAsync(c->hostRayCounters + 264, c->cur().blockLists, 12, hipMemcpyDeviceToHost, s));
     RT_HIP(hipEventRecord(c->evRayCounters, s));
     c->rayCountersInFlight = true;
     if (c->traceLaunches < RT_PRIME_LAUNCHES) RT_HIP(hipEventSynchronize(c->evRayCounters));
```

Result: slower. 3107 Mrays/s (-6.2%).
